# jsourati/nn-active-learning

Hardware: AMD Instinct MI355X
Metric: patches/sec Fisher-scored (32^3, 2-class) (higher is better)
Workload: dtype f32 (fp32 operands split into 16-bit pieces on the 16-bit MFMA, fp32 accumulate: fp16 pairs - 22-23 bits kept per operand, three products - in the conv under the head (forward + backward), in dec1's forward launch and in the other backward launches; bf16 triples - all 24 bits, exact, six products -

## Files before the change

include/alq.h:

```cpp
#ifndef ALQ_H
#define ALQ_H

#include <stddef.h>
#include <stdint.h>

#ifdef __cplusplus
extern "C" {
#endif

typedef struct alq_ctx alq_ctx;
typedef struct alq_model alq_model;

enum { ALQ_OK = 0, ALQ_EINVAL = -1, ALQ_EHIP = -2, ALQ_ENOMEM = -3, ALQ_EUNSUPPORTED = -4 };

enum { ALQ_CONV = 0, ALQ_CONVT = 1, ALQ_POOL = 2, ALQ_FC = 3 };

typedef struct {
    int32_t type;
    int32_t cout;
    int32_t k[3];
    int32_t s[3];
    int32_t relu;
    int32_t skip_src;
} alq_layer_t;
// ... 94 lines not shown
    float focal_gamma;
    float gce_q;
    float lwf_T;
    const float *d_class_w;
    const float *d_sample_w;
    const float *d_targets;
    const float *d_old_logits;
} alq_loss_t;

int alq_loss_stats(alq_ctx *ctx, const float *d_post, int c, int N, const int32_t *d_labels, const alq_loss_t *loss,
                   double *d_stats3);

int alq_param_grads_loss(alq_model *m, const float *d_x, int N, const int32_t *d_labels, const alq_loss_t *loss,
                         float loss_scale, float lwf_scale, float keep_prob, uint64_t seed, int64_t first_sample,
                         const int32_t *h_drop_layers, int n_drop_layers, float *d_grads, float *d_post, double *d_stats3);

int alq_rmsprop_step(alq_ctx *ctx, float *d_theta, const float *d_grad, float *d_ms, float *d_mom, int64_t n, float lr,
                     float decay, float momentum, float eps);

enum { ALQ_MT_L2 = 0, ALQ_MT_CE = 1 };
int64_t alq_mt_trip_voxels(void);
int alq_mt_cotangent(alq_ctx *ctx, const float *d_post, const float *d_teacher_post, int c, int64_t R, const int32_t *d_labels,
                     const alq_loss_t *loss, float loss_scale, float cons_scale, int measure, float *d_rows, double *d_stats3);
int alq_mt_stats(alq_ctx *ctx, const float *d_post, const float *d_teacher_post, int c, int64_t R, const int32_t *d_labels,
                 const alq_loss_t *loss, int measure, double *d_stats3);
int alq_param_grads_loss_mt(alq_model *m, const float *d_x, int N, const int32_t *d_labels, const alq_loss_t *loss,
                            float loss_scale, const float *d_teacher_post, int measure, float cons_scale, float keep_prob,
                            uint64_t seed, int64_t first_sample, const int32_t *h_drop_layers, int n_drop_layers, float *d_grads,
                            float *d_post, double *d_stats3);
int alq_model_set_aleatoric(alq_model *m, int on);
int alq_forward_au(alq_model *m, const float *d_x, int N, float keep_prob, uint64_t seed, int64_t first_sample,
                   const int32_t *h_drop_layers, int n_drop_layers, float *d_post, int64_t *d_pred, float *d_au, float *d_logits);
int64_t alq_mt_au_trip_voxels(void);
int alq_mt_cotangent_au(alq_ctx *ctx, const float *d_post, const float *d_teacher_post, const float *d_au, int c, int64_t R,
                        const int32_t *d_labels, const alq_loss_t *loss, float loss_scale, float cons_scale, float au_scale,
                        float au_log_rel_coeff, int measure, float *d_rows, double *d_stats3);
int alq_mt_stats_au(alq_ctx *ctx, const float *d_post, const float *d_teacher_post, const float *d_au, int c, int64_t R,
                    const int32_t *d_labels, const alq_loss_t *loss, float au_log_rel_coeff, int measure, double *d_stats3);
int alq_param_grads_loss_mt_au(alq_model *m, const float *d_x, int N, const int32_t *d_labels, const alq_loss_t *loss,
                               float loss_scale, const float *d_teacher_post, int measure, float cons_scale, float au_scale,
                               float au_log_rel_coeff, float keep_prob, uint64_t seed, int64_t first_sample,
                               const int32_t *h_drop_layers, int n_drop_layers, float *d_grads, float *d_post, double *d_stats3);
int alq_ema_step(alq_ctx *ctx, float *d_shadow, const float *d_theta, int64_t n, float decay);
int alq_perturb_input(alq_ctx *ctx, const float *d_x, float *d_out, int N, int H, int W, int C, float noise_std, uint64_t seed,
                      int64_t first_sample, int rotate, float angle);

int alq_sq_accum(alq_ctx *ctx, const float *d_grads, int64_t per_sample_len, int N, double *d_acc);

int alq_shrink_sum(alq_ctx *ctx, const float *d_grads, int N, int64_t P, const int64_t *h_layer_elems, int L, double *d_out);
int alq_class_layer_sums(alq_model *m, const float *d_x, int N, int J, const int32_t *d_cls, float *d_post, double *d_g);

int alq_diag_fisher(alq_model *m, const float *d_x, int N, const int32_t *d_cls, double *d_acc);

size_t alq_topk_mask_work_bytes(int64_t n);
int alq_topk_mask(alq_ctx *ctx, const double *d_v, int64_t n, int64_t k, float *d_mask, void *d_work);
int alq_threshold_mask(alq_ctx *ctx, const double *d_v, int64_t n, double thr, float *d_mask);
int alq_fisher_classes(alq_ctx *ctx, const double *d_g, const double *d_w, const double *d_diag, int N, int c, int L,
                       double *d_A);

int alq_row_norms(alq_ctx *ctx, const float *d_A, int64_t n, int f, double *d_norms);
int alq_cosine_sims(alq_ctx *ctx, const float *d_A, int64_t n, const float *d_B, int b, int f, const double *d_na,
                    const double *d_nb, double *d_C);
size_t alq_colsum_work_bytes(int64_t n, int b);
int alq_colsum_max(alq_ctx *ctx, const double *d_S, int64_t n, int b, const double *d_cmax,
                   const unsigned char *d_skip, double *d_out, void *d_work);
int alq_take_colmax(alq_ctx *ctx, const double *d_S, int64_t n, int b, int j, int first, double *d_v);
int alq_fold_rowmax(alq_ctx *ctx, const double *d_S, int t, int64_t n, double *d_v);

int alq_local_var2d(alq_ctx *ctx, const void *d_vol, int vol_is_f64, const int64_t pad_dims[3], const int32_t rads[3], int d,
                    const int64_t *d_inds, int64_t n, double *d_out);
int alq_segment_min(alq_ctx *ctx, const int32_t *d_labels, const int64_t dims[3], int32_t n_labels, const int64_t *d_inds,
                    const double *d_scores, int64_t n, double *d_table);

size_t alq_cc_work_bytes(const int64_t dims[3]);
int alq_cc_label(alq_ctx *ctx, const uint8_t *d_seg, const int64_t dims[3], int connectivity, int select_zero, int32_t *d_labels);
int alq_cc_keep_largest(alq_ctx *ctx, const uint8_t *d_seg, const int64_t dims[3], int connectivity, int skip_origin, uint8_t *d_out,
                        int64_t *d_info, void *d_work);
int alq_fill_holes(alq_ctx *ctx, const uint8_t *d_seg, const int64_t dims[3], uint8_t *d_out, int64_t *d_info, void *d_work);

typedef struct alq_dcrf_params {
    float sdims_smooth[2];
    float sdims_app[2];
    float schan;
    float compat_smooth, compat_app;
    int32_t niter;
} alq_dcrf_params;
size_t alq_dcrf_work_bytes(const int64_t dims[3]);
int alq_dcrf2d(alq_ctx *ctx, const float *d_post, const float *d_img, const int64_t dims[3], const alq_dcrf_params *par,
               float *d_q1, uint8_t *d_map, void *d_work);

int alq_llfc_grads(alq_ctx *ctx, const float *d_feat, const float *d_post, const int32_t *d_labels, int n, int d, int c,
                   float *d_out);
size_t alq_llfc_hess_max_bytes(void);
int alq_llfc_hess(alq_ctx *ctx, const float *d_feat_one, const float *d_post_one, int d, int c, double *d_H);
int alq_llfc_if_path(int d, int c);
size_t alq_llfc_if_work_bytes(int n_pool, int c);
int alq_llfc_stoch_if(alq_ctx *ctx, const float *d_pool_feat, const float *d_pool_post, const int32_t *d_pool_labels, int n_pool,
                      const float *d_tr_feat, const float *d_tr_post, int n_tr, const int32_t *d_draws, int T, double scale, int d,
                      int c, int path, float *d_V, void *d_work);

int alq_aopt_tile(void);
int alq_aopt_max_workgroups(void);
size_t alq_aopt_work_bytes(int64_t n, int L);
int alq_aopt_svec(alq_ctx *ctx, const double *d_A, int64_t n, int L, double *d_V);
int alq_aopt_stats(alq_ctx *ctx, const double *d_V, const double *d_q, int64_t n, int m, const double *h_kvec,
                   const double *h_R, double mu, double obj, double *d_out, void *d_work);
int alq_aopt_direction(alq_ctx *ctx, const double *d_V, const double *d_q, int64_t n, int m, const double *h_kvec,
                       const double *h_R, const double *h_c_r, const double *h_c_1, double ratio, double mu, double obj,
                       double *d_dq, double *d_out, void *d_work);
int alq_aopt_linesearch(alq_ctx *ctx, const double *d_q, const double *d_dq, int64_t n, const double *h_alpha, int J,
                        double *d_out, void *d_work);
int alq_aopt_update(alq_ctx *ctx, double *d_q, const double *d_dq, const double *d_V, int64_t n, int m, double alpha,
                    double *d_out, void *d_work);

typedef struct {
    int32_t layer;
    int32_t pad;
    int64_t idx;
    double delta;
} alq_flip_t;
int alq_ref64_scores(alq_ctx *ctx, const alq_layer_t *layers, int n_layers, const int32_t in_dims[4],
                     const double *const *h_dW, const double *const *h_db, const float *d_x, const int64_t *d_rows, int N,
                     const alq_flip_t *d_flips, int flips_per_sample, double eps, int cand_cap,
                     double *d_logits, double *d_S, double *d_rms, alq_flip_t *d_cand, double *d_cand_key, int32_t *d_cand_count);

int alq_prof_enable(alq_ctx *ctx, int on);
int alq_prof_reset(alq_ctx *ctx);
int alq_prof_num_classes(void);
const char *alq_prof_class_name(int cls);
int alq_prof_read(alq_ctx *ctx, int cls, double *ms, int64_t *launches, double *flops);

int alq_model_debug_copy(alq_model *m, int layer_idx, int what, int N, float *d_out,
                         int64_t *elems_out);

int alq_debug_set_stamp_buffer(void *d_buf);
int alq_debug_set(int key, int value);
enum {
    ALQ_INFO_SUBNORMALS_OK = 0,
    ALQ_INFO_C3D_FWD = 1,
    ALQ_INFO_C3D_BWD = 2,
    ALQ_INFO_C3D_ONE_ACC = 3,
    ALQ_INFO_FLIP_OVERFLOW = 5,
    ALQ_INFO_F16_DERIVED = 6,
    ALQ_INFO_T3D_FWD = 7,
    ALQ_INFO_T3D_BWD = 8,
    ALQ_INFO_E3D_BWD = 9,
    ALQ_INFO_D3D_FWD = 10,
    ALQ_INFO_D3D_BWD = 11,
    ALQ_INFO_F3D_FWD = 12,
    ALQ_INFO_C3D_BWD_FORM = 13,
    ALQ_INFO_HOST_PACK_ELEMS = 14,
    ALQ_INFO_LSUM = 15,
    ALQ_INFO_DCP_FORM = 16,
    ALQ_INFO_E3D_BWD_FORM = 17
};
int alq_model_engine_info(alq_model *m, int what);

int alq_synth_patches(alq_ctx *ctx, uint64_t seed, int64_t first_id, int64_t n,
                      int64_t elems_per_patch, float *d_out);

enum { ALQ_SRC_F32 = 0, ALQ_SRC_F64 = 1, ALQ_SRC_I16 = 2, ALQ_SRC_U8 = 3 };
int alq_vol_pack(alq_ctx *ctx, const void *const *d_src, int m, int src_type, const int32_t *dims, float *d_out);
int alq_mask_pack(alq_ctx *ctx, const uint8_t *d_src, const int32_t *dims, uint8_t *d_out);
int alq_slice_batch_check(const int32_t *h_dims, int nvol, const int32_t *h_desc, int b, const int32_t *crop, int C);
int alq_slice_batch(alq_ctx *ctx, const float *const *h_vols, const uint8_t *const *h_masks, const int32_t *h_dims, int nvol, int m,
                    const int32_t *h_desc, int b, const int32_t *crop, int C, float *d_X, int32_t *d_lab, int64_t *d_counts);
int64_t alq_slice_batch_trip_rows(void);
int alq_slice_batch_launch_samples(void);

#ifdef __cplusplus
}
#endif
#endif
```

nn-active-learning_amd/csrc/alq_internal.h:

```cpp
#pragma once
#include <hip/hip_runtime.h>

#include <cstdint>
#include <cstdio>
#include <memory>
#include <string>
#include <vector>

#include "alq.h"
#include "engine_switches.h"

namespace alq {

void set_error(const char *fmt, ...);

#define ALQ_HIP(expr)                                                                     \
    do {                                                                                  \
        hipError_t e_ = (expr);                                                           \
        if (e_ != hipSuccess) {                                                           \
            ::alq::set_error("%s:%d: %s -> %s", __FILE__, __LINE__, #expr,               \
                             hipGetErrorString(e_));                                      \
            return ALQ_EHIP;                                                              \
        }                                                                                 \
    } while (0)
// ... 254 lines not shown
    float *osumA, *osumB;
    const int *tdesc;
    const int *sdesc;
    const int *pdesc;
    const int *ttab;
    const int *vdesc;
    int in_cs, in_c0, out_cs, out_c0, Co;
    int mask_cs, mask_c0, mask_from, mask_to, split;
    int N, PT, tpg, rows;
    int PX, PYX, PZ;
    int smz, smy, smx;
    int soz, soy, sox, OD, OH, OW;
    int MD, MH, MW;
    int nph, ngr, NP;
    int nslots, plane_bytes;
    int in_pstride, out_pstride, in_bytes;
    int relu, accumulate, pair, store_from;
    int cls_ok;
    int in_split_ch, in_delta, out_split, out_delta, mask_split, mask_delta;
    int tt_ints, pd_off, td_off, wbytes, abytes;
    int dbg_repeat;
    unsigned long long *dbg;
    const unsigned *src_bits;
    int bits_pstride, bits_bytes;
    const float *fc_W;
    float *fc_part;
    unsigned char *fc_bits;
    int fc_F;
    int f16_ein;
    int f16_ew;
    const unsigned *in_amax, *in_amax2;
    unsigned *out_amax;
    int amax_from;
    int wp;
    int src_presplit;
    int xcd_order;
    int zreuse;
    float flip_tau;
    int flip_cap;
    unsigned *flip_cnt;
    unsigned *flip_list;
    const unsigned char *mask_bits;
    unsigned char *sign_out;
};

struct G4Geom {
    int kind = 0;
    int cls[3] = {0, 0, 0};
    int ID = 1, IH = 1, IW = 1, Ci = 0;
    int OD = 1, OH = 1, OW = 1, Co = 0;
    int k[3] = {1, 1, 1}, s[3] = {1, 1, 1}, lo[3] = {0, 0, 0};
    bool flipped = false;
    double flops_per_patch = 0;
};

struct Igemm4Plan {
    bool ok = false;
    Igemm4Args a;
    int NTW = 1;
    int wp = 3;
    int xw = 0;
    std::shared_ptr<Igemm4Plan> alt16;
    bool multi = false;
    bool fic = false;
    int tune_fic = -1;
    int tune_epi = -1;
    size_t lds_bytes = 0;
    double flops_per_patch = 0;
    int Ci = 0, Co = 0;
    struct Unit { int chunk = 0, S = 0, w_off = 0; std::vector<int> tap; };
    std::vector<Unit> units;
    std::vector<int> h_tdesc, h_sdesc, h_pdesc, h_ttab, h_vdesc;
    int *d_tdesc = nullptr, *d_sdesc = nullptr, *d_pdesc = nullptr, *d_ttab = nullptr, *d_vdesc = nullptr;
    std::vector<unsigned short> h_W;
    void *d_W = nullptr;
    std::vector<unsigned short> h_W16;
    void *d_W16 = nullptr;
    int w16_exp = 0;
};
int igemm4_build_plan(const G4Geom &g, int max_batch, Igemm4Plan *plan, int wp = 3);
void igemm4_pack_weights(Igemm4Plan *plan, const std::vector<float> &Bmat );
int igemm4_launch(alq_ctx *ctx, const Igemm4Plan &plan, const View &in, const View &out, const float *bias,
                  int relu, int accumulate, int N, int prof_cls, const Igemm2Fuse *fuse);

struct C3dPlan {
    bool ok = false;
    int D = 0;
    int w_exp = 0;
    int oneacc = 1;
    double flops_per_patch = 0;
    std::vector<unsigned short> h_W;
    void *d_W = nullptr;
    std::vector<unsigned short> h_W7;
    void *d_W7 = nullptr;
};
void c3d_bwd7_pack(C3dPlan *plan, const std::vector<float> &Bmat);
int c3d_subnormals_ok(alq_ctx *ctx);
int c3d_fwd_build(const View &in, const View &out, const int k[3], const int lo[3], const int s[3], C3dPlan *plan);
void c3d_fwd_pack(C3dPlan *plan, const std::vector<float> &Bmat );
int c3d_fwd_launch(alq_ctx *ctx, const C3dPlan &plan, const View &in, const float *bias, int N, const unsigned *amaxA, const unsigned *amaxB,
                   const float *fc_W, float *fc_part, float *asum_part, unsigned char *fc_bits, float flip_tau);
int c3d_bwd_build(const View &fwd_in, const View &fwd_out, const int k[3], const int lo[3], const int s[3], C3dPlan *plan);
void c3d_bwd_pack(C3dPlan *plan, const std::vector<float> &Bmat_fwd );
void c3d_presplit_vec(const float *v, long long F, int e, std::vector<unsigned short> *out);
int c3d_bwd_launch(alq_ctx *ctx, const C3dPlan &plan, int N, const unsigned char *bits, const void *vec16, int e_in, const unsigned char *maskA,
                   float *dB, float *sumA, float *sumB, int rows_per_wave = 8);

struct T3dPlan {
    bool ok = false;
    int kind = 0;
    int w_exp = 0;
    double flops_per_patch = 0;
    std::vector<unsigned short> h_W;
    void *d_W = nullptr;
};
int t3d_build(const View &in, const View &out, const int k[3], const int lo[3], const int s[3], T3dPlan *fwd, T3dPlan *bwd);
void t3d_fwd_pack(T3dPlan *plan, const float *W );
void t3d_bwd_pack(T3dPlan *plan, const float *W);
void t3d8_fwd_pack(T3dPlan *plan, const float *W );
void t3d8_bwd_pack(T3dPlan *plan, const float *W );
int t3d8_bwd_launch(alq_ctx *ctx, const T3dPlan &plan, const View &dout, const View &din, int N, float in_bound, const unsigned char *mask_bits, float *dsum);
int t3d_fwd_launch(alq_ctx *ctx, const T3dPlan &plan, const View &in, const View &out, const float *bias, int N, float *osum, unsigned *out_amax);
int t3d_bwd_launch(alq_ctx *ctx, const T3dPlan &plan, const View &dout, const View &din, int N, float in_bound, const unsigned char *mask_bits,
                   float *dsum);

struct E3dPlan {
    bool ok = false;
    int w_exp = 0;
    double flops_per_patch = 0;
    std::vector<unsigned short> h_Whi, h_Wlo;
    void *d_Whi = nullptr, *d_Wlo = nullptr;
};
int e3d_build(const View &in, const View &out, const int k[3], const int lo[3], const int s[3], E3dPlan *plan);
void e3d_pack(E3dPlan *plan, const float *W );
int e3d_bwd_launch(alq_ctx *ctx, const E3dPlan &plan, int N, const float *skip, const float *dpool, const unsigned char *am2, const unsigned char *sg2,
                   const unsigned char *am1, const unsigned char *sg1, float *dsum2, float *dsum1, float in_bound,
                   bool rows );

struct D3dPlan {
    bool ok = false;
    int w_exp = 0;
    double flops_per_patch = 0;
    std::vector<unsigned short> h_Whi, h_Wlo;
    void *d_Whi = nullptr, *d_Wlo = nullptr;
    std::vector<unsigned short> h_Bhi, h_Blo;
    void *d_Bhi = nullptr, *d_Blo = nullptr;
};
void d3d_bwd_pack(D3dPlan *plan, const float *W);
int d3d_bwd_launch(alq_ctx *ctx, const D3dPlan &plan, int N, const float *dout, float in_bound, float *dinA, float *dinB, float *sumB);
int d3d_build(const View &in, const View &out, const int k[3], const int lo[3], const int s[3], D3dPlan *plan);
void d3d_pack(D3dPlan *plan, const float *W );
int d3d_fwd_launch(alq_ctx *ctx, const D3dPlan &plan, int N, const float *inA, const float *inB, const unsigned *amaxA, const unsigned *amaxB,
                   const float *bias, int relu, float *out, unsigned char *sg, float *osum);

struct F3dPlan {
    bool ok = false;
    int w_exp = 0;
    double flops_per_patch = 0;
    std::vector<unsigned short> h_Whi, h_Wlo;
    void *d_Whi = nullptr, *d_Wlo = nullptr;
};
int f3d_build(const View &in, const View &out, const int k[3], const int lo[3], const int s[3], F3dPlan *plan);
void f3d_pack(F3dPlan *plan, const float *W );
int f3d_fwd_launch(alq_ctx *ctx, const F3dPlan &plan, int N, const float *in, const unsigned *amax, const float *bias, float *out, unsigned char *sg,
                   float *osum, float *pout, unsigned char *parg, float *posum);

struct DirectArgs {
    const float *in;
    float *out;
    const float *W;
    const float *bias;
    float *osum;
    int in_cs, in_c0, Ci, ID, IH, IW;
    int out_cs, out_c0, Co, OD, OH, OW;
    int MD, MH, MW;
    int PT, TZ, TY, TX, HZ, HY, HX, rows;
    int minz, miny, minx;
    int ntaps, tnx, tny, tnz;
    int tilesZ, tilesY, tilesX;
    int N, relu;
};

struct DirectPlan {
    DirectArgs a;
    bool ok = false;
    size_t lds_bytes = 0;
    double flops_per_patch = 0;
    float *d_W = nullptr;
};

int direct_build_plan(const IgemmPlan &p1, DirectPlan *dp);
int direct_launch(alq_ctx *ctx, const DirectPlan &dp, const View &in, const View &out, const float *bias, int relu,
                  int N, float *osum, int prof_cls);
int direct_conv_pool_launch(alq_ctx *ctx, const float *d_W, const View &in, const View &out, const View &pout,
                            const float *bias, int relu, uint8_t *argmax, float *osum, float *posum, int N,
                            double flops_per_patch, unsigned *amax = nullptr, unsigned char *sg = nullptr, unsigned char *psg = nullptr);

struct FcGemmPlan {
    bool ok = false;
    int K = 0, N = 0;
    std::vector<unsigned short> h_W;
    void *d_W = nullptr;
    std::vector<unsigned short> h_W16;
    void *d_W16 = nullptr;
    int w_exp = 0;
    int form = 0;
};
int fcgemm_build_plan(int K, int N, FcGemmPlan *plan);
void fcgemm_pack_weights(FcGemmPlan *plan, const std::vector<float> &Bmat );
void fcgemm_pack_weights_f16(FcGemmPlan *plan, const std::vector<float> &Bmat );
int fcgemm_launch(alq_ctx *ctx, const FcGemmPlan &plan, const View &in, const View &out, const float *bias, int relu,
                  int M, int prof_cls, float in_bound = 0.f, unsigned *row_amax = nullptr);

int wpack_stats(alq_ctx *ctx, const float *d_W, int Co, long long F, void *d_scal);
int wpack_permute(alq_ctx *ctx, const float *d_W, float *d_Wp, int Co, int D, int H, int Wd, int C);
int wpack_fc(alq_ctx *ctx, const float *d_Wp, long long ld, int K, int N, int kmajor, void *d_W3, void *d_W16, const void *d_scal);

struct Gemm {
    IgemmPlan p1;
    Igemm2Plan p2;
    Igemm3Plan p3;
    Igemm4Plan p4;
    FcGemmPlan pfc;
    bool pfc_f16 = false;
    bool p3_f16 = false;
    unsigned *fc_row_amax = nullptr;
    DirectPlan pd;
};

int k_pool_fwd(alq_ctx *, const View &in, const View &out, uint8_t *argmax, const int w[3],
               const int lo[3], int N, float *osum = nullptr, bool *fused = nullptr);
int k_pool_bwd_first(alq_ctx *, const View &dout, const View &pool_out, const uint8_t *argmax, const int w[3],
                     int ID, int IH, int IW, int N, float *dsum, int accumulate, int use_signs = 0);
int k_pool_bwd(alq_ctx *, const View &dout, const View &din, const uint8_t *argmax,
               const int w[3], const int lo[3], int N, int accumulate, const View *mask_act = nullptr,
               float *dsum = nullptr, bool *fused = nullptr, int store_din = 1, int use_signs = 0);
int k_chansum(alq_ctx *, const View &in, float *field, int N);
int k_mask_chansum(alq_ctx *, const View &dact, const View *act_or_null, float *field, int N);
int boxdot_slabs(long long vox);
int boxdot_conv_slabs(int D, int H, int W, const int k[3]);
int boxdot_convT_slabs(int ID, int IH, int IW, const int k[3], const int s[3]);
int k_boxdot_conv(alq_ctx *, const float *dsum, const float *asum, const float *asum2, int D, int H, int W,
                  const int k[3], const int lo[3], int N, double *Spart, int nslab_max);
int k_boxdot_convT(alq_ctx *, const float *dsum, const float *asum, const float *asum2, int ID, int IH, int IW,
                   const int k[3], const int s[3], const int lo[3], int N, double *Spart, int nslab_max);
int k_fc_small_fwd(alq_ctx *, const float *act, int64_t F, const float *Wp, int nout, int N,
                   float *partials, int nslices, unsigned *maskbits = nullptr);
int k_fc_small_dsum_bits(alq_ctx *, const unsigned *maskbits, const float *wv, int64_t F, int N, float *dsum);
int k_fc_small_finish(alq_ctx *, const float *partials, int nslices, const float *bias, int nout,
                      int relu, int N, float *out);
int k_fc_small_finish_diff(alq_ctx *, const float *partials, int nslices, const float *bias, int N, float *out);
int k_fc_small_bwd(alq_ctx *, const float *delta, int nout, const float *Wp, int64_t F, int N,
                   float *dact, const float *mask_act = nullptr, float *dsum = nullptr, int C = 0,
                   bool *fused = nullptr);
int k_rowsum_field(alq_ctx *, const float *field, int64_t len, int N, float *out);
struct FwdBoundsArgs { int nl; float L[16]; float B[16]; int src2[16]; int from_input = 0; };
int k_rowmax_abs(alq_ctx *, const float *x, int N, long long K, unsigned *out);
int k_fwd_bounds(alq_ctx *, const unsigned *amax0, int N, int stride, const FwdBoundsArgs &a, unsigned *bound_all);
int flip_segments(int N);
int flip_list_len(int N);
int k_flip_fix(alq_ctx *, unsigned *list, unsigned *cnt, int cap, int N, const float *inA, const float *inB, int CA, int CB,
               int D, int H, int W, int kz, int ky, int kx, int lz, int ly, int lx, const float *W32, const float *bias, int Co,
               unsigned char *bits, long long F, unsigned *overflow = nullptr);
int k_rowmax_u32(alq_ctx *, const unsigned *in, int len, int N, unsigned *out);
int k_softmax(alq_ctx *, const float *logits, int c, int N, float *post_cN, int64_t *pred);
int k_fill_unit_cotangent(alq_ctx *, float *dlogits, int N);
int k_fisher_finalize(alq_ctx *, const double *Spart, const int *nslab, int nslab_max, int max_batch, double *S,
                      int L, const double *sizes, const float *post_cN, const float *p1_branch, int N,
                      double diag_load, float *p1_out, double *g0, double *g1, double *A, double *trace,
                      double *Apart, int *nblocks_out);
int k_reduce_Asum(alq_ctx *, const double *Apart, int nblocks, int LL, double *Asum);
int fc_small_slices(int64_t F);

int k_dropout(alq_ctx *, const View &t, int N, long long first_sample, unsigned long long seed, int layer, float keep_prob);
int k_logit_cotangent(alq_ctx *, const float *post_cN, int c, int N, int mode, int cls, const int *labels, float scale,
                      float *dlogits);
int k_ce_loss(alq_ctx *, const float *post_cN, int c, int N, const int *labels, double *d_out);
long long wgrad_partial_floats(const View &U, const View &V, const int k[3]);
int k_wgrad(alq_ctx *, const View &U, const View &V, const int k[3], const int s[3], const int lo[3], int N, int sum_n,
            float *partial, float *d_out, long long out_stride);
int k_bgrad(alq_ctx *, const View &delta, int N, int sum_n, float *d_out, long long out_stride);
int k_fc_wgrad(alq_ctx *, const float *delta, const View &a, int nout, int N, int sum_n, float *d_out, long long out_stride);
int k_sgd(alq_ctx *, float *theta, const float *g, long long n, float lr);
int k_loss_cotangent(alq_ctx *, const float *post_cN, int c, int N, const int *labels, const alq_loss_t *loss, float loss_scale,
                     float lwf_scale, float *dlogits, double *d_stats3);
int k_dense_head_fwd(alq_ctx *, const float *x, long long R, int Ci, int c, const float *W, const float *b, float *post_cR, int64_t *pred,
                     float *z);
int k_dense_head_fwd_au(alq_ctx *, const float *x, long long R, int Ci, int c, const float *W, const float *b, float *post_cR,
                        int64_t *pred, float *au, float *z);
int k_dense_head_bwd(alq_ctx *, const float *delta, const float *x, long long R, int Ci, int c, const float *W, float *dx, int accumulate,
                     double *part, float *d_dW_db);
int k_rmsprop(alq_ctx *, float *theta, const float *g, float *ms, float *mom, long long n, float lr, float decay, float momentum,
              float eps);
int k_adam(alq_ctx *, float *theta, const float *g, float *m, float *v, long long n, float lr_t, float b1, float b2, float eps);
int k_sq_accum(alq_ctx *, const float *g, long long per, int N, double *acc);
int k_shrink_sum(alq_ctx *, const float *g, int N, long long P, const long long *off, int L, double *out);
int k_fisher_classes(alq_ctx *, const double *g, const double *w, const double *diag, int N, int c, int L, double *A);

long long gnorm_partials(const View &U, const View &V, const int k[3], const int s[3], const int lo[3]);
int k_gnorm_weight(alq_ctx *, const View &U, const View &V, const int k[3], const int s[3], const int lo[3], int N, double *part,
                   double *d_sq, int ld, int col);
int k_gnorm_bias(alq_ctx *, const View &delta, int N, double *d_sq, int ld, int col);
int k_gnorm_fc(alq_ctx *, const float *delta, int nout, const View &a, int N, double *d_sq, int ld, int col);

long long dfisher_weight_scratch(const View &U, const View &V, const int k[3], const int s[3], const int lo[3], int max_batch);
int k_dfisher_weight(alq_ctx *, const View &U, const View &V, const int k[3], const int s[3], const int lo[3], int N, double *scratch,
// ... 98 lines not shown
```

nn-active-learning_amd/csrc/engine_switches.h:

```cpp
#ifndef ALQ_ENGINE_SWITCHES_H
#define ALQ_ENGINE_SWITCHES_H
#include <cstddef>
#include <cstdlib>

namespace alq {

enum Knob {
    KNOB_REPEAT = 0,
    KNOB_FLAGS = 1,
    KNOB_NO_BWD_FUSE = 2,
    KNOB_NO_FWD_FUSE = 3,
    KNOB_NO_V3 = 4,
    KNOB_NO_V4 = 5,
    KNOB_NO_POOL_FIRST = 6,
    KNOB_NO_CONV_POOL = 7,
    KNOB_DCP_NARROW = 8,
    KNOB_E3D_GRID_CAP = 9,
    ALQ_NKNOBS = 10
};

struct EngineSwitches {
    int knobs[ALQ_NKNOBS] = {0, 0, 0, 0, 0, 0, 0, 0, 0, 0};
    int disable_v2 = 0;
    int disable_v3 = 0;
    int disable_v4 = 0;
    int no_fcgemm = 0;
    int no_split = 0;
    int no_wide2d_rule = 0;
    int no_v3_f16 = 0;
    int no_v3_f16_fwd = 0;
    int no_co_split = 0;
    int no_co_split_f16 = 0;
    int no_class_tiles = 0;
    int no_fc_bits = 0;
    int no_fc_fuse = 0;
    int no_fc_f16 = 0;
    int no_fc_f16_fwd = 0;
    int f16_derived_mask = 0;
    int has_f16_derived_mask = 0;
    int no_f16x2 = 0;
    int no_xcd_order = 0;
    int no_fixed = 0;
    int no_bound16 = 0;
    int no_flipfix = 0;
    int no_presplit = 0;
    int no_signs = 0;
    int no_signs0 = 0;
    int f16_fwd_mask = -1;
    int no_f16_derived = 0;
    int no_light_kernels = 0;
    int no_c3d = 0;
    int c3_bwd_rows = 7;
    int no_e3d = 0;
    int e3d_rows = 0;
    int no_d3d = 0;
    int no_d3b = 0;
    int no_f3d = 0;
    int no_t3d = 0;
};

enum SwitchRule {
    SW_PRESENT,
    SW_FIRST_IS_1,
    SW_ATOI_EQ,
    SW_INT,
    SW_ROWS
};

struct SwitchRow {
    const char *env;
    size_t member;
    SwitchRule rule;
    int arg;
};

#define ALQ_SW(env, member, rule, arg) {env, offsetof(EngineSwitches, member), rule, arg}
inline const SwitchRow kSwitchTable[] = {
    ALQ_SW("ALQ_DEBUG_REPEAT", knobs[KNOB_REPEAT], SW_INT, 0),
    ALQ_SW("ALQ_DEBUG_FLAGS", knobs[KNOB_FLAGS], SW_INT, 0),
    ALQ_SW("ALQ_NO_BWD_FUSE", knobs[KNOB_NO_BWD_FUSE], SW_INT, 0),
    ALQ_SW("ALQ_NO_FWD_FUSE", knobs[KNOB_NO_FWD_FUSE], SW_INT, 0),
    ALQ_SW("ALQ_NO_V3", knobs[KNOB_NO_V3], SW_INT, 0),
    ALQ_SW("ALQ_NO_V4", knobs[KNOB_NO_V4], SW_INT, 0),
    ALQ_SW("ALQ_NO_POOL_FIRST", knobs[KNOB_NO_POOL_FIRST], SW_INT, 0),
    ALQ_SW("ALQ_NO_CONV_POOL", knobs[KNOB_NO_CONV_POOL], SW_INT, 0),
    ALQ_SW("ALQ_DCP_NARROW", knobs[KNOB_DCP_NARROW], SW_INT, 0),
    ALQ_SW("ALQ_E3D_GRID_CAP", knobs[KNOB_E3D_GRID_CAP], SW_INT, 0),
    ALQ_SW("ALQ_DISABLE_V2", disable_v2, SW_FIRST_IS_1, 0),
    ALQ_SW("ALQ_DISABLE_V3", disable_v3, SW_FIRST_IS_1, 0),
    ALQ_SW("ALQ_DISABLE_V4", disable_v4, SW_PRESENT, 0),
    ALQ_SW("ALQ_NO_FCGEMM", no_fcgemm, SW_PRESENT, 0),
    ALQ_SW("ALQ_NO_SPLIT", no_split, SW_PRESENT, 0),
    ALQ_SW("ALQ_NO_WIDE2D_RULE", no_wide2d_rule, SW_PRESENT, 0),
    ALQ_SW("ALQ_NO_V3_F16", no_v3_f16, SW_PRESENT, 0),
    ALQ_SW("ALQ_NO_V3_F16_FWD", no_v3_f16_fwd, SW_PRESENT, 0),
    ALQ_SW("ALQ_NO_CO_SPLIT", no_co_split, SW_PRESENT, 0),
    ALQ_SW("ALQ_NO_CO_SPLIT_F16", no_co_split_f16, SW_PRESENT, 0),
    ALQ_SW("ALQ_NO_CLASS_TILES", no_class_tiles, SW_PRESENT, 0),
    ALQ_SW("ALQ_NO_FC_BITS", no_fc_bits, SW_PRESENT, 0),
    ALQ_SW("ALQ_NO_FC_FUSE", no_fc_fuse, SW_PRESENT, 0),
    ALQ_SW("ALQ_NO_FC_F16", no_fc_f16, SW_PRESENT, 0),
    ALQ_SW("ALQ_NO_FC_F16_FWD", no_fc_f16_fwd, SW_PRESENT, 0),
    ALQ_SW("ALQ_F16_DERIVED_MASK", f16_derived_mask, SW_INT, 0),
    ALQ_SW("ALQ_F16_DERIVED_MASK", has_f16_derived_mask, SW_PRESENT, 0),
    ALQ_SW("ALQ_NO_F16X2", no_f16x2, SW_PRESENT, 0),
    ALQ_SW("ALQ_NO_XCD_ORDER", no_xcd_order, SW_PRESENT, 0),
    ALQ_SW("ALQ_NO_FIXED", no_fixed, SW_PRESENT, 0),
    ALQ_SW("ALQ_NO_BOUND16", no_bound16, SW_PRESENT, 0),
    ALQ_SW("ALQ_NO_FLIPFIX", no_flipfix, SW_PRESENT, 0),
    ALQ_SW("ALQ_NO_PRESPLIT", no_presplit, SW_PRESENT, 0),
    ALQ_SW("ALQ_NO_SIGNS", no_signs, SW_PRESENT, 0),
    ALQ_SW("ALQ_NO_SIGNS0", no_signs0, SW_PRESENT, 0),
    ALQ_SW("ALQ_F16_FWD_MASK", f16_fwd_mask, SW_INT, 0),
    ALQ_SW("ALQ_F16_DERIVED", no_f16_derived, SW_ATOI_EQ, 0),
    ALQ_SW("ALQ_NO_F16_DERIVED", no_f16_derived, SW_ATOI_EQ, 1),
    ALQ_SW("ALQ_NO_LIGHT_KERNELS", no_light_kernels, SW_PRESENT, 0),
    ALQ_SW("ALQ_NO_C3D", no_c3d, SW_PRESENT, 0),
    ALQ_SW("ALQ_C3D_BWD_ROWS", c3_bwd_rows, SW_ROWS, 0),
    ALQ_SW("ALQ_NO_E3D", no_e3d, SW_PRESENT, 0),
    ALQ_SW("ALQ_E3D_ROWS", e3d_rows, SW_ATOI_EQ, 1),
    ALQ_SW("ALQ_NO_D3D", no_d3d, SW_PRESENT, 0),
    ALQ_SW("ALQ_NO_D3D_BWD", no_d3b, SW_PRESENT, 0),
    ALQ_SW("ALQ_NO_F3D", no_f3d, SW_PRESENT, 0),
    ALQ_SW("ALQ_NO_T3D", no_t3d, SW_PRESENT, 0),
};
#undef ALQ_SW
inline const int kNumSwitchRows = (int)(sizeof(kSwitchTable) / sizeof(kSwitchTable[0]));

inline int &switch_member(EngineSwitches &sw, const SwitchRow &row) {
    return *reinterpret_cast<int *>(reinterpret_cast<char *>(&sw) + row.member);
}

inline EngineSwitches read_engine_switches() {
    EngineSwitches sw;
    for (const SwitchRow &row : kSwitchTable) {
        const char *v = std::getenv(row.env);
        int &dst = switch_member(sw, row);
        switch (row.rule) {
            case SW_PRESENT:    if (v) dst = 1; break;
            case SW_FIRST_IS_1: if (v && v[0] == '1') dst = 1; break;
            case SW_ATOI_EQ:    if (v && std::atoi(v) == row.arg) dst = 1; break;
            case SW_INT:        if (v) dst = std::atoi(v); break;
            case SW_ROWS:       dst = (v && std::atoi(v) == 4) ? 4 : ((v && std::atoi(v) == 8) ? 8 : 7); break;
        }
    }
    return sw;
}

}
#endif
```

nn-active-learning_amd/csrc/igemm2.hip:

```cpp
#include "alq_internal.h"

#include <algorithm>
#include <cmath>
#include <cstring>

namespace alq {

typedef float f32x4 __attribute__((ext_vector_type(4)));
typedef float f32x2 __attribute__((ext_vector_type(2)));

#ifdef ALQ_STAMPS
#define STAMP(var) asm volatile("s_memtime %0\n\ts_waitcnt lgkmcnt(0)" : "=s"(var)::"memory")
#define PHASE_END(idx)                         \
    do {                                       \
        unsigned long long t_now_;             \
        STAMP(t_now_);                         \
        ph[idx] += t_now_ - t_last;            \
        t_last = t_now_;                       \
    } while (0)
#else
#define PHASE_END(idx) do {} while (0)
#endif

constexpr int I2_CBP = 12;
// ... 331 lines not shown
                        mm(a1, b1);
                        __builtin_amdgcn_sched_barrier(0);
                    }
                }
            }
            PHASE_END(6);
        }
        have_pend = true;
        p_out = c_out; p_cls = c_cls; p_l = c_l; p_g = c_g;
        more = next_more;
    }
    if (have_pend) flush();
#ifdef ALQ_STAMPS
    PHASE_END(7);
    if (a.dbg && tid == 0)
        for (int i = 0; i < 8; ++i) a.dbg[blockIdx.x * 8 + i] = ph[i];
#endif
}

int igemm2_build_plan(const IgemmPlan &p1, Igemm2Plan *p2) {
    p2->ok = false;
    const IgemmArgs &a1 = p1.a;
    if (p1.smallc || p1.CB != 8 || a1.NB != 1 || p1.NTW > 3 || a1.ntaps > 27 || a1.Co % 4) return ALQ_OK;
    const int halo = a1.HZ * a1.HY * a1.HX;
    const int nhv = a1.PT * halo;
    if (nhv * 2 > 256 * I2_MAXSLOT) return ALQ_OK;
    if (a1.HZ > 255 || a1.HY > 255 || a1.HX > 255 || a1.PT > 127) return ALQ_OK;
    const size_t wchunk = (size_t)a1.ntaps * p1.NTW * 128 * 4;
    size_t wres_max = I2_WRES_MAX;
    if (const char *e = getenv("ALQ_WRES_KB")) wres_max = (size_t)atoi(e) * 1024;
    const bool wres = wchunk * a1.nchunks <= wres_max * p1.NTW;
    const size_t wbytes = wres ? wchunk * a1.nchunks : wchunk;
    const size_t lds = wbytes + (size_t)nhv * I2_CBP * 4;
    if (lds > 156 * 1024) return ALQ_OK;
    Igemm2Args &a = p2->a;
    std::memset(&a, 0, sizeof(a));
    a.Ci = a1.Ci; a.ID = a1.ID; a.IH = a1.IH; a.IW = a1.IW;
    a.Co = a1.Co; a.OD = a1.OD; a.OH = a1.OH; a.OW = a1.OW;
    a.MD = a1.MD; a.MH = a1.MH; a.MW = a1.MW;
    a.sm = a1.sm; a.so = a1.so; a.ooffz = a1.ooffz; a.ooffy = a1.ooffy; a.ooffx = a1.ooffx;
    a.PT = a1.PT; a.TZ = a1.TZ; a.TY = a1.TY; a.TX = a1.TX; a.HZ = a1.HZ; a.HY = a1.HY; a.HX = a1.HX;
    a.rows = a1.rows; a.minz = a1.minz; a.miny = a1.miny; a.minx = a1.minx;
    a.ntaps = a1.ntaps; a.nchunks = a1.nchunks;
    a.tilesZ = a1.tilesZ; a.tilesY = a1.tilesY; a.tilesX = a1.tilesX;
    {
        std::vector<int> off(a1.ntaps);
        for (int t = 0; t < a1.ntaps; ++t) off[t] = a1.tapoff[t] / 10 * I2_CBP;
        bool found = false;
        for (int nx = 1; nx <= a1.ntaps && !found; ++nx) {
            if (a1.ntaps % nx) continue;
            for (int ny = 1; nx * ny <= a1.ntaps && !found; ++ny) {
                if ((a1.ntaps / nx) % ny) continue;
                const int nz = a1.ntaps / (nx * ny);
                const int sx = nx > 1 ? off[1] - off[0] : 0;
                const int sy = ny > 1 ? off[nx] - off[0] : 0;
                const int sz = nz > 1 ? off[nx * ny] - off[0] : 0;
                bool okb = true;
                for (int t = 0; t < a1.ntaps && okb; ++t) {
                    const int ix = t % nx, iy = (t / nx) % ny, iz = t / (nx * ny);
                    okb = off[t] == off[0] + iz * sz + iy * sy + ix * sx;
                }
                if (okb) {
                    a.t0 = off[0]; a.tsx = sx; a.tsy = sy; a.tsz = sz; a.tnx = nx; a.tny = ny;
                    found = true;
                }
            }
        }
        if (!found) return ALQ_OK;
    }
    a.split = 1 << 30;
    {
        const int dimsI[3] = {a.ID, a.IH, a.IW}, dimsM[3] = {a.MD, a.MH, a.MW};
        const int T[3] = {a.TZ, a.TY, a.TX}, tiles[3] = {a.tilesZ, a.tilesY, a.tilesX};
        const int mins[3] = {a.minz, a.miny, a.minx}, H[3] = {a.HZ, a.HY, a.HX};
        auto cls_of = [&](int d, int t) { return (t == 0 ? 1 : 0) | (t == tiles[d] - 1 ? 2 : 0); };
        auto valid1 = [&](int d, int t, int h) {
            const int c = t * T[d] * a.sm + mins[d] + h;
            return c >= 0 && c < dimsI[d];
        };
        for (int d = 0; d < 3; ++d)
            for (int t = 1; t + 1 < tiles[d]; ++t)
                for (int h = 0; h < H[d]; ++h)
                    if (!valid1(d, t, h)) return ALQ_OK;
        a.tpg = a.tilesZ * a.tilesY * a.tilesX;
        a.in_pstride = a.PT * a.ID * a.IH * a.IW;
        a.out_pstride = a.PT * a.OD * a.OH * a.OW;
        p2->h_tdesc.assign((size_t)a.tpg * 8, 0);
        for (int tz = 0; tz < a.tilesZ; ++tz)
            for (int ty = 0; ty < a.tilesY; ++ty)
                for (int tx = 0; tx < a.tilesX; ++tx) {
                    int *td = &p2->h_tdesc[(((size_t)tz * a.tilesY + ty) * a.tilesX + tx) * 8];
                    const int mz0 = tz * a.TZ, my0 = ty * a.TY, mx0 = tx * a.TX;
                    const int z0 = mz0 * a.sm + a.minz, y0 = my0 * a.sm + a.miny, x0 = mx0 * a.sm + a.minx;
                    td[0] = (z0 * a.IH + y0) * a.IW + x0;
                    td[1] = ((mz0 * a.so + a.ooffz) * a.OH + my0 * a.so + a.ooffy) * a.OW + mx0 * a.so + a.ooffx;
                    const int cls = cls_of(0, tz) | (cls_of(1, ty) << 2) | (cls_of(2, tx) << 4);
                    const bool full = a.rows == 256 && mz0 + a.TZ <= a.MD && my0 + a.TY <= a.MH && mx0 + a.TX <= a.MW;
                    td[2] = cls | (full ? 256 : 0);
                    td[3] = mz0; td[4] = my0; td[5] = mx0;
                }
        (void)dimsM;
        auto rep = [&](int d, int c) { return (c & 1) ? 0 : ((c & 2) ? tiles[d] - 1 : (tiles[d] > 2 ? 1 : 0)); };
        p2->h_sdesc.assign((size_t)nhv * 4, 0);
        for (int pt = 0; pt < a.PT; ++pt)
            for (int hz = 0; hz < a.HZ; ++hz)
                for (int hy = 0; hy < a.HY; ++hy)
                    for (int hx = 0; hx < a.HX; ++hx) {
                        const int hv = ((pt * a.HZ + hz) * a.HY + hy) * a.HX + hx;
                        int *sd = &p2->h_sdesc[(size_t)hv * 4];
                        sd[0] = ((pt * a.ID + hz) * a.IH + hy) * a.IW + hx;
                        unsigned long long m = 0;
                        for (int c = 0; c < 64; ++c) {
                            const int cz = c & 3, cy = (c >> 2) & 3, cx = (c >> 4) & 3;
                            if (valid1(0, rep(0, cz), hz) && valid1(1, rep(1, cy), hy) && valid1(2, rep(2, cx), hx))
                                m |= 1ull << c;
                        }
                        sd[1] = (int)(unsigned)(m & 0xffffffffull);
                        sd[2] = (int)(unsigned)(m >> 32);
                        sd[3] = (pt << 24) | (hz << 16) | (hy << 8) | hx;
                    }
    }
    p2->NTW = p1.NTW;
    p2->wres = wres;
    p2->lds_bytes = lds;
    int max_wgs = 2;
    if (const char *e = getenv("ALQ_MAX_WGS")) max_wgs = atoi(e);
    p2->wgs_per_cu = std::max<int>(1, std::min<int>(max_wgs, (int)((160 * 1024) / (lds + 512))));
    p2->flops_per_patch = p1.flops_per_patch;
    p2->ok = true;
    return ALQ_OK;
}

void igemm2_pack_weights(Igemm2Plan *p2, const std::vector<float> &Bmat) {
    const Igemm2Args &a = p2->a;
    const int NTW = p2->NTW, Ci = a.Ci, Co = a.Co;
    p2->h_W.assign((size_t)a.nchunks * a.ntaps * NTW * 128, 0.f);
    for (int ch = 0; ch < a.nchunks; ++ch)
        for (int tp = 0; tp < a.ntaps; ++tp)
            for (int nt = 0; nt < NTW; ++nt)
                for (int lane = 0; lane < 64; ++lane)
                    for (int s = 0; s < 2; ++s) {
                        const int c = ch * 8 + 2 * (lane >> 4) + s;
                        const int co = nt * 16 + (lane & 15);
                        if (co < Co)
                            p2->h_W[((((size_t)ch * a.ntaps + tp) * NTW + nt) * 64 + lane) * 2 + s] =
                                Bmat[((size_t)tp * Ci + c) * Co + co];
                    }
}

unsigned long long *g_igemm2_dbg = nullptr;
int g_no_f16x2 = 0;
int g_no_xcd_order = 0;
int g_no_fixed = 0;
int g_dbg_knobs[ALQ_NKNOBS] = {0, 0, 0, 0, 0, 0, 0, 0, 0, 0};

template <int NTW, bool WRES, int GEO, bool SUMS>
static int launch2_s(alq_ctx *ctx, const Igemm2Plan &plan, const Igemm2Args &a, unsigned grid) {
    auto kfn = igemm2_kernel<NTW, WRES, GEO, SUMS>;
    if (plan.lds_bytes > 64 * 1024)
        ALQ_HIP(hipFuncSetAttribute(reinterpret_cast<const void *>(kfn), hipFuncAttributeMaxDynamicSharedMemorySize,
                                    (int)plan.lds_bytes));
    hipLaunchKernelGGL(kfn, dim3(grid), dim3(256), plan.lds_bytes, ctx->stream, a);
    ALQ_HIP(hipGetLastError());
    return ALQ_OK;
}

template <int NTW, bool WRES, int GEO>
static int launch2_t(alq_ctx *ctx, const Igemm2Plan &plan, const Igemm2Args &a, unsigned grid) {
    return (a.osumA || a.osumB) ? launch2_s<NTW, WRES, GEO, true>(ctx, plan, a, grid)
                                : launch2_s<NTW, WRES, GEO, false>(ctx, plan, a, grid);
}

int igemm2_launch(alq_ctx *ctx, const Igemm2Plan &plan, const View &in, const View &out, const float *bias, int relu,
                  int accumulate, int N, int prof_cls, const Igemm2Fuse *fuse) {
    Igemm2Args a = plan.a;
    ALQ_REQUIRE(in.C == a.Ci && in.D == a.ID && in.H == a.IH && in.W == a.IW, ALQ_EINVAL,
                "igemm2: input view does not match plan");
    ALQ_REQUIRE(out.C == a.Co && out.D == a.OD && out.H == a.OH && out.W == a.OW, ALQ_EINVAL,
                "igemm2: output view does not match plan");
    ALQ_REQUIRE(plan.d_W != nullptr, ALQ_EINVAL, "igemm2: weights not set");
    ALQ_REQUIRE((long long)N * in.vox() * in.cs < (1LL << 29) && (long long)N * out.vox() * out.cs < (1LL << 29),
                ALQ_EUNSUPPORTED, "igemm2: tensor exceeds the 32-bit byte-offset range (lower the batch)");
    ALQ_REQUIRE(in.cs % 4 == 0 && in.c0 % 4 == 0 && out.cs % 4 == 0 && out.c0 % 4 == 0, ALQ_EUNSUPPORTED,
                "igemm2: channel slice not 16-byte aligned");
    if (fuse) ALQ_REQUIRE(fuse->split % 4 == 0 && fuse->mask_cs % 4 == 0 && fuse->mask_c0 % 4 == 0 && fuse->mask_from % 4 == 0, ALQ_EUNSUPPORTED,
                          "igemm2: fused epilogue needs 4-channel aligned slices");
    a.in = in.p; a.in_cs = in.cs; a.in_c0 = in.c0;
    a.out = out.p; a.out_cs = out.cs; a.out_c0 = out.c0;
    a.W = plan.d_W; a.bias = bias; a.relu = relu; a.accumulate = accumulate; a.N = N;
    a.in_bytes = (int)((long long)N * in.vox() * in.cs * 4);
    a.dbg = nullptr;
    if (g_igemm2_dbg) {
        static int want = -2;
        if (want == -2) { const char *e = getenv("ALQ_STAMP_ONLY"); want = e ? atoi(e) : -1; }
        static int ordinal = 0;
        static unsigned long long *last = nullptr;
        if (last != g_igemm2_dbg) { last = g_igemm2_dbg; ordinal = 0; }
        if (want < 0 || ordinal == want) a.dbg = g_igemm2_dbg;
        ++ordinal;
    }
    a.dbg_repeat = g_dbg_knobs[KNOB_REPEAT];
    a.dbg_flags = g_dbg_knobs[KNOB_FLAGS];
    if (fuse) {
        a.mask = fuse->mask; a.mask_cs = fuse->mask_cs; a.mask_c0 = fuse->mask_c0; a.mask_from = fuse->mask_from;
        a.osumA = fuse->osumA; a.osumB = fuse->osumB;
        a.split = fuse->split > 0 ? fuse->split : (1 << 30);
    }
    const int pgroups = (N + a.PT - 1) / a.PT;
    const long long total = (long long)pgroups * a.tilesZ * a.tilesY * a.tilesX;
    const unsigned grid = (unsigned)std::min<long long>(total, 256LL * plan.wgs_per_cu);
    ProfScope ps(ctx, prof_cls, plan.flops_per_patch * N);
    int geo = 0;
    if (a.ntaps == 27 && a.tnx == 3 && a.tny == 3 && a.HY == 6 && a.HX == 18) {
        const int SX = I2_CBP, SY = 18 * I2_CBP, SZ = 6 * 18 * I2_CBP;
        if (a.t0 == 0 && a.tsx == SX && a.tsy == SY && a.tsz == SZ) geo = 1;
        if (a.t0 == 2 * (SX + SY + SZ) && a.tsx == -SX && a.tsy == -SY && a.tsz == -SZ) geo = 2;
    }
#define ALQ_L2(NT)                                                                                       \
    case NT:                                                                                             \
        if (geo == 1) return plan.wres ? launch2_t<NT, true, 1>(ctx, plan, a, grid) : launch2_t<NT, false, 1>(ctx, plan, a, grid); \
        if (geo == 2) return plan.wres ? launch2_t<NT, true, 2>(ctx, plan, a, grid) : launch2_t<NT, false, 2>(ctx, plan, a, grid); \
        return plan.wres ? launch2_t<NT, true, 0>(ctx, plan, a, grid) : launch2_t<NT, false, 0>(ctx, plan, a, grid)
    switch (plan.NTW) { ALQ_L2(1); ALQ_L2(2); ALQ_L2(3); }
#undef ALQ_L2
    set_error("igemm2: NTW=%d unsupported", plan.NTW);
    return ALQ_EUNSUPPORTED;
}

}
```

nn-active-learning_amd/csrc/model.hip:

```cpp
#include <algorithm>
#include <cmath>
#include <cstring>
#include <string>

#include "model_types.h"

namespace alq {

static void same_pads(int in, int k, int s, int *out, int *lo) {
    *out = (in + s - 1) / s;
    int total = (*out - 1) * s + k - in;
    if (total < 0) total = 0;
    *lo = total / 2;
}

}

using namespace alq;

static int g_knob_override[ALQ_NKNOBS] = {-1, -1, -1, -1, -1, -1, -1, -1, -1, -1};

static void apply_knobs(const alq_model *m) {
    for (int k = 0; k < ALQ_NKNOBS; ++k) g_dbg_knobs[k] = g_knob_override[k] >= 0 ? g_knob_override[k] : m->sw.knobs[k];
    g_no_f16x2 = m->sw.no_f16x2;
    g_no_xcd_order = m->sw.no_xcd_order;
    g_no_fixed = m->sw.no_fixed;
}

static int gemm_build(const EngineSwitches &sw, const ConvDesc &d, int max_batch, Gemm *g, const G4Geom *g4 = nullptr) {
    ALQ_TRY(igemm_build_plan(d, max_batch, &g->p1));
    if (g4 && !sw.disable_v4) {
        G4Geom gg = *g4;
        gg.flops_per_patch = g->p1.flops_per_patch;
        ALQ_TRY(igemm4_build_plan(gg, max_batch, &g->p4));
    }
    ALQ_TRY(igemm2_build_plan(g->p1, &g->p2));
    ALQ_TRY(direct_build_plan(g->p1, &g->pd));
    if (sw.disable_v2) { g->p2.ok = false; g->pd.ok = false; }
    ALQ_TRY(igemm3_build_plan(g->p2, &g->p3));
    if (d.ID == 1 && d.IH == 1 && d.IW == 1 && d.tz.size() == 1 && d.sm == 1 && d.so == 1 && !sw.no_fcgemm)
        ALQ_TRY(fcgemm_build_plan(d.Ci, d.Co, &g->pfc));
    if (sw.disable_v3) g->p3.ok = false;
    return ALQ_OK;
}

int prepare_call(alq_model *m, bool fisher) {
    m->last.call_fisher = fisher;
    apply_knobs(m);
    if (!two_slot_allowed()) ALQ_TRY(refresh_fallback_forms(m));
    return ALQ_OK;
}

enum GemmRoute { ROUTE_DIRECT, ROUTE_FCGEMM, ROUTE_IGEMM4, ROUTE_IGEMM3, ROUTE_IGEMM2, ROUTE_IGEMM };
static GemmRoute gemm_route(const Gemm &g, const View &in, const View &out, int accumulate, const Igemm2Fuse *fuse) {
    if (g.pd.ok && !accumulate && !(fuse && (fuse->mask || fuse->osumB || fuse->split))) return ROUTE_DIRECT;
    if (g.pfc.ok && !accumulate && !fuse && two_slot_allowed()) return ROUTE_FCGEMM;
    const bool split_view = in.split != 0 || out.split != 0;
    if (g.p4.ok && (two_slot_allowed() || split_view)) return ROUTE_IGEMM4;
    if (g.p3.ok && !g_dbg_knobs[KNOB_NO_V3]) return ROUTE_IGEMM3;
    return g.p2.ok ? ROUTE_IGEMM2 : ROUTE_IGEMM;
}

int gemm_launch(alq_ctx *ctx, const Gemm &g, const View &in, const View &out, const float *bias, int relu,
                int accumulate, int N, int cls, const Igemm2Fuse *fuse, bool *fused, float fc_in_bound) {
    const GemmRoute route = gemm_route(g, in, out, accumulate, fuse);
    ALQ_REQUIRE(route <= ROUTE_FCGEMM || g.p4.ok || (in.split == 0 && out.split == 0), ALQ_EUNSUPPORTED, "split concat view without a two-slot plan");
    if (fused) *fused = fuse != nullptr && route != ROUTE_FCGEMM && route != ROUTE_IGEMM;
    const int cls3 = cls == PROF_IGEMM_BWD ? PROF_IGEMM3_BWD : PROF_IGEMM3_FWD;
    switch (route) {
        case ROUTE_DIRECT: return direct_launch(ctx, g.pd, in, out, bias, relu, N, fuse ? fuse->osumA : nullptr, PROF_DIRECT);
        case ROUTE_FCGEMM:
            return fcgemm_launch(ctx, g.pfc, in, out, bias, relu, N, cls3, (g_no_f16x2 || bias || relu) ? 0.f : fc_in_bound,
                                 (cls == PROF_IGEMM_FWD && !g_no_f16x2) ? g.fc_row_amax : nullptr);
        case ROUTE_IGEMM4: return igemm4_launch(ctx, g.p4, in, out, bias, relu, accumulate, N, cls3, fuse);
        case ROUTE_IGEMM3: return igemm3_launch(ctx, g.p2, g.p3, in, out, bias, relu, accumulate, N, cls3, fuse);
        case ROUTE_IGEMM2: return igemm2_launch(ctx, g.p2, in, out, bias, relu, accumulate, N, cls, fuse);
        case ROUTE_IGEMM: break;
    }
    return igemm_launch(ctx, g.p1, in, out, bias, relu, accumulate, N, cls);
}

static void enum_taps(const int k[3], std::vector<int> *tz, std::vector<int> *ty, std::vector<int> *tx) {
    for (int z = 0; z < k[0]; ++z)
        for (int y = 0; y < k[1]; ++y)
            for (int x = 0; x < k[2]; ++x) {
                tz->push_back(z); ty->push_back(y); tx->push_back(x);
            }
}

static int build_model(alq_model *m, const alq_layer_t *specs, int n_layers) {
    const EngineSwitches &sw = m->sw;
    m->layers.resize(n_layers);
    struct Shp { int D, H, W, C; };
    std::vector<Shp> outs(n_layers);
    Shp cur = {m->in_dims[0], m->in_dims[1], m->in_dims[2], m->in_dims[3]};
    bool flat = false;
    int pidx = 0;
    std::vector<int> src_of(n_layers, -1);
    std::vector<int> dest_of(n_layers, -1);
    for (int i = 0; i < n_layers; ++i) {
        Layer &ly = m->layers[i];
        ly.spec = specs[i];
        const alq_layer_t &sp = ly.spec;
        Shp in = cur;
        if (sp.skip_src >= 0) {
            ALQ_REQUIRE(sp.skip_src < i - 1, ALQ_EUNSUPPORTED, "layer %d: skip source %d must be an earlier, non-adjacent layer", i, sp.skip_src);
            ALQ_REQUIRE(dest_of[sp.skip_src] < 0, ALQ_EUNSUPPORTED, "layer %d feeds more than one concat", sp.skip_src);
            const Shp &s = outs[sp.skip_src];
            ALQ_REQUIRE(!flat && s.D == cur.D && s.H == cur.H && s.W == cur.W, ALQ_EUNSUPPORTED,
                        "layer %d: concat of maps of different size (resize_image_with_crop_or_pad) is outside the scored path", i);
            in.C = cur.C + s.C;
            src_of[i] = sp.skip_src;
            dest_of[sp.skip_src] = i;
        }
        Shp o = in;
        switch (sp.type) {
            case ALQ_CONV: {
                ALQ_REQUIRE(!flat, ALQ_EINVAL, "layer %d: conv after fc", i);
                ALQ_REQUIRE(sp.s[0] == 1 && sp.s[1] == 1 && sp.s[2] == 1, ALQ_EUNSUPPORTED, "layer %d: strided conv", i);
                for (int d = 0; d < 3; ++d) {
                    int od;
                    same_pads((&in.D)[d], sp.k[d], 1, &od, &ly.lo[d]);
                }
                o.C = sp.cout;
                ly.pidx = pidx++;
                ly.w_elems = (int64_t)sp.k[0] * sp.k[1] * sp.k[2] * in.C * sp.cout;
                ly.b_elems = sp.cout;
                break;
            }
            case ALQ_CONVT: {
                ALQ_REQUIRE(!flat, ALQ_EINVAL, "layer %d: conv_transpose after fc", i);
                for (int d = 0; d < 3; ++d) {
                    ALQ_REQUIRE(sp.k[d] >= sp.s[d], ALQ_EUNSUPPORTED, "layer %d: conv_transpose kernel < stride", i);
                    int od;
                    same_pads((&in.D)[d] * sp.s[d], sp.k[d], sp.s[d], &od, &ly.lo[d]);
                }
                ALQ_REQUIRE(sp.s[0] == sp.s[1] || in.D == 1, ALQ_EUNSUPPORTED, "layer %d: anisotropic stride", i);
                ALQ_REQUIRE(sp.s[1] == sp.s[2], ALQ_EUNSUPPORTED, "layer %d: anisotropic stride", i);
                o.D = in.D * sp.s[0]; o.H = in.H * sp.s[1]; o.W = in.W * sp.s[2];
                o.C = sp.cout;
                ly.pidx = pidx++;
                ly.w_elems = (int64_t)sp.k[0] * sp.k[1] * sp.k[2] * in.C * sp.cout;
                ly.b_elems = sp.cout;
                break;
            }
            case ALQ_POOL: {
                ALQ_REQUIRE(!flat, ALQ_EINVAL, "layer %d: pool after fc", i);
                for (int d = 0; d < 3; ++d) {
                    ALQ_REQUIRE(sp.k[d] == sp.s[d], ALQ_EUNSUPPORTED, "layer %d: pool window != stride", i);
                    ALQ_REQUIRE(sp.k[0] * sp.k[1] * sp.k[2] <= 255, ALQ_EUNSUPPORTED, "layer %d: pool window too large", i);
                    same_pads((&in.D)[d], sp.k[d], sp.s[d], &(&o.D)[d], &ly.lo[d]);
                }
                break;
            }
            case ALQ_FC: {
                ly.F = (int64_t)in.D * in.H * in.W * in.C;
                o = {1, 1, 1, sp.cout};
                ly.pidx = pidx++;
                ly.w_elems = ly.F * sp.cout;
                ly.b_elems = sp.cout;
                flat = true;
                break;
            }
            default:
                ALQ_REQUIRE(false, ALQ_EINVAL, "layer %d: unknown type %d", i, sp.type);
        }
        outs[i] = o;
        cur = o;
    }
    m->L = pidx;
    if (n_layers > 0 && specs[n_layers - 1].type == ALQ_CONV) {
        const int hl = n_layers - 1;
        const alq_layer_t &hs = specs[hl];
// ... 270 lines not shown
            }
        } else if (sp.type == ALQ_POOL) {
            uint8_t *am;
            ALQ_TRY(m->dalloc(&am, (size_t)NB * ly.out.vox() * ly.out.C));
            ly.argmax = am;
        } else {
            ALQ_REQUIRE(ly.in.cs == ly.in.C && ly.in.c0 == 0, ALQ_EUNSUPPORTED, "layer %d: fc on a concat slice", i);
            if (sp.cout <= 8) {
                ly.dense_fc_small = true;
                ly.fc_slices = fc_small_slices(ly.F);
                ALQ_TRY(m->dalloc(&ly.d_Wp, (size_t)sp.cout * ly.F));
                ALQ_TRY(m->dalloc(&ly.fc_partials, (size_t)NB * ly.fc_slices * sp.cout));
                if (sp.cout == 2 && ly.F % 1024 == 0 && i == n_layers - 1 && i > 0 && m->layers[i - 1].spec.relu && m->layers[i - 1].pidx > 0 &&
                    m->layers[i - 1].spec.type == ALQ_CONV && m->layers[i - 1].out.C == 8 && !sw.no_fc_bits) {
                    ALQ_TRY(m->dalloc(&ly.fc_maskbits, (size_t)NB * (ly.F / 16)));
                    ALQ_TRY(m->dalloc(&ly.fc_wv, (size_t)ly.F));
                    ALQ_TRY(m->dalloc(&ly.fc_wv16, (size_t)ly.F));
                    const Layer &cv = m->layers[i - 1];
                    const Igemm4Plan &fp = cv.fwd[0].p4;
                    if (sp.cout == 2 && !sp.relu && fp.ok && fp.NTW == 1 && !fp.multi && fp.a.pair && fp.a.PT == 1 && cv.out.cs == 8 &&
                        cv.out.c0 == 0 && !cv.out.split && cv.osum && !cv.out_is_skip_src && !sw.no_fc_fuse &&
                        cv.bwd.p4.ok && cv.bwd.p4.NTW == 1 && !cv.bwd.p4.multi && cv.bwd.p4.a.PT == 1 && !cv.dout.split) {
                        ly.fc_slices2 = fp.a.tpg * 4;
                        ALQ_TRY(m->dalloc(&ly.fc_part2, (size_t)NB * ly.fc_slices2));
                        if (cv.c3f.ok && ly.F == (int64_t)cv.out.vox() * 8) {
                            ALQ_TRY(m->dalloc(&ly.c3_part, (size_t)NB * 4));
                            ALQ_TRY(m->dalloc(&ly.c3_asum, (size_t)NB * 4));
                            if (cv.c3b.ok) ALQ_TRY(m->dalloc(&ly.fc_wv16c, (size_t)ly.F * 2));
                        }
                    }
                }
            } else {
                ConvDesc d;
                d.ID = d.IH = d.IW = 1; d.Ci = (int)ly.F;
                d.OD = d.OH = d.OW = 1; d.Co = sp.cout;
                d.MD = d.MH = d.MW = 1;
                d.tz = {0}; d.ty = {0}; d.tx = {0};
                ly.fwd.resize(1);
                ALQ_TRY(gemm_build(sw, d, NB, &ly.fwd[0]));
                if (ly.fwd[0].pfc.ok && !sw.no_fc_f16_fwd) {
                    ly.fwd[0].pfc_f16 = true;
                    ALQ_TRY(m->dalloc(&ly.fwd[0].fc_row_amax, (size_t)m->max_batch));
                }
                if (!first_param) {
                    ConvDesc b = d;
                    b.Ci = sp.cout; b.Co = (int)ly.F;
                    ALQ_TRY(gemm_build(sw, b, NB, &ly.bwd));
                    ly.bwd.pfc_f16 = ly.bwd.pfc.ok && !sw.no_fc_f16;
                    ly.has_bwd = true;
                }
            }
        }
    }
    ALQ_HIP(hipMemcpy(m->sizes, h_sizes.data(), m->L * sizeof(double), hipMemcpyHostToDevice));
    std::vector<int> h_nslab(m->L, 1);
    for (const Layer &ly : m->layers) {
        if (ly.pidx < 0) continue;
        if (ly.spec.type == ALQ_CONV) h_nslab[ly.pidx] = boxdot_conv_slabs(ly.out.D, ly.out.H, ly.out.W, ly.spec.k);
        else if (ly.spec.type == ALQ_CONVT) h_nslab[ly.pidx] = boxdot_convT_slabs(ly.in.D, ly.in.H, ly.in.W, ly.spec.k, ly.spec.s);
        else h_nslab[ly.pidx] = boxdot_slabs(1);
        m->nslab_max = std::max(m->nslab_max, h_nslab[ly.pidx]);
    }
    ALQ_TRY(m->dalloc(&m->nslab, (size_t)m->L));
    ALQ_TRY(m->dalloc(&m->Spart, (size_t)m->L * NB * m->nslab_max));
    ALQ_HIP(hipMemcpy(m->nslab, h_nslab.data(), m->L * sizeof(int), hipMemcpyHostToDevice));
    return ALQ_OK;
}

View flat_view(const View &v) {
    View f;
    f.p = v.p; f.D = f.H = f.W = 1;
    f.C = (int)(v.vox() * v.C); f.cs = f.C; f.c0 = 0;
    return f;
}

static int ensure_bounds(alq_model *m) {
    if (m->bound_all) return ALQ_OK;
    const int nl = (int)m->layers.size();
    ALQ_TRY(m->dalloc(&m->bound_all, (size_t)nl * m->max_batch));
    for (int k = 0; k < nl; ++k) m->layers[k].bound_fwd = m->bound_all + (size_t)k * m->max_batch;
    return ALQ_OK;
}

static int ensure_amax_tiles(alq_model *m, size_t len) {
    if (len <= m->amax_tiles_len) return ALQ_OK;
    ALQ_TRY(m->dalloc(&m->amax_tiles, (size_t)m->max_batch * len));
    m->amax_tiles_len = len;
    return ALQ_OK;
}

static FwdBoundsArgs fwd_bounds_args(const alq_model *m) {
    const int nl = (int)m->layers.size();
    FwdBoundsArgs ba;
    ba.nl = nl;
    for (int k = 0; k < nl && k < 16; ++k) {
        const Layer &lk = m->layers[k];
        const bool par = lk.pidx >= 0 && lk.spec.type != ALQ_FC;
        ba.L[k] = par ? lk.out_l1 : 1.f;
        ba.B[k] = par ? lk.out_bmax : 0.f;
        ba.src2[k] = lk.spec.skip_src;
    }
    return ba;
}


static bool dcp_applies(const alq_model *m, int i, const DropSpec *drop) {
    if (i != 0 || m->layers.size() < 2) return false;
    const Layer &ly = m->layers[0], &nx = m->layers[1];
    const alq_layer_t &sp = ly.spec;
    const View &in = ly.in;
    return ly.spec.type == ALQ_CONV && nx.spec.type == ALQ_POOL && ly.fwd[0].pd.ok && ly.fwd[0].pd.d_W && in.C == 1 && in.cs == 1 &&
           sp.cout == 8 && sp.k[0] == 3 && sp.k[1] == 3 && sp.k[2] == 3 && ly.lo[0] == 1 && ly.lo[1] == 1 && ly.lo[2] == 1 &&
           nx.spec.k[0] == 2 && nx.spec.k[1] == 2 && nx.spec.k[2] == 2 && nx.lo[0] == 0 && nx.lo[1] == 0 && nx.lo[2] == 0 &&
           in.D % 2 == 0 && in.H % 2 == 0 && in.W % 2 == 0 && nx.out.D * 2 == in.D && nx.out.H * 2 == in.H &&
           nx.out.W * 2 == in.W && ((ly.out.cs | ly.out.c0 | nx.out.cs | nx.out.c0) & 3) == 0 && !g_dbg_knobs[KNOB_NO_CONV_POOL] &&
           !(drop && (drop->on(0) || drop->on(1)));
}

static bool flipfix_applies(const alq_model *m, const Layer &ly, const Layer &nx, const View &in, const Igemm2Fuse &fz, bool with_sums) {
    const alq_layer_t &sp = ly.spec;
    return with_sums && fz.fc_bits && fz.in_amax && !g_no_f16x2 && !m->sw.no_flipfix && ly.d_W32 && ly.fwd_l1 > 0.f &&
           sp.s[0] == 1 && sp.s[1] == 1 && sp.s[2] == 1 && in.c0 == 0 && nx.F % 64 == 0 &&
           ((in.split == 0 && in.cs == in.C) || (in.split > 0 && in.cs == in.split && in.C == 2 * in.split));
}

static bool c3d_fwd_applies(const alq_model *m, const Layer &ly, const Layer &nx, const Igemm2Fuse &fz) {
    return ly.c3f.ok && ly.c3f.d_W && nx.c3_part && fz.in_amax && fz.in_amax2 && !g_no_f16x2 && !m->sw.no_c3d;
}

static bool d3d_fwd_applies(const alq_model *m, int i, const View &in, const Igemm2Fuse *fuse, const std::vector<char> &prod, bool with_sums,
                            bool light, const DropSpec *drop) {
    const Layer &ly = m->layers[i];
    return fuse && ly.d3f.ok && ly.d3f.d_Whi && !m->sw.no_d3d && fuse->in_amax && fuse->in_amax2 && !prod[i] && !g_no_f16x2 && two_slot_allowed() &&
           ((with_sums && fuse->osumA) || (light && !m->sw.no_light_kernels)) && in.split == 16 && !(drop && drop->on(i));
}

static bool f3d_fwd_applies(const alq_model *m, int i, const View &in, const Igemm2Fuse *fuse, const std::vector<char> &prod,
                            const std::vector<char> &cons, bool with_sums, bool light, const DropSpec *drop) {
    const Layer &ly = m->layers[i];
    const Layer *nx = i + 1 < (int)m->layers.size() ? &m->layers[i + 1] : nullptr;
    return fuse && ly.f3f.ok && ly.f3f.d_Whi && !m->sw.no_f3d && cons[i] == 2 && fuse->in_amax && !fuse->in_amax2 && !prod[i] && !g_no_f16x2 && two_slot_allowed() &&
           ((with_sums && fuse->osumA) || (light && !m->sw.no_light_kernels)) && ly.spec.relu && in.split == 0 && !(drop && (drop->on(i) || drop->on(i + 1))) && nx && nx->spec.type == ALQ_POOL &&
           nx->spec.k[0] == 2 && nx->spec.k[1] == 2 && nx->spec.k[2] == 2 && nx->lo[0] == 0 && nx->lo[1] == 0 && nx->lo[2] == 0 && nx->out.D == 8 && nx->out.H == 8 &&
           nx->out.W == 8 && nx->out.C == 16 && nx->out.cs == 16 && nx->out.c0 == 0 && !nx->out.split && nx->argmax && !prod[i + 1];
}

static bool t3d_fwd_applies(const alq_model *m, int i, const std::vector<char> &prod, const std::vector<char> &cons, bool with_sums,
                            const DropSpec *drop) {
    const Layer &ly = m->layers[i];
    return ly.t3f.ok && ly.t3f.d_W && !m->sw.no_t3d && !g_dbg_knobs[KNOB_NO_FWD_FUSE] && two_slot_allowed() && !cons[i] && !ly.spec.relu &&
           !(drop && drop->on(i)) && (!with_sums || ly.osum) && !(ly.t3f.kind == 8 && prod[i]);
}

int run_forward(alq_model *m, const float *d_x, int N, bool with_sums, bool keep_all, const DropSpec *drop) {
    alq_ctx *ctx = m->ctx;
    const int nl = (int)m->layers.size();
    bool skip_next = false;
    bool fc_head_fused = false;
    bool c3_head = false;
    m->last.fwd = {};
    const bool no16 = g_no_f16x2 != 0;
    std::vector<char> prod(nl, 0), cons(nl, 0);
    const bool light = !with_sums && !keep_all;
    if ((with_sums || light) && !no16 && !g_dbg_knobs[KNOB_NO_FWD_FUSE] && two_slot_allowed()) {
        auto prod_ok = [&](int p) {
            if (p < 0) return false;
            const Layer &l = m->layers[p];
            if (p == 0 && dcp_applies(m, 0, drop)) return true;
            if (!l.osum) return false;
            if (l.spec.type == ALQ_CONV) return l.fwd[0].p4.ok && !l.fwd[0].pd.ok && !l.fwd[0].pfc.ok && l.fwd[0].p4.a.PT == 1;
            if (l.spec.type == ALQ_CONVT) return l.fwd_all.ok && l.fwd_all.a.PT == 1;
            return false;
        };
        size_t need = 0;
        for (int j = 1; j < nl; ++j) {
            const Layer &l = m->layers[j];
            if (l.dense_head) continue;
            const Igemm4Plan *pl = l.spec.type == ALQ_CONV ? &l.fwd[0].p4 : (l.spec.type == ALQ_CONVT ? &l.fwd_all : nullptr);
            if (!pl || !pl->ok || !pl->d_W16 || pl->multi || pl->a.PT != 1 || !l.osum) continue;
            if (l.spec.type == ALQ_CONV && (l.fwd[0].pd.ok || l.fwd[0].pfc.ok)) continue;
            const int s_ = l.spec.skip_src;
            if (m->sw.f16_fwd_mask < 0 && !m->sw.no_f16_derived && nl <= 16 && ((m->f16_fwd_derived >> j) & 1) && l.spec.type == ALQ_CONV && dcp_applies(m, 0, drop) &&
                (s_ >= 0) == (l.in.split != 0) && !(drop && drop->layers)) {
                cons[j] = 2;
                prod[0] = 1;
                continue;
            }
            if (!(j == nl - 2 && m->layers[nl - 1].fc_part2 && l.spec.type == ALQ_CONV) && m->sw.f16_fwd_mask < 0) continue;
            if (l.spec.type == ALQ_CONVT && !pl->fic) continue;
            if (!prod_ok(j - 1) || (s_ >= 0 && !prod_ok(s_))) continue;
            if ((s_ >= 0) != (l.in.split != 0)) continue;
            if (m->sw.f16_fwd_mask >= 0 && !((m->sw.f16_fwd_mask >> j) & 1)) continue;
            cons[j] = 1; prod[j - 1] = 1;
            if (s_ >= 0) prod[s_] = 1;
        }
        for (int p = 0; p < nl; ++p) {
            if (!prod[p]) continue;
            Layer &l = m->layers[p];
            if (!l.amax_fwd) ALQ_TRY(m->dalloc(&l.amax_fwd, (size_t)m->max_batch));
            if (l.spec.type == ALQ_CONV && !(p == 0 && dcp_applies(m, 0, drop))) need = std::max(need, (size_t)l.fwd[0].p4.a.tpg * 4);
            if (l.spec.type == ALQ_CONVT) need = std::max(need, (size_t)l.fwd_all.a.tpg * (l.fwd_all.multi ? l.fwd_all.a.ngr : 1) * 4);
            if (l.spec.type == ALQ_CONVT && l.t3f.ok) need = std::max(need, (size_t)16);
        }
        ALQ_TRY(ensure_amax_tiles(m, need));
    }
    bool any_derived = false;
    for (int j = 0; j < nl; ++j) any_derived = any_derived || cons[j] == 2;
    m->last.fwd.f16_derived = any_derived;
    if (any_derived) ALQ_TRY(ensure_bounds(m));
    const bool v3f16 = m->v3_fwd_f16 && (with_sums || light) && !no16 && !drop && !any_derived && !dcp_applies(m, 0, drop) && nl <= 16 &&
                       !g_dbg_knobs[KNOB_NO_FWD_FUSE] && two_slot_allowed() && m->layers[0].in.split == 0 && m->layers[0].in.cs == m->layers[0].in.C;
    if (v3f16) {
        if (!m->in_amax) ALQ_TRY(m->dalloc(&m->in_amax, (size_t)m->max_batch));
        ALQ_TRY(ensure_bounds(m));
        ALQ_TRY(k_rowmax_abs(ctx, d_x, N, (long long)m->layers[0].in.vox() * m->layers[0].in.C, m->in_amax));
        FwdBoundsArgs ba = fwd_bounds_args(m);
        ba.from_input = 1;
        ALQ_TRY(k_fwd_bounds(ctx, m->in_amax, N, m->max_batch, ba, m->bound_all));
    }
    auto take_amax = [&](Igemm2Fuse &fz, int j) {
        if (!cons[j]) return;
        const bool dv = cons[j] == 2;
        fz.in_amax = dv ? m->layers[j - 1].bound_fwd : m->layers[j - 1].amax_fwd;
        if (m->layers[j].spec.skip_src >= 0) {
            const Layer &sl = m->layers[m->layers[j].spec.skip_src];
            fz.in_amax2 = dv ? sl.bound_fwd : sl.amax_fwd;
        }
    };
    for (Layer &l : m->layers) l.signs_ready = false;
    for (int i = 0; i < nl; ++i) {
        Layer &ly = m->layers[i];
        ALQ_REQUIRE(ly.pidx < 0 || ly.weights_set, ALQ_EINVAL, "weights of parameterised layer %d not set", ly.pidx);
        if (ly.dense_head) break;
        if (skip_next) { skip_next = false; continue; }
        View in = ly.in;
        if (i == 0) in.p = const_cast<float *>(d_x);
        Igemm2Fuse fz;
        fz.osumA = with_sums ? ly.osum : nullptr;
        const bool head_conv = i + 2 == nl && m->layers[nl - 1].fc_part2 && ly.spec.type == ALQ_CONV;
        const bool light_here = light && (prod[i] || cons[i] || head_conv);
        const Igemm2Fuse *fuse = ((with_sums || light_here) && ly.osum && !g_dbg_knobs[KNOB_NO_FWD_FUSE]) ? &fz : nullptr;
        bool fused = false;
        switch (ly.spec.type) {
            case ALQ_CONV: {
                Layer *nx = i + 1 < nl ? &m->layers[i + 1] : nullptr;
                const alq_layer_t &sp = ly.spec;
                if (dcp_applies(m, i, drop)) {
                    if (prod[i]) ALQ_HIP(hipMemsetAsync(ly.amax_fwd, 0, (size_t)N * sizeof(unsigned), ctx->stream));
                    const bool sg_here = with_sums && !m->sw.no_signs && !m->sw.no_signs0 && sp.relu && ly.out.sg != nullptr;
                    ALQ_TRY(direct_conv_pool_launch(ctx, ly.fwd[0].pd.d_W, in, ly.out, nx->out, ly.d_bias, sp.relu, nx->argmax,
                                                    with_sums ? ly.osum : nullptr, with_sums ? nx->osum : nullptr, N,
                                                    ly.fwd[0].pd.flops_per_patch, prod[i] ? ly.amax_fwd : nullptr,
                                                    sg_here ? ly.out.sg : nullptr, (sg_here && nx->out.sg) ? nx->out.sg : nullptr));
                    m->last.fwd.dcp = g_dcp_last_form;
                    ly.signs_ready = sg_here;
                    nx->signs_ready = sg_here && nx->out.sg != nullptr;
                    if (any_derived)
                        ALQ_TRY(k_fwd_bounds(ctx, ly.amax_fwd, N, m->max_batch, fwd_bounds_args(m), m->bound_all));
                    fused = true;
                    skip_next = true;
                    break;
                }
                if (fuse && nx && i + 2 == nl && nx->fc_part2 && two_slot_allowed()) {
                    fz.fc_W = nx->fc_wv; fz.fc_F = nx->F; fz.fc_part = nx->fc_part2; fz.fc_bits = with_sums ? nx->fc_maskbits : nullptr;
                    take_amax(fz, i);
                    const bool flipfix = flipfix_applies(m, ly, *nx, in, fz, with_sums);
                    if (flipfix) {
                        if (!m->flip_list) {
                            m->flip_cap = flip_list_len(m->max_batch);
                            ALQ_TRY(m->dalloc(&m->flip_cnt, (size_t)flip_segments(m->max_batch)));
                            ALQ_TRY(m->dalloc(&m->flip_list, (size_t)m->flip_cap));
                            ALQ_TRY(m->dalloc(&m->flip_overflow, (size_t)1));
                            ALQ_HIP(hipMemsetAsync(m->flip_overflow, 0, sizeof(unsigned), ctx->stream));
                        }
                        fz.flip_cnt = m->flip_cnt; fz.flip_list = m->flip_list; fz.flip_cap = m->flip_cap; fz.flip_l1 = ly.fwd_l1; fz.flip_bias_nonzero = ly.out_bmax > 0.f;
                    }
                    c3_head = c3d_fwd_applies(m, ly, *nx, fz);
                    if (c3_head)
                        ALQ_TRY(c3d_fwd_launch(ctx, ly.c3f, in, ly.d_bias, N, fz.in_amax, fz.in_amax2, nx->fc_wv, nx->c3_part,
                                               with_sums ? nx->c3_asum : nullptr, reinterpret_cast<unsigned char *>(fz.fc_bits),
                                               flipfix ? std::ldexp(ly.fwd_l1, -24) : 0.f));
                    else
                        ALQ_TRY(igemm4_launch(ctx, ly.fwd[0].p4, in, ly.out, ly.d_bias, ly.spec.relu, 0, N, PROF_IGEMM3_FWD, &fz));
                    if (flipfix)
                        ALQ_TRY(k_flip_fix(ctx, m->flip_list, m->flip_cnt, m->flip_cap, N, in.p, in.split ? in.p + in.delta : nullptr,
                                           in.split ? in.split : in.C, in.split ? in.C - in.split : 0, in.D, in.H, in.W, sp.k[0], sp.k[1], sp.k[2],
                                           ly.lo[0], ly.lo[1], ly.lo[2], ly.d_W32, ly.d_bias, sp.cout,
                                           reinterpret_cast<unsigned char *>(nx->fc_maskbits), nx->F, m->flip_overflow));
                    fused = true;
                    fc_head_fused = true;
                    m->last.fwd.head_fused = true;
                    m->last.fwd.c3 = c3_head;
                    break;
                }
                if (fuse) take_amax(fz, i);
                if (d3d_fwd_applies(m, i, in, fuse, prod, with_sums, light, drop)) {
                    const bool sgd = with_sums && !m->sw.no_signs && ly.spec.relu && ly.out.sg;
                    ALQ_TRY(d3d_fwd_launch(ctx, ly.d3f, N, in.p, in.p + in.delta, fz.in_amax, fz.in_amax2, ly.d_bias, ly.spec.relu ? 1 : 0, ly.out.p,
                                           sgd ? ly.out.sg : nullptr, fz.osumA));
                    ly.signs_ready = sgd;
                    fused = true;
                    m->last.fwd.d3f = 1;
                    break;
                }
                if (f3d_fwd_applies(m, i, in, fuse, prod, cons, with_sums, light, drop)) {
                    const bool sgd = with_sums && !m->sw.no_signs && ly.out.sg;
                    ALQ_TRY(f3d_fwd_launch(ctx, ly.f3f, N, in.p, fz.in_amax, ly.d_bias, ly.out.p, sgd ? ly.out.sg : nullptr, fz.osumA, nx->out.p, nx->argmax,
                                           with_sums ? nx->osum : nullptr));
                    ly.signs_ready = sgd;
                    nx->signs_ready = false;
                    fused = true;
                    skip_next = true;
                    m->last.fwd.f3f = 1;
                    break;
                }
                if (fuse && prod[i]) fz.out_amax = m->amax_tiles;
                if (!ly.fwd_co.empty() && !prod[i] && !cons[i] && two_slot_allowed()) {
                    Igemm2Fuse sz;
                    const bool s16 = v3f16 && i >= 1 && in.split == 0 && ly.spec.skip_src < 0 && !m->sw.no_co_split_f16;
                    if (s16) sz.in_amax = m->layers[i - 1].bound_fwd;
                    for (size_t j = 0; j < ly.fwd_co.size(); ++j) {
                        View oj = ly.out;
                        oj.c0 = ly.out.c0 + (int)j * ly.fwd_co_w;
                        oj.C = ly.fwd_co_w;
                        bool f1 = false;
                        ALQ_TRY(gemm_launch(ctx, ly.fwd_co[j], in, oj, ly.d_bias + j * ly.fwd_co_w, ly.spec.relu, 0, N, PROF_IGEMM_FWD, s16 ? &sz : nullptr, &f1));
                    }
                    fused = false;
                    ly.signs_ready = false;
                    break;
                }
                const bool sg_here = with_sums && fuse && !m->sw.no_signs && ly.spec.relu && ly.out.sg && gemm_route(ly.fwd[0], in, ly.out, 0, fuse) == ROUTE_IGEMM4;
                if (sg_here) fz.sign_out = ly.out.sg;
                {
                    Igemm2Fuse hz;
                    const Igemm2Fuse *fu = fuse;
                    if (v3f16 && !ly.fwd[0].p4.ok && !ly.fwd[0].pd.ok && !ly.fwd[0].pfc.ok && ly.fwd[0].p3.ok && ly.fwd[0].p3.d_W16 && ly.fwd[0].p2.a.PT == 1 &&
                        in.split == 0 && ly.spec.skip_src < 0) {
                        if (fuse) hz = *fuse;
                        hz.in_amax = i == 0 ? m->in_amax : m->layers[i - 1].bound_fwd;
                        hz.in_amax2 = nullptr;
                        fu = &hz;
                    }
                    bool f2 = false;
                    ALQ_TRY(gemm_launch(ctx, ly.fwd[0], in, ly.out, ly.d_bias, ly.spec.relu, 0, N, PROF_IGEMM_FWD, fu, &f2));
                    fused = fuse ? f2 : false;
                }
                ly.signs_ready = sg_here;
                if (fuse && prod[i]) ALQ_TRY(k_rowmax_u32(ctx, m->amax_tiles, ly.fwd[0].p4.a.tpg * 4, N, ly.amax_fwd));
                break;
            }
            case ALQ_CONVT: {
                if (t3d_fwd_applies(m, i, prod, cons, with_sums, drop)) {
                    const bool want_amax = prod[i] != 0;
                    ALQ_TRY(t3d_fwd_launch(ctx, ly.t3f, in, ly.out, ly.d_bias, N, with_sums ? ly.osum : nullptr, want_amax ? m->amax_tiles : nullptr));
                    if (want_amax) ALQ_TRY(k_rowmax_u32(ctx, m->amax_tiles, 16, N, ly.amax_fwd));
                    ly.signs_ready = false;
                    fused = true;
                    m->last.fwd.t3f += 1;
                    break;
                }
                if (ly.fwd_all.ok && two_slot_allowed()) {
                    const bool want_amax = fuse && prod[i];
                    if (fuse) take_amax(fz, i);
                    if (want_amax) fz.out_amax = m->amax_tiles;
                    const bool sg_here = with_sums && fuse && !m->sw.no_signs && ly.spec.relu && ly.out.sg;
                    if (sg_here) fz.sign_out = ly.out.sg;
                    ALQ_TRY(igemm4_launch(ctx, ly.fwd_all, in, ly.out, ly.d_bias, ly.spec.relu, 0, N, PROF_IGEMM3_FWD, fuse));
                    ly.signs_ready = sg_here;
                    if (want_amax)
                        ALQ_TRY(k_rowmax_u32(ctx, m->amax_tiles, ly.fwd_all.a.tpg * (ly.fwd_all.multi ? ly.fwd_all.a.ngr : 1) * 4, N, ly.amax_fwd));
                    fused = fuse != nullptr;
                    break;
                }
                bool all = true;
                for (auto &p : ly.fwd) {
                    bool f1 = false;
                    ALQ_TRY(gemm_launch(ctx, p, in, ly.out, ly.d_bias, ly.spec.relu, 0, N, PROF_IGEMM_FWD, fuse, &f1));
                    all = all && f1;
                }
                fused = all;
                break;
            }
            case ALQ_POOL:
                ALQ_TRY(k_pool_fwd(ctx, in, ly.out, ly.argmax, ly.spec.k, ly.lo, N, with_sums ? ly.osum : nullptr, &fused));
                break;
            case ALQ_FC:
                if (with_sums) {
                    const bool prev_spatial = i > 0 && m->layers[i - 1].osum != nullptr;
                    if (c3_head) ALQ_TRY(k_rowsum_field(ctx, ly.c3_asum, 4, N, ly.asum));
                    else if (prev_spatial) ALQ_TRY(k_rowsum_field(ctx, m->layers[i - 1].osum, m->layers[i - 1].out.vox(), N, ly.asum));
                    else ALQ_TRY(k_chansum(ctx, flat_view(in), ly.asum, N));
                }
                if (ly.dense_fc_small && fc_head_fused) {
                    ALQ_TRY(k_fc_small_finish_diff(ctx, c3_head ? ly.c3_part : ly.fc_part2, c3_head ? 4 : ly.fc_slices2, ly.d_bias, N, ly.out.p));
                } else if (ly.dense_fc_small) {
                    ALQ_TRY(k_fc_small_fwd(ctx, in.p, ly.F, ly.d_Wp, ly.spec.cout, N, ly.fc_partials, ly.fc_slices,
                                           with_sums ? ly.fc_maskbits : nullptr));
                    ALQ_TRY(k_fc_small_finish(ctx, ly.fc_partials, ly.fc_slices, ly.d_bias, ly.spec.cout,
                                              ly.spec.relu, N, ly.out.p));
                } else {
                    ALQ_TRY(gemm_launch(ctx, ly.fwd[0], flat_view(in), ly.out, ly.d_bias, ly.spec.relu, 0, N,
                                        PROF_IGEMM_FWD));
                }
                break;
        }
        if (drop && drop->on(i)) {
            ALQ_REQUIRE(keep_all && !with_sums, ALQ_EINVAL, "dropout only in passes that keep every activation");
            ALQ_TRY(k_dropout(ctx, ly.spec.type == ALQ_FC ? flat_view(ly.out) : ly.out, N, drop->first_sample, drop->seed, i, drop->keep_prob));
        }
        if (with_sums && ly.osum && !fused) ALQ_TRY(k_chansum(ctx, ly.out, ly.osum, N));
        if (with_sums && i == 0 && ly.pidx == 0 && ly.spec.type != ALQ_FC && in.C > 1)
            ALQ_TRY(k_chansum(ctx, in, ly.asum, N));
    }
    return ALQ_OK;
}

struct SideStream {
    alq_ctx *c;
    hipStream_t main;
    bool on = false;
    explicit SideStream(alq_ctx *ctx) : c(ctx), main(ctx->stream) {
        if (!c->side || c->side_off) return;
        if (hipEventRecord(c->ev_fork, main) != hipSuccess || hipStreamWaitEvent(c->side, c->ev_fork, 0) != hipSuccess) {
            (void)hipGetLastError();
            return;
        }
        c->stream = c->side;
        c->side_used = true;
        on = true;
    }
    ~SideStream() { if (on) c->stream = main; }
    SideStream(const SideStream &) = delete;
    SideStream &operator=(const SideStream &) = delete;
};

static int side_join(alq_ctx *c) {
    if (!c->side || !c->side_used) return ALQ_OK;
    c->side_used = false;
    ALQ_HIP(hipEventRecord(c->ev_join, c->side));
    ALQ_HIP(hipStreamWaitEvent(c->stream, c->ev_join, 0));
    return ALQ_OK;
}


static bool pool_first_ok(const Layer &pl, const Layer &src) {
    return pl.spec.type == ALQ_POOL && src.pidx == 0 && src.spec.type != ALQ_FC && pl.spec.k[1] == 2 && pl.spec.k[2] == 2 &&
           (pl.spec.k[0] == 1 || pl.spec.k[0] == 2) && pl.lo[0] == 0 && pl.lo[1] == 0 && pl.lo[2] == 0 &&
           src.out.D == pl.out.D * pl.spec.k[0] && src.out.H == pl.out.H * 2 && src.out.W == pl.out.W * 2 &&
           (pl.out.C == 4 || pl.out.C == 8 || pl.out.C == 16) && ((pl.dout.cs | pl.dout.c0 | pl.out.cs | pl.out.c0) & 3) == 0 &&
           src.spec.relu && !g_dbg_knobs[KNOB_NO_POOL_FIRST];
}

static bool e3d_bwd_applies(const alq_model *m, int i, bool prev_is_src) {
    const Layer &ly = m->layers[i];
    if (!(ly.spec.type == ALQ_POOL && i >= 3 && !m->sw.no_e3d && two_slot_allowed() && !g_no_f16x2 && !m->sw.no_bound16 && !m->sw.no_signs &&
          !g_dbg_knobs[KNOB_NO_BWD_FUSE] && !g_dbg_knobs[KNOB_NO_POOL_FIRST]))
        return false;
    const Layer &cv = m->layers[i - 1], &p1 = m->layers[i - 2], &c0 = m->layers[i - 3];
    return cv.spec.type == ALQ_CONV && cv.e3b.ok && cv.e3b.d_Whi && cv.spec.relu && cv.signs_ready && cv.out.sg && prev_is_src &&
           p1.spec.type == ALQ_POOL && pool_first_ok(p1, c0) && c0.dsum_partial && p1.signs_ready && p1.out.sg && p1.spec.k[0] == 2 &&
           ly.spec.k[0] == 2 && ly.spec.k[1] == 2 && ly.spec.k[2] == 2 && ly.lo[0] == 0 && ly.lo[1] == 0 && ly.lo[2] == 0 &&
           ly.dout.D == 8 && ly.dout.H == 8 && ly.dout.W == 8 && ly.dout.C == 16 && ly.dout.cs == 16 && ly.dout.c0 == 0 && !ly.dout.split &&
           cv.dout.cs == 16 && cv.dout.c0 == 0 && !cv.dout.split && cv.out.cs == 16 && cv.out.c0 == 0 && p1.out.cs == 8 && p1.out.c0 == 0 &&
           p1.out.C == 8 && c0.out.D == 32 && cv.dout_bound > 0.f && cv.dsum && c0.dsum;
}

static bool head_bits_apply(const alq_model *m, int i, bool prev_param, bool prev_is_src) {
    const Layer &ly = m->layers[i];
    const Layer *prev = i > 0 ? &m->layers[i - 1] : nullptr;
    return ly.dense_fc_small && ly.fc_maskbits && prev_param && prev->out.cs == prev->out.C &&
           prev->out.c0 == 0 && two_slot_allowed() && prev->bwd.p4.ok && prev->bwd.p4.NTW == 1 && !prev->bwd.p4.multi &&
           prev->bwd.p4.a.PT == 1 && !prev->dout.split && !prev_is_src &&
           !(i >= 2 && m->layers[i - 2].out_is_skip_src && prev->spec.skip_src < 0);
}

static bool c3d_bwd_applies(const alq_model *m, const Layer &ly, const unsigned short *vec16c, const Igemm2Fuse *fuse, int acc) {
    return ly.c3b.ok && ly.c3b.d_W && vec16c && !m->sw.no_c3d && !g_no_f16x2 && fuse && !acc && fuse->in_vec_amax > 0.f &&
           fuse->split == 8 && fuse->store_from == 8 && fuse->mask_bits && fuse->mask_from == 0 && fuse->mask_to == 8 && fuse->osumA && fuse->osumB &&
           ly.din.split == 8 && ly.din.cs == 8 && ly.din.C == 16;
}

static bool t3d_bwd_applies(const alq_model *m, const Layer &ly, const Igemm2Fuse *fuse, int acc, bool hand, bool prev_param) {
    return ly.spec.type == ALQ_CONVT && ly.t3b.ok && ly.t3b.d_W && !m->sw.no_t3d && two_slot_allowed() && !g_no_f16x2 && !acc && fuse && !hand &&
           fuse->in_bound > 0.f && !fuse->in_amax && fuse->split == 0 && fuse->store_from == 0 && fuse->osumA && !fuse->osumB && fuse->mask_from == 0 &&
           (!fuse->mask || fuse->mask_bits) && !ly.dout.split && !ly.din.split && prev_param;
}

static bool d3d_bwd_applies(const alq_model *m, const Layer &ly, const Igemm2Fuse *fuse, int acc, bool hand) {
    return ly.spec.type == ALQ_CONV && ly.d3f.ok && ly.d3f.d_Bhi && !m->sw.no_d3d && !m->sw.no_d3b && two_slot_allowed() && !g_no_f16x2 && !acc && fuse && !hand &&
           fuse->in_bound > 0.f && !fuse->in_amax && fuse->split == 16 && fuse->store_from == 0 && !fuse->mask && !fuse->osumA && fuse->osumB &&
           !ly.dout.split && ly.dout.cs == 16 && ly.dout.c0 == 0 && ly.din.split == 16 && ly.din.cs == 16 && ly.din.c0 == 0 && ly.din.C == 32;
}

static int run_backward_main(alq_model *m, const float *d_x, int N);
static int run_backward(alq_model *m, const float *d_x, int N) {
    const int rc = run_backward_main(m, d_x, N);
    const int rj = side_join(m->ctx);
    return rc != ALQ_OK ? rc : rj;
}

static int run_backward_main(alq_model *m, const float *d_x, int N) {
    alq_ctx *ctx = m->ctx;
    const int nl = (int)m->layers.size();
    ALQ_REQUIRE(m->nclass == 2, ALQ_EUNSUPPORTED, "Fisher scoring is binary (PW_NNAL.py:766), got %d classes", m->nclass);
    ALQ_TRY(k_fill_unit_cotangent(ctx, m->dlogits, N));
    for (Layer &l : m->layers) { l.delta_ready = false; l.dsum_partial = false; l.dout_bits = nullptr; l.dout_vec = nullptr; l.dout_vec16 = nullptr; l.dout_vec16c = nullptr; l.dout_amax = nullptr; }
    m->last.bwd = {};
    {
        for (Layer &l : m->layers) l.dout_bound = 0.f;
        m->layers[nl - 1].dout_bound = 1.f;
        for (int i = nl - 1; i >= 1; --i) {
            const Layer &ly = m->layers[i];
            double inb = ly.dout_bound;
            if (ly.spec.type == ALQ_FC)
                inb = (ly.spec.cout == 2 && ly.fc_wv_amax > 0.f && i == nl - 1) ? (double)ly.fc_wv_amax : (i < nl - 1 ? ly.bwd_l1 * ly.dout_bound : 0.0);
            else if (ly.spec.type != ALQ_POOL) inb = ly.bwd_l1 * ly.dout_bound;
            if (!(inb > 0.0) || ly.dout_bound <= 0.f) inb = 0.0;
            auto add = [&](Layer &p) { p.dout_bound = (p.dout_bound < 0.f || inb <= 0.0) ? -1.f : p.dout_bound + (float)(inb * (1.0 + 1e-6)); };
            add(m->layers[i - 1]);
            if (ly.spec.skip_src >= 0) add(m->layers[ly.spec.skip_src]);
        }
    }
    int e3_conv = -1;
    for (int i = nl - 1; i >= 0; --i) {
        Layer &ly = m->layers[i];
        const bool prev_is_src = (i > 0 && m->layers[i - 1].out_is_skip_src && ly.spec.skip_src < 0);
        if (e3d_bwd_applies(m, i, prev_is_src)) {
            Layer &cv = m->layers[i - 1], &p1 = m->layers[i - 2], &c0 = m->layers[i - 3];
            ALQ_TRY(e3d_bwd_launch(ctx, cv.e3b, N, cv.dout.p, ly.dout.p, ly.argmax, cv.out.sg, p1.argmax, p1.out.sg, cv.dsum, c0.dsum, cv.dout_bound, m->sw.e3d_rows != 0));
            m->last.bwd.e3b_form = m->sw.e3d_rows ? 1 : 2;
            cv.delta_ready = true;
            c0.delta_ready = true;
            e3_conv = i - 1;
            m->last.bwd.e3b = 1;
            continue;
        }
        if (e3_conv >= 0 && i == e3_conv - 1) continue;
        Layer *prev = i > 0 ? &m->layers[i - 1] : nullptr;
        const bool prev_param = prev && prev->pidx >= 0 && prev->spec.type != ALQ_FC;
        if (ly.spec.type == ALQ_POOL && prev_param && pool_first_ok(ly, *prev) && (prev->dsum_partial || !prev_is_src)) {
            ALQ_TRY(k_pool_bwd_first(ctx, ly.dout, ly.out, ly.argmax, ly.spec.k, prev->out.D, prev->out.H, prev->out.W, N,
                                     prev->dsum, prev->dsum_partial ? 1 : 0, ly.signs_ready ? 1 : 0));
            prev->delta_ready = true;
            continue;
        }
        if (ly.spec.type == ALQ_POOL) {
            bool fused = false;
            ALQ_TRY(k_pool_bwd(ctx, ly.dout, ly.din, ly.argmax, ly.spec.k, ly.lo, N, prev_is_src ? 1 : 0,
                               (prev_param && prev->spec.relu) ? &prev->out : nullptr, prev_param ? prev->dsum : nullptr,
                               &fused, !(prev_param && prev->pidx == 0),
                               (prev_param && prev->signs_ready) ? 1 : 0));
            if (prev_param && fused) prev->delta_ready = true;
            continue;
        }
        const bool isfc = ly.spec.type == ALQ_FC;
        if (!ly.delta_ready) {
            View dv = isfc ? flat_view(ly.dout) : ly.dout;
            View av = isfc ? flat_view(ly.out) : ly.out;
            ALQ_TRY(k_mask_chansum(ctx, dv, ly.spec.relu ? &av : nullptr, ly.dsum, N));
        }
        const float *as1 = ly.asum, *as2 = nullptr;
        if (!isfc) {
            if (i == 0) as1 = ly.in.C == 1 ? d_x : ly.asum;
            else as1 = m->layers[i - 1].osum;
            if (ly.spec.skip_src >= 0) as2 = m->layers[ly.spec.skip_src].osum;
        }
        double *Sdst = m->Spart + (size_t)ly.pidx * m->max_batch * m->nslab_max;
        {
            SideStream beside(ctx);
            if (ly.spec.type == ALQ_CONVT) {
                ALQ_TRY(k_boxdot_convT(ctx, ly.dsum, as1, as2, ly.in.D, ly.in.H, ly.in.W, ly.spec.k, ly.spec.s, ly.lo, N, Sdst, m->nslab_max));
            } else if (isfc) {
                const int one[3] = {1, 1, 1}, zero[3] = {0, 0, 0};
                ALQ_TRY(k_boxdot_conv(ctx, ly.dsum, ly.asum, nullptr, 1, 1, 1, one, zero, N, Sdst, m->nslab_max));
            } else {
                ALQ_TRY(k_boxdot_conv(ctx, ly.dsum, as1, as2, ly.out.D, ly.out.H, ly.out.W, ly.spec.k, ly.lo, N, Sdst, m->nslab_max));
            }
        }
        if (ly.pidx == 0) break;
        if (i == e3_conv) continue;
        const int acc = prev_is_src ? 1 : 0;
        bool fused = false;
        if (isfc) {
            ALQ_REQUIRE(!acc, ALQ_EUNSUPPORTED, "layer %d: fc consumer of a skip source", i);
            if (head_bits_apply(m, i, prev_param, prev_is_src)) {
                {
                    SideStream beside(ctx);
                    ALQ_TRY(k_fc_small_dsum_bits(ctx, ly.fc_maskbits, ly.fc_wv, ly.F, N, prev->dsum));
                }
                prev->dout_bits = ly.fc_maskbits;
                prev->dout_vec = ly.fc_wv;
                prev->dout_vec16 = ly.fc_wv16;
                prev->dout_vec16c = ly.fc_wv16c;
                prev->dout_vec_amax = ly.spec.cout == 2 ? ly.fc_wv_amax : 0.f;
                fused = true;
            } else if (ly.dense_fc_small) {
                const bool can = prev_param && prev->out.cs == prev->out.C;
                ALQ_TRY(k_fc_small_bwd(ctx, ly.dout.p, ly.spec.cout, ly.d_Wp, ly.F, N, ly.din.p,
                                       (can && prev->spec.relu) ? prev->out.p : nullptr, can ? prev->dsum : nullptr,
                                       can ? prev->out.C : 0, &fused));
            } else {
                ALQ_TRY(gemm_launch(ctx, ly.bwd, ly.dout, flat_view(ly.din), nullptr, 0, 0, N, PROF_IGEMM_BWD, nullptr, nullptr,
                                    (ly.dout_bound > 0.f && !m->sw.no_bound16) ? ly.dout_bound : 0.f));
            }
        } else {
            Igemm2Fuse fz;
            const Igemm2Fuse *fuse = nullptr;
            if (prev_param && !g_dbg_knobs[KNOB_NO_BWD_FUSE]) {
                const int Cs = ly.spec.skip_src >= 0 ? m->layers[ly.spec.skip_src].out.C : 0;
                if (prev->spec.relu) {
                    fz.mask = prev->out.p; fz.mask_cs = prev->out.cs; fz.mask_c0 = prev->out.c0; fz.mask_from = Cs;
                    if (prev->signs_ready) fz.mask_bits = prev->out.sg;
                }
                if (Cs > 0) { fz.split = Cs; fz.osumB = prev->dsum; } else { fz.osumA = prev->dsum; }
                if (Cs > 0 && (two_slot_allowed() || ly.din.split) && ly.bwd.p4.ok) {
                    Layer &sl = m->layers[ly.spec.skip_src];
                    const bool next_pool = ly.spec.skip_src + 1 < nl && pool_first_ok(m->layers[ly.spec.skip_src + 1], sl);
                    const bool sliced = sl.out.p == prev->out.p && sl.out.cs == prev->out.cs && prev->out.c0 == sl.out.c0 + Cs;
                    const bool splitv = ly.in.split == Cs && sl.out.p == ly.in.p;
                    if (next_pool && (sliced || splitv) && (Cs & 3) == 0) {
                        fz.mask = sl.out.p; fz.mask_cs = sl.out.cs; fz.mask_c0 = sl.out.c0; fz.mask_from = 0;
                        fz.mask_bits = (sl.signs_ready && (!prev->spec.relu || prev->signs_ready)) ? sl.out.sg : nullptr;
                        if (splitv) { fz.mask_split = Cs; fz.mask_delta = ly.in.delta; }
                        if (!prev->spec.relu) fz.mask_to = Cs;
                        fz.osumA = sl.dsum; fz.store_from = Cs;
                        sl.dsum_partial = true;
                    }
                }
                fuse = &fz;
            }
            if (ly.dout_bits) {
                fz.in_bits = ly.dout_bits; fz.in_vec = ly.dout_vec; fz.in_vec_amax = ly.dout_vec_amax;
                fz.in_vec16 = m->sw.no_presplit ? nullptr : ly.dout_vec16;
                const unsigned short *vec16c = ly.dout_vec16c;
                ly.dout_bits = nullptr; ly.dout_vec = nullptr; ly.dout_vec16 = nullptr; ly.dout_vec16c = nullptr;
                const bool honoured = fuse != nullptr;
                const bool c3 = c3d_bwd_applies(m, ly, vec16c, fuse, acc);
                m->last.bwd.c3_bwd = c3;
                if (c3) {
                    int ex = 0;
                    (void)std::frexp(fz.in_vec_amax, &ex);
                    ALQ_TRY(c3d_bwd_launch(ctx, ly.c3b, N, reinterpret_cast<const unsigned char *>(fz.in_bits), vec16c, 14 - ex, fz.mask_bits,
                                           ly.din.p + ly.din.delta, fz.osumA, fz.osumB, m->sw.c3_bwd_rows));
                } else {
                    ALQ_TRY(igemm4_launch(ctx, ly.bwd.p4, ly.dout, ly.din, nullptr, 0, acc, N, PROF_IGEMM3_BWD, &fz));
                }
                fused = honoured;
            } else {
                const bool p4_here = fuse && two_slot_allowed() && ly.bwd.p4.ok && !ly.bwd.p4.multi && ly.bwd.p4.a.PT == 1 && !g_no_f16x2;
                bool hand = false;
                if (p4_here && prev_param && !acc && !(prev->dout_bound > 0.f && !m->sw.no_bound16) && prev->pidx > 0 && prev->bwd.p4.ok && !prev->bwd.p4.multi && prev->bwd.p4.a.PT == 1 &&
                    prev->bwd.p4.d_W16 && !prev->dout.split &&
                    ((prev->bwd.p4.NTW == 1 && prev->bwd.p4.fic) || prev->bwd.p4.NTW == 2)) {
                    const size_t len = (size_t)ly.bwd.p4.a.tpg * 4;
                    if (!m->amax_a) { ALQ_TRY(m->dalloc(&m->amax_a, (size_t)m->max_batch)); ALQ_TRY(m->dalloc(&m->amax_b, (size_t)m->max_batch)); }
                    ALQ_TRY(ensure_amax_tiles(m, len));
                    fz.out_amax = m->amax_tiles;
                    fz.amax_from = fz.split > 0 && fz.split < (1 << 29) ? fz.split : 0;
                    hand = true;
                }
                if (p4_here && !acc && ly.dout_amax) fz.in_amax = ly.dout_amax;
                if (p4_here && !acc && !fz.in_amax && ly.dout_bound > 0.f && !m->sw.no_bound16) fz.in_bound = ly.dout_bound;
                if (!fuse && !acc && two_slot_allowed() && ly.bwd.p4.ok && !ly.bwd.p4.multi && ly.bwd.p4.a.PT == 1 && !g_no_f16x2 && !ly.dout_amax &&
                    ly.dout_bound > 0.f && !m->sw.no_bound16 && !g_dbg_knobs[KNOB_NO_BWD_FUSE]) {
                    fz = Igemm2Fuse();
                    fz.in_bound = ly.dout_bound;
                    fuse = &fz;
                }
                if (!ly.bwd.p4.ok && ly.bwd.p3.ok && ly.bwd.p3.d_W16 && !acc && !g_no_f16x2 && ly.dout_bound > 0.f && !m->sw.no_bound16 && !g_dbg_knobs[KNOB_NO_BWD_FUSE] &&
                    two_slot_allowed() && !ly.bwd.pd.ok && !ly.bwd.pfc.ok) {
                    if (!fuse) { fz = Igemm2Fuse(); fuse = &fz; }
                    fz.in_bound = ly.dout_bound;
                }
                const unsigned *mine = ly.dout_amax;
                ly.dout_amax = nullptr;
                if (t3d_bwd_applies(m, ly, fuse, acc, hand, prev_param)) {
                    ALQ_TRY(t3d_bwd_launch(ctx, ly.t3b, ly.dout, ly.din, N, fz.in_bound, fz.mask ? fz.mask_bits : nullptr, fz.osumA));
                    fused = true;
                    m->last.bwd.t3b += 1;
                } else if (d3d_bwd_applies(m, ly, fuse, acc, hand)) {
                    ALQ_TRY(d3d_bwd_launch(ctx, ly.d3f, N, ly.dout.p, fz.in_bound, ly.din.p, ly.din.p + ly.din.delta, fz.osumB));
                    fused = true;
                    m->last.bwd.d3b = 1;
                } else
                ALQ_TRY(gemm_launch(ctx, ly.bwd, ly.dout, ly.din, nullptr, 0, acc, N, PROF_IGEMM_BWD, fuse, &fused));
                if (hand) {
                    unsigned *dst = mine == m->amax_a ? m->amax_b : m->amax_a;
                    ALQ_TRY(k_rowmax_u32(ctx, m->amax_tiles, ly.bwd.p4.a.tpg * 4, N, dst));
                    prev->dout_amax = dst;
                }
            }
        }
        if (prev_param && fused) prev->delta_ready = true;
    }
    return ALQ_OK;
}

int make_drop(const alq_model *m, float keep_prob, uint64_t seed, int64_t first_sample, const int32_t *h_layers, int n_layers,
              DropSpec *d) {
    ALQ_REQUIRE(keep_prob > 0.f && keep_prob <= 1.f, ALQ_EINVAL, "keep_prob %g outside (0, 1]", (double)keep_prob);
    ALQ_REQUIRE(n_layers == 0 || h_layers, ALQ_EINVAL, "dropout layer list missing");
    d->keep_prob = keep_prob; d->seed = seed; d->first_sample = first_sample; d->layers = 0;
    for (int i = 0; i < n_layers; ++i) {
        ALQ_REQUIRE(h_layers[i] >= 0 && h_layers[i] < (int)m->layers.size() && h_layers[i] < 64, ALQ_EINVAL, "dropout layer %d", h_layers[i]);
        d->layers |= 1ull << h_layers[i];
    }
    return ALQ_OK;
}

extern "C" {

int alq_model_out_voxels(const alq_model *m) { return m ? (int)m->V : ALQ_EINVAL; }

int alq_model_set_aleatoric(alq_model *m, int on) {
    ALQ_REQUIRE(m, ALQ_EINVAL, "alq_model_set_aleatoric: null model");
    ALQ_REQUIRE(m->dense && m->nclass >= 3, ALQ_EUNSUPPORTED,
                "alq_model_set_aleatoric: a log-variance channel needs a 1x1 conv head of 3 .. 8 channels (2 .. 7 classes beside it)");
    if (on && !m->au) {
        ALQ_HIP(hipSetDevice(m->ctx->device));
        ALQ_TRY(m->dalloc(&m->au, (size_t)m->max_batch * m->V));
    }
    m->aleatoric = on != 0;
    return ALQ_OK;
}

int alq_forward_au(alq_model *m, const float *d_x, int N, float keep_prob, uint64_t seed, int64_t first_sample,
                   const int32_t *h_drop_layers, int n_drop_layers, float *d_post, int64_t *d_pred, float *d_au, float *d_logits) {
    ALQ_REQUIRE(m && d_x && d_au, ALQ_EINVAL, "alq_forward_au: null argument");
    ALQ_REQUIRE(m->aleatoric, ALQ_EUNSUPPORTED, "alq_forward_au: the model has no log-variance channel (alq_model_set_aleatoric)");
    ALQ_REQUIRE(N >= 0 && N <= m->max_batch, ALQ_EINVAL, "alq_forward_au: N=%d exceeds max_batch=%d", N, m->max_batch);
    if (N == 0) return ALQ_OK;
    ALQ_HIP(hipSetDevice(m->ctx->device));
    DropSpec ds;
    ALQ_TRY(make_drop(m, keep_prob, seed, first_sample, h_drop_layers, n_drop_layers, &ds));
    ALQ_TRY(prepare_call(m, false));
    ALQ_TRY(run_forward(m, d_x, N, false, true, &ds));
    return dense_forward_head(m, d_x, N, d_post, d_pred, false, d_au, d_logits);
}

int alq_forward_dropout(alq_model *m, const float *d_x, int N, float keep_prob, uint64_t seed, int64_t first_sample,
                        const int32_t *h_drop_layers, int n_drop_layers, float *d_post, int64_t *d_pred) {
    ALQ_REQUIRE(m && d_x, ALQ_EINVAL, "alq_forward_dropout: null argument");
    ALQ_REQUIRE(N >= 0 && N <= m->max_batch, ALQ_EINVAL, "alq_forward_dropout: N=%d exceeds max_batch=%d", N, m->max_batch);
    if (N == 0) return ALQ_OK;
    ALQ_HIP(hipSetDevice(m->ctx->device));
    DropSpec ds;
    ALQ_TRY(make_drop(m, keep_prob, seed, first_sample, h_drop_layers, n_drop_layers, &ds));
    ALQ_TRY(prepare_call(m, false));
    ALQ_TRY(run_forward(m, d_x, N, false, true, &ds));
    if (m->dense) return dense_forward_head(m, d_x, N, d_post, d_pred, false);
    ALQ_TRY(k_softmax(m->ctx, m->logits, m->nclass, N, d_post ? d_post : m->post, d_pred));
    return ALQ_OK;
}

int alq_model_create(alq_ctx *ctx, const alq_layer_t *layers, int n_layers, const int32_t in_dims[4],
                     int max_batch, alq_model **out) {
    ALQ_REQUIRE(ctx && layers && in_dims && out, ALQ_EINVAL, "alq_model_create: null argument");
    ALQ_REQUIRE(n_layers >= 1 && n_layers <= 64 && max_batch >= 1, ALQ_EINVAL, "alq_model_create: bad sizes");
    ALQ_HIP(hipSetDevice(ctx->device));
    alq_model *m = new alq_model();
    m->ctx = ctx;
    m->max_batch = max_batch;
    m->sw = read_engine_switches();
    for (int i = 0; i < 4; ++i) m->in_dims[i] = in_dims[i];
    m->epp = (int64_t)in_dims[0] * in_dims[1] * in_dims[2] * in_dims[3];
    const int rc = build_model(m, layers, n_layers);
    if (rc != ALQ_OK) {
        alq_model_destroy(m);
        return rc;
    }
    if (const char *t = getenv("ALQ_G4_TUNE")) {
        std::string all(t);
        size_t pos = 0;
        while (pos < all.size()) {
            size_t end = all.find(';', pos);
            if (end == std::string::npos) end = all.size();
            const std::string item = all.substr(pos, end - pos);
            pos = end + 1;
            if (item.size() < 3 || (item[0] != 'f' && item[0] != 'b')) continue;
            const size_t colon = item.find(':');
            if (colon == std::string::npos) continue;
            const int li = atoi(item.substr(1, colon - 1).c_str());
            if (li < 0 || li >= (int)m->layers.size()) continue;
            Layer &ly = m->layers[li];
            Igemm4Plan *pl = item[0] == 'b' ? &ly.bwd.p4 : (ly.spec.type == ALQ_CONVT ? &ly.fwd_all : (ly.fwd.empty() ? nullptr : &ly.fwd[0].p4));
            if (!pl) continue;
            const size_t fi = item.find("fic="), ei = item.find("epi=");
            if (fi != std::string::npos) pl->tune_fic = atoi(item.c_str() + fi + 4);
            if (ei != std::string::npos) pl->tune_epi = atoi(item.c_str() + ei + 4);
        }
    }
    {
        const int nl = (int)m->layers.size();
        if (nl >= 4 && nl <= 16 && m->layers[nl - 1].fc_part2 && m->layers[nl - 2].spec.type == ALQ_CONV &&
            m->layers[nl - 3].spec.type == ALQ_CONVT && !m->layers[nl - 3].spec.relu && m->layers[nl - 4].spec.type == ALQ_CONV &&
            m->layers[nl - 4].spec.relu)
            m->f16_fwd_derived = 1 << (nl - 4);
        for (int i = 1; i + 1 < nl; ++i)
            if (m->layers[i].f3f.ok && m->f16_fwd_derived) m->f16_fwd_derived |= 1 << i;
        if (m->sw.has_f16_derived_mask) m->f16_fwd_derived = m->sw.f16_derived_mask;
    }
    *out = m;
    return ALQ_OK;
}

int alq_model_destroy(alq_model *m) {
    if (!m) return ALQ_OK;
    (void)hipStreamSynchronize(m->ctx->stream);
    for (void *p : m->allocs) (void)hipFree(p);
    delete m;
    return ALQ_OK;
}

int alq_model_num_param_layers(const alq_model *m) { return m ? m->L : ALQ_EINVAL; }
int alq_model_max_batch(const alq_model *m) { return m ? m->max_batch : ALQ_EINVAL; }

int alq_model_layer_out_elems(const alq_model *m, int layer_idx, int64_t *elems) {
    ALQ_REQUIRE(m && elems && layer_idx >= 0 && layer_idx < (int)m->layers.size(), ALQ_EINVAL, "bad layer index");
    *elems = m->layers[layer_idx].out.elems();
    return ALQ_OK;
}

int alq_forward(alq_model *m, const float *d_x, int N, float *d_post, int64_t *d_pred, float *d_feat,
                int feature_layer_idx) {
    ALQ_REQUIRE(m && d_x, ALQ_EINVAL, "alq_forward: null argument");
    ALQ_REQUIRE(N >= 0 && N <= m->max_batch, ALQ_EINVAL, "alq_forward: N=%d exceeds max_batch=%d", N, m->max_batch);
    if (N == 0) return ALQ_OK;
    ALQ_HIP(hipSetDevice(m->ctx->device));
    ALQ_TRY(prepare_call(m, false));
    ALQ_TRY(run_forward(m, d_x, N, false, d_feat != nullptr));
    if (m->dense) ALQ_TRY(dense_forward_head(m, d_x, N, d_post, d_pred, d_feat && feature_layer_idx == (int)m->layers.size() - 1));
    else ALQ_TRY(k_softmax(m->ctx, m->logits, m->nclass, N, d_post ? d_post : m->post, d_pred));
    if (d_feat) {
        ALQ_REQUIRE(feature_layer_idx >= 0 && feature_layer_idx < (int)m->layers.size(), ALQ_EINVAL, "bad feature layer");
        const View &v = m->layers[feature_layer_idx].out;
        ALQ_REQUIRE(v.cs == v.C, ALQ_EUNSUPPORTED, "feature layer is a concat slice");
        ALQ_HIP(hipMemcpyAsync(d_feat, v.p, (size_t)N * v.elems() * sizeof(float), hipMemcpyDeviceToDevice, m->ctx->stream));
    }
    return ALQ_OK;
}

int alq_fisher(alq_model *m, const float *d_x, int N, const float *d_p1_in, double diag_load, float *d_p1_out,
               double *d_g0, double *d_g1, double *d_A, double *d_trace, double *d_Asum) {
    ALQ_REFUSE_DENSE(m, "alq_fisher");
    ALQ_REQUIRE(m && d_x, ALQ_EINVAL, "alq_fisher: null argument");
    ALQ_REQUIRE(N >= 0 && N <= m->max_batch, ALQ_EINVAL, "alq_fisher: N=%d exceeds max_batch=%d", N, m->max_batch);
    ALQ_HIP(hipSetDevice(m->ctx->device));
    if (N == 0) {
        if (d_Asum) ALQ_HIP(hipMemsetAsync(d_Asum, 0, sizeof(double) * m->L * m->L, m->ctx->stream));
        return ALQ_OK;
    }
    struct SkipGuard {
        alq_ctx *c;
        explicit SkipGuard(alq_ctx *ctx) : c(ctx) { c->prof_skip = c->prof_on && (c->prof_pass++ % c->prof_every) != 0; }
        ~SkipGuard() { c->prof_skip = false; }
    } guard(m->ctx);
    ALQ_TRY(prepare_call(m, true));
    ALQ_TRY(run_forward(m, d_x, N, true));
    ALQ_TRY(k_softmax(m->ctx, m->logits, m->nclass, N, m->post, nullptr));
    ALQ_TRY(run_backward(m, d_x, N));
    int nblocks = 0;
    ALQ_TRY(k_fisher_finalize(m->ctx, m->Spart, m->nslab, m->nslab_max, m->max_batch, m->S, m->L, m->sizes, m->post,
                              d_p1_in, N, diag_load, d_p1_out, d_g0, d_g1, d_A, d_trace, m->Apart, &nblocks));
    if (d_Asum) ALQ_TRY(k_reduce_Asum(m->ctx, m->Apart, nblocks, m->L * m->L, d_Asum));
    return ALQ_OK;
}

static int stage_rows(alq_model *m, const float *d_pool, const int64_t *d_rows, int N) {
    ALQ_REQUIRE(d_pool && d_rows, ALQ_EINVAL, "null pool / row list");
    if (!m->x_stage) ALQ_TRY(m->dalloc(&m->x_stage, (size_t)m->max_batch * m->epp));
    return gather_rows_impl(m->ctx, d_pool, d_rows, N, m->epp, m->x_stage);
}

int alq_forward_rows(alq_model *m, const float *d_pool, const int64_t *d_rows, int N, float *d_post, int64_t *d_pred,
                     float *d_feat, int feature_layer_idx) {
    ALQ_REFUSE_DENSE(m, "alq_forward_rows");
    ALQ_REQUIRE(m != nullptr, ALQ_EINVAL, "alq_forward_rows: null model");
    ALQ_REQUIRE(N >= 0 && N <= m->max_batch, ALQ_EINVAL, "alq_forward_rows: N=%d exceeds max_batch=%d", N, m->max_batch);
    if (N == 0) return ALQ_OK;
    ALQ_HIP(hipSetDevice(m->ctx->device));
    ALQ_TRY(stage_rows(m, d_pool, d_rows, N));
    return alq_forward(m, m->x_stage, N, d_post, d_pred, d_feat, feature_layer_idx);
}

int alq_fisher_rows(alq_model *m, const float *d_pool, const int64_t *d_rows, int N, const float *d_p1_in, double diag_load,
                    float *d_p1_out, double *d_g0, double *d_g1, double *d_A, double *d_trace, double *d_Asum) {
    ALQ_REFUSE_DENSE(m, "alq_fisher_rows");
    ALQ_REQUIRE(m != nullptr, ALQ_EINVAL, "alq_fisher_rows: null model");
    ALQ_REQUIRE(N >= 0 && N <= m->max_batch, ALQ_EINVAL, "alq_fisher_rows: N=%d exceeds max_batch=%d", N, m->max_batch);
    ALQ_HIP(hipSetDevice(m->ctx->device));
    if (N > 0) ALQ_TRY(stage_rows(m, d_pool, d_rows, N));
    return alq_fisher(m, N > 0 ? m->x_stage : d_pool, N, d_p1_in, diag_load, d_p1_out, d_g0, d_g1, d_A, d_trace, d_Asum);
}

int alq_model_debug_copy(alq_model *m, int layer_idx, int what, int N, float *d_out, int64_t *elems_out) {
    ALQ_REQUIRE(m && d_out && N >= 1 && N <= m->max_batch, ALQ_EINVAL, "alq_model_debug_copy: bad argument");
    ALQ_HIP(hipSetDevice(m->ctx->device));
    if (what == 4) {
        if (elems_out) *elems_out = (int64_t)N * m->L;
        return debug_f64_copy(m->ctx, m->S, (long long)N * m->L, d_out);
    }
    if (what == 5) {
        const Layer &head = m->layers.back();
        ALQ_REQUIRE(head.fc_part2 && m->last.fwd.head_fused, ALQ_EUNSUPPORTED, "the last pass did not run the fused fc head");
        const int ns = m->last.fwd.c3 ? 4 : head.fc_slices2;
        if (elems_out) *elems_out = (int64_t)N * ns;
        ALQ_HIP(hipMemcpyAsync(d_out, m->last.fwd.c3 ? head.c3_part : head.fc_part2, (size_t)N * ns * sizeof(float), hipMemcpyDeviceToDevice,
                               m->ctx->stream));
        return ALQ_OK;
    }
    ALQ_REQUIRE(layer_idx >= 0 && layer_idx < (int)m->layers.size(), ALQ_EINVAL, "bad layer index");
    const Layer &ly = m->layers[layer_idx];
    if (what >= 6 && what <= 10) {
        ALQ_REQUIRE(ly.spec.type == ALQ_FC && ly.fwd.size() == 1 && ly.fwd[0].pfc.ok && ly.weights_set, ALQ_EUNSUPPORTED, "layer %d has no streaming-GEMM weights", layer_idx);
        if (what == 10) {
            int32_t wd[4] = {ly.fwd[0].pfc.w_exp, ly.bwd.pfc.w_exp, 0, 0};
            std::memcpy(&wd[2], &ly.bwd_l1, 8);
            if (elems_out) *elems_out = 4;
            ALQ_HIP(hipMemcpyAsync(d_out, wd, 16, hipMemcpyHostToDevice, m->ctx->stream));
            ALQ_HIP(hipStreamSynchronize(m->ctx->stream));
            return ALQ_OK;
        }
        const FcGemmPlan &pl = what <= 7 ? ly.fwd[0].pfc : ly.bwd.pfc;
        const void *src = (what & 1) ? pl.d_W16 : pl.d_W;
        ALQ_REQUIRE(pl.ok && src, ALQ_EUNSUPPORTED, "layer %d: this form is not packed", layer_idx);
        const int64_t e = (int64_t)pl.K * pl.N * ((what & 1) ? 2 : 3) / 2;
        if (elems_out) *elems_out = e;
        ALQ_HIP(hipMemcpyAsync(d_out, src, (size_t)e * 4, hipMemcpyDeviceToDevice, m->ctx->stream));
        return ALQ_OK;
    }
    if (what >= 11 && what <= 13) {
        if (what == 11) {
            ALQ_REQUIRE(ly.osum && m->last.call_fisher, ALQ_EUNSUPPORTED, "layer %d: no channel sums of its output in the last pass", layer_idx);
            if (elems_out) *elems_out = (int64_t)N * ly.out.vox();
            ALQ_HIP(hipMemcpyAsync(d_out, ly.osum, (size_t)N * ly.out.vox() * sizeof(float), hipMemcpyDeviceToDevice, m->ctx->stream));
            return ALQ_OK;
        }
        if (what == 12) {
            const View &v = ly.out;
            ALQ_REQUIRE(v.sg && ly.signs_ready && ((v.C | v.cs | v.c0) & 3) == 0 && ((int64_t)N * v.vox() * v.cs) % 16 == 0, ALQ_EUNSUPPORTED,
                        "layer %d: no sign field of its output in the last pass", layer_idx);
            if (elems_out) *elems_out = (int64_t)N * v.vox() * v.cs / 16;
            ALQ_HIP(hipMemcpyAsync(d_out, v.sg, (size_t)N * v.vox() * v.cs / 4, hipMemcpyDeviceToDevice, m->ctx->stream));
            return ALQ_OK;
        }
        ALQ_REQUIRE(ly.spec.type == ALQ_POOL && ly.argmax && ((int64_t)N * ly.out.vox() * ly.out.C) % 4 == 0, ALQ_EUNSUPPORTED, "layer %d has no arg-max field", layer_idx);
        if (elems_out) *elems_out = (int64_t)N * ly.out.vox() * ly.out.C / 4;
        ALQ_HIP(hipMemcpyAsync(d_out, ly.argmax, (size_t)N * ly.out.vox() * ly.out.C, hipMemcpyDeviceToDevice, m->ctx->stream));
        return ALQ_OK;
    }
    if (what == 0 || what == 1) {
        const Layer &head = m->layers.back();
        ALQ_REQUIRE(!(layer_idx + 2 == (int)m->layers.size() && head.spec.type == ALQ_FC &&
                      (what == 0 ? m->last.fwd.head_fused
                                 : (m->last.call_fisher && head.fc_maskbits != nullptr && two_slot_allowed()))),
                    ALQ_EUNSUPPORTED, "layer %d: this tensor is not materialised in a Fisher pass (fc head fused into the layer: "
                    "create the model under ALQ_NO_FC_BITS=1 to keep it)", layer_idx);
        const View &v = what == 0 ? ly.out : ly.dout;
        if (elems_out) *elems_out = (int64_t)N * v.elems();
        return debug_view_copy(m->ctx, v, N, d_out);
    }
    ALQ_REQUIRE(ly.pidx >= 0 && !ly.dense_head && (what == 2 || what == 3), ALQ_EINVAL, "layer has no channel-sum fields");
    const bool isfc = ly.spec.type == ALQ_FC;
    const int64_t e = (int64_t)N * (isfc ? 1 : (what == 2 ? ly.in.vox() : ly.out.vox()));
    if (elems_out) *elems_out = e;
    ALQ_HIP(hipMemcpyAsync(d_out, what == 2 ? ly.asum : ly.dsum, e * sizeof(float), hipMemcpyDeviceToDevice,
                           m->ctx->stream));
    return ALQ_OK;
}

int alq_model_engine_info(alq_model *m, int what) {
    ALQ_REQUIRE(m, ALQ_EINVAL, "alq_model_engine_info: bad argument");
    switch (what) {
        case ALQ_INFO_SUBNORMALS_OK:
            ALQ_HIP(hipSetDevice(m->ctx->device));
            return c3d_subnormals_ok(m->ctx);
        case ALQ_INFO_C3D_FWD: return m->last.fwd.c3 ? 1 : 0;
        case ALQ_INFO_C3D_BWD: return m->last.bwd.c3_bwd ? 1 : 0;
        case ALQ_INFO_C3D_ONE_ACC:
            for (const Layer &ly : m->layers)
                if (ly.c3f.ok) return ly.c3f.oneacc;
            return 0;
        case ALQ_INFO_FLIP_OVERFLOW: {
            ALQ_HIP(hipSetDevice(m->ctx->device));
            if (!m->flip_overflow) return 0;
            unsigned h = 0;
            ALQ_HIP(hipMemcpyAsync(&h, m->flip_overflow, sizeof(unsigned), hipMemcpyDeviceToHost, m->ctx->stream));
            ALQ_HIP(hipStreamSynchronize(m->ctx->stream));
            return h > 0x7fffffffu ? 0x7fffffff : (int)h;
        }
        case ALQ_INFO_F16_DERIVED: return m->last.fwd.f16_derived ? 1 : 0;
        case ALQ_INFO_T3D_FWD: return m->last.fwd.t3f;
        case ALQ_INFO_T3D_BWD: return m->last.bwd.t3b;
        case ALQ_INFO_E3D_BWD: return m->last.bwd.e3b;
        case ALQ_INFO_D3D_FWD: return m->last.fwd.d3f;
        case ALQ_INFO_D3D_BWD: return m->last.bwd.d3b;
        case ALQ_INFO_F3D_FWD: return m->last.fwd.f3f;
        case ALQ_INFO_C3D_BWD_FORM: return m->last.bwd.c3_bwd ? m->sw.c3_bwd_rows : 0;
        case ALQ_INFO_HOST_PACK_ELEMS: return m->host_pack_elems > 0x7fffffffll ? 0x7fffffff : (int)m->host_pack_elems;
        case ALQ_INFO_LSUM: return m->last.lsum;
        case ALQ_INFO_DCP_FORM: return m->last.fwd.dcp;
        case ALQ_INFO_E3D_BWD_FORM: return m->last.bwd.e3b_form;
        default: break;
    }
    set_error("alq_model_engine_info: bad argument");
    return ALQ_EINVAL;
}

int alq_debug_set(int key, int value) {
    ALQ_REQUIRE(key >= 0 && key < ALQ_NKNOBS, ALQ_EINVAL, "alq_debug_set: bad key");
    g_knob_override[key] = value > 0 ? value : -1;
    g_dbg_knobs[key] = value;
    return ALQ_OK;
}

int alq_debug_set_stamp_buffer(void *d_buf) {
    g_igemm2_dbg = reinterpret_cast<unsigned long long *>(d_buf);
    return ALQ_OK;
}

}
```

nn-active-learning_amd/csrc/model_types.h:

```cpp
#pragma once
#include <algorithm>

#include "alq_internal.h"

namespace alq {

struct Layer {
    alq_layer_t spec;
    int pidx = -1;
    View in, out;
    View din, dout;
    int lo[3] = {0, 0, 0};
    bool dense_fc_small = false;
    bool dense_head = false;
    int64_t F = 0;
    int64_t w_elems = 0, b_elems = 0;
    float *d_bias = nullptr;
    float *d_Wp = nullptr;
    std::vector<Gemm> fwd;
    std::vector<Gemm> fwd_co;
    int fwd_co_w = 0;
    Igemm4Plan fwd_all;
    Gemm bwd;
    bool has_bwd = false;
    bool weights_set = false;
    float *d_Wres = nullptr;
    bool fallback_stale = false;
    uint8_t *argmax = nullptr;
    float *asum = nullptr, *dsum = nullptr;
    double *ls_field = nullptr;
    float *osum = nullptr;
    bool delta_ready = false;
    bool signs_ready = false;
    bool dsum_partial = false;
    float *fc_partials = nullptr;
    unsigned *fc_maskbits = nullptr;
    float *fc_wv = nullptr;
    unsigned *fc_wv16 = nullptr;
    float fc_wv_amax = 0.f;
    const unsigned *dout_amax = nullptr;
    unsigned *amax_fwd = nullptr;
    float dout_vec_amax = 0.f;
    double bwd_l1 = 0;
    float dout_bound = 0.f;
    float *d_W32 = nullptr;
    float fwd_l1 = 0.f;
    float out_l1 = 0.f, out_bmax = 0.f;
    unsigned *bound_fwd = nullptr;
    float *fc_part2 = nullptr;
    int fc_slices2 = 0;
    C3dPlan c3f, c3b;
    D3dPlan d3f;
    F3dPlan f3f;
    E3dPlan e3b;
    T3dPlan t3f, t3b;
    float *c3_part = nullptr, *c3_asum = nullptr;
    unsigned short *fc_wv16c = nullptr;
    const unsigned short *dout_vec16c = nullptr;
    const unsigned *dout_bits = nullptr;
    const float *dout_vec = nullptr;
    const unsigned *dout_vec16 = nullptr;
    int fc_slices = 0;
    bool out_is_skip_src = false;
    std::vector<std::vector<int>> class_taps;
    std::vector<float> hv_hW;
    int hv_src = 0;
    bool hv_stale = false;
    float *hv_W = nullptr;
    double *hv_A = nullptr, *hv_D = nullptr, *hv_Ra = nullptr, *hv_Rd = nullptr;
};

}

struct PassInfo {
    struct Fwd {
        bool head_fused = false;
        bool c3 = false;
        int t3f = 0;
        int d3f = 0;
        int f3f = 0;
        int dcp = 0;
        bool f16_derived = false;
    } fwd;
    struct Bwd {
        bool c3_bwd = false;
        int t3b = 0;
        int e3b = 0;
        int e3b_form = 0;
        int d3b = 0;
    } bwd;
    int lsum = 0;
    bool call_fisher = false;
};

struct alq_model {
    alq_ctx *ctx = nullptr;
    int max_batch = 0;
    alq::EngineSwitches sw;
    PassInfo last;
    unsigned *amax_a = nullptr, *amax_b = nullptr, *amax_tiles = nullptr;
    unsigned *flip_cnt = nullptr, *flip_list = nullptr;
    int flip_cap = 0;
    unsigned *bound_all = nullptr;
    unsigned *in_amax = nullptr;
    bool v3_fwd_f16 = false;
    unsigned *flip_overflow = nullptr;
    size_t amax_tiles_len = 0;
    int in_dims[4] = {1, 1, 1, 1};
    int nclass = 0;
    bool dense = false;
    int64_t V = 1;
    bool aleatoric = false;
    float *au = nullptr;
    double *dh_part = nullptr;
    int L = 0;
    std::vector<alq::Layer> layers;
    std::vector<void *> allocs;
    float *logits = nullptr, *dlogits = nullptr, *post = nullptr;
    double *S = nullptr, *sizes = nullptr, *Apart = nullptr;
    double *Spart = nullptr;
    int *nslab = nullptr;
    int nslab_max = 1;
    float *wg_partial = nullptr;
    size_t wg_partial_len = 0;
    double *gn_partial = nullptr;
    size_t gn_partial_len = 0;
    double *df_scratch = nullptr;
    double *ls_part = nullptr;
    std::vector<int> ls_nslab;
    int ls_nslab_max = 0;
    float *x_stage = nullptr;
    int64_t epp = 0;
    int f16_fwd_derived = 0;
    int64_t host_pack_elems = 0;
    void *d_wscal = nullptr;
    bool hv_ready = false;
    double *hv_part = nullptr;
    double *hv_p64 = nullptr;

    template <typename T>
    int dalloc(T **p, size_t count) {
        void *q = nullptr;
        const size_t bytes = std::max<size_t>(count * sizeof(T), 256);
        if (hipMalloc(&q, bytes) != hipSuccess) {
            alq::set_error("hipMalloc of %zu bytes failed", bytes);
            return ALQ_ENOMEM;
        }
        allocs.push_back(q);
        *p = reinterpret_cast<T *>(q);
        return ALQ_OK;
    }
};

template <typename T, typename D>
int ensure(alq_model *m, D **d, size_t count) {
    T *p = static_cast<T *>(*d);
    if (!p) ALQ_TRY(m->dalloc(&p, count));
    *d = p;
    return ALQ_OK;
}

template <typename T, typename D>
int upload(alq_model *m, D **d, const std::vector<T> &h) {
    ALQ_TRY(ensure<T>(m, d, h.size()));
    ALQ_HIP(hipMemcpyAsync(*d, h.data(), h.size() * sizeof(T), hipMemcpyHostToDevice, m->ctx->stream));
    return ALQ_OK;
}

template <typename T, typename D>
int upload_release(alq_model *m, D **d, std::vector<T> *h) {
    ALQ_TRY(upload(m, d, *h));
    ALQ_HIP(hipStreamSynchronize(m->ctx->stream));
    std::vector<T>().swap(*h);
    return ALQ_OK;
}

namespace alq { int refresh_fallback_forms(alq_model *m); }

struct DropSpec {
    unsigned long long layers = 0;
    float keep_prob = 1.f;
    unsigned long long seed = 0;
    long long first_sample = 0;
    bool on(int i) const { return keep_prob < 1.f && i < 64 && ((layers >> i) & 1ull); }
};
int make_drop(const alq_model *m, float keep_prob, uint64_t seed, int64_t first_sample, const int32_t *h_layers, int n_layers, DropSpec *d);
int prepare_call(alq_model *m, bool fisher);
int run_forward(alq_model *m, const float *d_x, int N, bool with_sums, bool keep_all = false, const DropSpec *drop = nullptr);
int gemm_launch(alq_ctx *ctx, const alq::Gemm &g, const alq::View &in, const alq::View &out, const float *bias, int relu, int accumulate, int N,
                int cls, const alq::Igemm2Fuse *fuse = nullptr, bool *fused = nullptr, float fc_in_bound = 0.f);
alq::View flat_view(const alq::View &v);

int dense_forward_head(alq_model *m, const float *d_x, int N, float *d_post, int64_t *d_pred, bool want_logits, float *d_au = nullptr,
                       float *d_logits = nullptr);
#define ALQ_REFUSE_ALEATORIC(m, who)                                                                                           \
    ALQ_REQUIRE(!(m) || !(m)->aleatoric, ALQ_EUNSUPPORTED,                                                                      \
                "%s: the model's head has a log-variance channel (alq_model_set_aleatoric): alq_param_grads_loss_mt_au", who)
#define ALQ_REFUSE_DENSE(m, who)                                                                                                \
    ALQ_REQUIRE(!(m) || !(m)->dense, ALQ_EUNSUPPORTED, "%s: not defined for a fully-convolutional model (1x1 conv head)", who)
```

nn-active-learning_amd/csrc/sweep_common.h:

```cpp
#ifndef ALQ_SWEEP_COMMON_H
#define ALQ_SWEEP_COMMON_H
#include "alq_internal.h"

#include <algorithm>

namespace alq {

typedef float f32x4 __attribute__((ext_vector_type(4)));
typedef float f32x2 __attribute__((ext_vector_type(2)));
typedef int i32x4 __attribute__((ext_vector_type(4)));
typedef int i32x2 __attribute__((ext_vector_type(2)));
typedef __bf16 bf16x2 __attribute__((ext_vector_type(2)));
typedef __bf16 bf16x8 __attribute__((ext_vector_type(8)));
typedef _Float16 f16x8 __attribute__((ext_vector_type(8)));
typedef _Float16 f16x2 __attribute__((ext_vector_type(2)));

__device__ inline __amdgpu_buffer_rsrc_t sw_rsrc(const void *base, unsigned long long bytes) {
    return __builtin_amdgcn_make_buffer_rsrc(const_cast<void *>(base), 0, (int)(unsigned)bytes, 0x00020000);
}
constexpr unsigned SW_OOB = 0xffffff00u;

__device__ inline int sw_s(unsigned v) { return __builtin_amdgcn_readfirstlane((int)v); }

template <int V> struct IC { static constexpr int value = V; };

constexpr int SW_FILL_MASK = 0x096;

__device__ inline int sw_patch_exp(unsigned fm) {
    const int ex = (int)((fm >> 23) & 255u) - 126;
    const int ce = 14 - ex;
    return fm ? (ce < 96 ? ce : 96) : 0;
}

#define SW_XCD_DEAL(N)                                                                                         \
    const int G8 = (int)gridDim.x >> 3, xcd = (int)blockIdx.x & 7, jb = (int)blockIdx.x >> 3;                  \
    const int npx = (N) > xcd ? ((N) - xcd + 7) >> 3 : 0
#define SW_PATCH_ORDER(N)                                                                                      \
    SW_XCD_DEAL(N);                                                                                            \
    const int npw = npx > jb ? (npx - jb + G8 - 1) / G8 : 0;                                                   \
    auto patch_of = [&](int i) __attribute__((always_inline)) { return 8 * (jb + (i < npw ? i : npw - 1) * G8) + xcd; }

inline unsigned sweep_grid(const alq_ctx *ctx, long long items, int per_cu) {
    const long long g = std::min<long long>((long long)per_cu * ctx->num_cus, items);
    return (unsigned)std::max<long long>(8, (g + 7) / 8 * 8);
}

inline bool is_conv3_same(const int k[3], const int lo[3], const int s[3]) {
    return k[0] == 3 && k[1] == 3 && k[2] == 3 && s[0] == 1 && s[1] == 1 && s[2] == 1 && lo[0] == 1 && lo[1] == 1 && lo[2] == 1;
}

#define SWEEP_REQUIRE_PATCHES(N, name) ALQ_REQUIRE((N) < 4096, ALQ_EUNSUPPORTED, name ": 32-bit byte offsets hold fewer than 4096 patches per pass")

template <typename K, typename A>
inline int sweep_launch(alq_ctx *ctx, K kernel, unsigned grid, unsigned block, size_t lds, const A &args) {
    ALQ_HIP(hipFuncSetAttribute(reinterpret_cast<const void *>(kernel), hipFuncAttributeMaxDynamicSharedMemorySize, (int)lds));
    hipLaunchKernelGGL(kernel, dim3(grid), dim3(block), lds, ctx->stream, args);
    ALQ_HIP(hipGetLastError());
    return ALQ_OK;
}

}

#endif
```

nn-active-learning_amd/csrc/t3d.hip:

```cpp
#include "f16_pair.h"
#include "sweep_common.h"
#ifndef T3_CLOBBER
#define T3_CLOBBER : "memory"
#endif

#include <algorithm>
#include <cmath>
#include <cstdlib>
#include <cstring>
#include <vector>

namespace alq {

struct T3FwdArgs {
    const float *in;
    float *out;
    const unsigned short *W;
    const float *bias;
    float *osum;
    unsigned *out_amax;
    int N;
};
struct T3BwdArgs {
    const float *dout;
    float *din;
    const unsigned short *W;
    const unsigned char *mask_bits;
    float *dsum;
    float inv;
    float scale;
    int N;
};

constexpr int T3F_ROWB = 17 * 32, T3F_WAVE = 2 * 3 * T3F_ROWB;
constexpr int T3B_ROWB = 34 * 16, T3B_WAVE = 6 * 2 * T3B_ROWB;

__device__ inline unsigned t3_split2(float &a, float &b) {
    const bf16x2 h = __builtin_convertvector(f32x2{a, b}, bf16x2);
    const unsigned hb = __builtin_bit_cast(unsigned, h);
    a -= __builtin_bit_cast(float, hb << 16);
    b -= __builtin_bit_cast(float, hb & 0xffff0000u);
    return hb;
}
__device__ inline unsigned t3_pack2(float a, float b) {
    return __builtin_amdgcn_perm(__builtin_bit_cast(unsigned, b), __builtin_bit_cast(unsigned, a), 0x07060302u);
}

struct T3Cur { int p, iz, s; bool ok; };
__device__ inline T3Cur t3_tile(int T, int total, int wave) {
    const int G8 = (int)gridDim.x >> 3, x = (int)blockIdx.x & 7, j = (int)blockIdx.x >> 3;
    const int v = j + (T >> 4) * G8;
    T3Cur c;
    c.p = 8 * (v >> 2) + x;
    c.iz = 4 * (v & 3) + wave;
    c.s = T & 15;
    c.ok = T < total;
    return c;
}
__device__ inline int t3_total_tiles(int N) {
    const int G8 = (int)gridDim.x >> 3, x = (int)blockIdx.x & 7, j = (int)blockIdx.x >> 3;
    const int np = N > x ? (N - x + 7) >> 3 : 0;
    const int nv = 4 * np;
    return nv > j ? 16 * ((nv - j + G8 - 1) / G8) : 0;
}

constexpr int T3F_PF = 4;
template <bool SUMS, bool AMAX>
__global__ __launch_bounds__(256, 2) void t3d_fwd_kernel(const T3FwdArgs a) {
    extern __shared__ __attribute__((aligned(16))) char t3lds[];
    const int lane = threadIdx.x & 63, wave = __builtin_amdgcn_readfirstlane((int)(threadIdx.x >> 6));
    char *strip = t3lds + wave * T3F_WAVE;
    if (lane < 12) {
        const int r = lane >> 1;
        *reinterpret_cast<i32x4 *>(strip + r * T3F_ROWB + (lane & 1) * 16) = i32x4{0, 0, 0, 0};
    }
    const int n = lane & 15, kg = lane >> 4;
    const int w_off = ((lane >> 2) + 1) * 32 + (lane & 3) * 8;
    const int f_off = (n + 1 - (kg >> 1)) * 32 + (kg & 1) * 16;
    bf16x8 wr[9][3];
#pragma unroll
    for (int c = 0; c < 9; ++c)
#pragma unroll
        for (int pc = 0; pc < 3; ++pc)
            wr[c][pc] = *reinterpret_cast<const bf16x8 *>(a.W + ((size_t)(c * 3 + pc) * 64 + lane) * 8);
    f32x4 bias4 = *reinterpret_cast<const f32x4 *>(a.bias + 4 * (kg & 1));
#pragma unroll
    for (int c = 0; c < 9; ++c)
#pragma unroll
        for (int pc = 0; pc < 3; ++pc) asm volatile("" : "+v"(wr[c][pc]));
    asm volatile("" : "+v"(bias4));
    const __amdgpu_buffer_rsrc_t in_rsrc = sw_rsrc(a.in, (unsigned long long)a.N * 16 * 16 * 16 * 16 * 4);
    const __amdgpu_buffer_rsrc_t out_rsrc = sw_rsrc(a.out, (unsigned long long)a.N * 32 * 32 * 32 * 8 * 4);
    const __amdgpu_buffer_rsrc_t sum_rsrc = sw_rsrc(a.osum, SUMS ? (unsigned long long)a.N * 32 * 32 * 32 * 4 : 0ull);
    const unsigned ld_off = (unsigned)lane * 16u;
    const unsigned st_off = (unsigned)(2 * n + (kg >> 1)) * 32u + (unsigned)(kg & 1) * 16u;
    const unsigned sm_off = (kg & 1) ? SW_OOB : (unsigned)(2 * n + (kg >> 1)) * 4u;
    const int total = t3_total_tiles(a.N);

    f32x4 R0[T3F_PF], R1[T3F_PF];
    auto fetch = [&](int T, f32x4 &r0, f32x4 &r1) __attribute__((always_inline)) {
        const T3Cur c = t3_tile(T, total, wave);
        const unsigned row0 = ((unsigned)(c.p * 16 + c.iz) * 16u + (unsigned)c.s) * 1024u;
        r0 = __builtin_bit_cast(f32x4, __builtin_amdgcn_raw_buffer_load_b128(in_rsrc, (int)(c.ok ? ld_off : SW_OOB), (int)row0, 0));
        r1 = __builtin_bit_cast(f32x4, __builtin_amdgcn_raw_buffer_load_b128(in_rsrc, (int)((c.ok && c.iz > 0) ? ld_off : SW_OOB), (int)(row0 - 16u * 1024u), 0));
    };
#pragma unroll
    for (int k = 0; k < T3F_PF; ++k) { R0[k] = f32x4{0.f, 0.f, 0.f, 0.f}; R1[k] = f32x4{0.f, 0.f, 0.f, 0.f}; }

    bf16x8 fo[2][3];
#pragma unroll
    for (int d = 0; d < 2; ++d)
#pragma unroll
        for (int pc = 0; pc < 3; ++pc) fo[d][pc] = bf16x8{0, 0, 0, 0, 0, 0, 0, 0};
    float amx = 0.f;
    const __amdgpu_buffer_rsrc_t amx_rsrc = sw_rsrc(a.out_amax, AMAX ? (unsigned long long)a.N * 16 * 4 : 0ull);
    static_assert(16 % T3F_PF == 0, "a sweep must start at k = 0");
    if (total > 0)
    for (int T0 = -T3F_PF; T0 < total; T0 += T3F_PF) {
        const bool live = T0 >= 0;
        const unsigned st_o = live ? st_off : SW_OOB, sm_o = live ? sm_off : SW_OOB;
#pragma unroll
        for (int k = 0; k < T3F_PF; ++k) {
            const int T = T0 + k;
            __builtin_amdgcn_sched_barrier(0);
            const T3Cur cur = t3_tile(live ? T : 0, total, wave);
            const int p = cur.p, iz = cur.iz, iy = cur.s;
            {
                auto split_row = [&](int base, const f32x4 &R) __attribute__((always_inline)) {
                    float x = R.x, y = R.y, z = R.z, w = R.w;
                    const unsigned h0 = t3_split2(x, y), h1 = t3_split2(z, w);
                    const unsigned m0 = t3_split2(x, y), m1 = t3_split2(z, w);
                    *reinterpret_cast<i32x2 *>(strip + (base + 0) * T3F_ROWB + w_off) = i32x2{(int)h0, (int)h1};
                    *reinterpret_cast<i32x2 *>(strip + (base + 1) * T3F_ROWB + w_off) = i32x2{(int)m0, (int)m1};
                    *reinterpret_cast<i32x2 *>(strip + (base + 2) * T3F_ROWB + w_off) = i32x2{(int)t3_pack2(x, y), (int)t3_pack2(z, w)};
                };
                split_row(0, R0[k]);
                split_row(3, R1[k]);
            }
            fetch(T + T3F_PF, R0[k], R1[k]);
            bf16x8 fn[2][3];
#pragma unroll
            for (int d = 0; d < 2; ++d)
#pragma unroll
                for (int pc = 0; pc < 3; ++pc)
                    fn[d][pc] = *reinterpret_cast<const bf16x8 *>(strip + (d * 3 + pc) * T3F_ROWB + f_off);
            if (k == 0) {
                const int keep = iy == 0 ? 0 : -1;
#pragma unroll
                for (int d = 0; d < 2; ++d)
#pragma unroll
                    for (int pc = 0; pc < 3; ++pc) {
                        i32x4 t = __builtin_bit_cast(i32x4, fo[d][pc]);
                        t.x &= keep; t.y &= keep; t.z &= keep; t.w &= keep;
                        fo[d][pc] = __builtin_bit_cast(bf16x8, t);
                    }
            }
            f32x4 acc[2][2];
#pragma unroll
            for (int i = 0; i < 2; ++i)
#pragma unroll
                for (int j = 0; j < 2; ++j) acc[i][j] = f32x4{0.f, 0.f, 0.f, 0.f};
#pragma unroll
            for (int cz = 0; cz < 3; ++cz)
#pragma unroll
                for (int cy = 0; cy < 3; ++cy) {
                    const int pz = cz == 2, dz = cz == 1, py = cy == 2, dy = cy == 1;
                    const bf16x8 *w = wr[cz * 3 + cy];
                    const bf16x8 *f = dy ? fo[dz] : fn[dz];
                    f32x4 c = acc[pz][py];
                    c = __builtin_amdgcn_mfma_f32_16x16x32_bf16(w[2], f[0], c, 0, 0, 0);
                    c = __builtin_amdgcn_mfma_f32_16x16x32_bf16(w[0], f[2], c, 0, 0, 0);
                    c = __builtin_amdgcn_mfma_f32_16x16x32_bf16(w[1], f[1], c, 0, 0, 0);
                    c = __builtin_amdgcn_mfma_f32_16x16x32_bf16(w[1], f[0], c, 0, 0, 0);
                    c = __builtin_amdgcn_mfma_f32_16x16x32_bf16(w[0], f[1], c, 0, 0, 0);
                    c = __builtin_amdgcn_mfma_f32_16x16x32_bf16(w[0], f[0], c, 0, 0, 0);
                    acc[pz][py] = c;
                }
#pragma unroll
            for (int d = 0; d < 2; ++d)
#pragma unroll
                for (int pc = 0; pc < 3; ++pc) fo[d][pc] = fn[d][pc];
            f32x4 vv[4];
#pragma unroll
            for (int i = 0; i < 4; ++i) {
                f32x4 v = acc[i >> 1][i & 1];
                v.x += bias4.x; v.y += bias4.y; v.z += bias4.z; v.w += bias4.w;
                vv[i] = v;
                if constexpr (AMAX)
                    amx = fmaxf(fmaxf(amx, fmaxf(__builtin_fabsf(v.x), __builtin_fabsf(v.y))), fmaxf(__builtin_fabsf(v.z), __builtin_fabsf(v.w)));
            }
#pragma unroll
            for (int i = 0; i < 4; ++i) {
                const int pz = i >> 1, py = i & 1;
                const f32x4 v = vv[i];
                const unsigned orow = ((unsigned)p * 32u + (unsigned)(2 * iz + pz)) * 32u + (unsigned)(2 * iy + py);
                __builtin_amdgcn_raw_buffer_store_b128(__builtin_bit_cast(i32x4, v), out_rsrc, (int)st_o, (int)(orow * 1024u), 0);
                if constexpr (SUMS) {
                    const float s = (v.x + v.y) + (v.z + v.w);
                    const float t = s + __shfl_xor(s, 16, 64);
// ... 477 lines not shown
```

Before: 283,700.

## Fuse dec1 conv forward with following transposed-conv upsample into one kernel

Adds a d3t kernel that computes the dec1 3x3x3 conv with fp16-pair MFMA and, in the same launch, splits its output into bf16 triples in LDS and runs the 2x transposed conv, writing the upsampled output directly. The intermediate dec1 activation is no longer written and re-read from global memory when it is not needed. Where a later pass needs it (backward masks, debug reads), a separate d3d launch materialises it. The fused kernel uses a large LDS footprint and one wave per EU, so occupancy is lower and the schedule is more complex.

```diff
diff --git a/include/alq.h b/include/alq.h
--- a/include/alq.h
+++ b/include/alq.h
@@ -270,7 +270,8 @@
     ALQ_INFO_HOST_PACK_ELEMS = 14,
     ALQ_INFO_LSUM = 15,
     ALQ_INFO_DCP_FORM = 16,
-    ALQ_INFO_E3D_BWD_FORM = 17
+    ALQ_INFO_E3D_BWD_FORM = 17,
+    ALQ_INFO_D3T_FWD = 19
 };
 int alq_model_engine_info(alq_model *m, int what);
 
diff --git a/nn-active-learning_amd/csrc/alq_internal.h b/nn-active-learning_amd/csrc/alq_internal.h
--- a/nn-active-learning_amd/csrc/alq_internal.h
+++ b/nn-active-learning_amd/csrc/alq_internal.h
@@ -430,6 +430,8 @@
 void d3d_pack(D3dPlan *plan, const float *W );
 int d3d_fwd_launch(alq_ctx *ctx, const D3dPlan &plan, int N, const float *inA, const float *inB, const unsigned *amaxA, const unsigned *amaxB,
                    const float *bias, int relu, float *out, unsigned char *sg, float *osum);
+int d3t_fwd_launch(alq_ctx *ctx, const D3dPlan &plan, const T3dPlan &up, int N, const float *inA, const float *inB, const unsigned *amaxA, const unsigned *amaxB,
+                   const float *bias, int relu, float *mid, unsigned char *sg, float *osum, const float *bias2, float *out, float *osum2, unsigned *out_amax);
 
 struct F3dPlan {
     bool ok = false;
diff --git a/nn-active-learning_amd/csrc/d3t.hip b/nn-active-learning_amd/csrc/d3t.hip
--- /dev/null
+++ b/nn-active-learning_amd/csrc/d3t.hip
@@ -0,0 +1,426 @@
+#include "f16_pair.h"
+#include "sweep_common.h"
+
+#include <algorithm>
+#include <cmath>
+#include <cstdlib>
+#include <cstring>
+
+namespace alq {
+
+struct D3TArgs {
+    const float *inA, *inB;
+    const unsigned *amaxA, *amaxB;
+    const unsigned short *Whi;
+    const unsigned short *Wlo;
+    const float *bias;
+    float *mid;
+    unsigned char *sg;
+    float *osum;
+    const unsigned short *W2;
+    const float *bias2;
+    float *out;
+    float *osum2;
+    unsigned *out_amax;
+    int e_w;
+    int relu;
+    int N;
+};
+
+constexpr int DT_KG = 18 * 16;
+constexpr int DT_ROWB = 4 * DT_KG;
+constexpr int DT_SLOT = 2 * DT_ROWB;
+constexpr int DT_PLANE = 18 * DT_SLOT;
+constexpr int DT_STRIP = 2 * DT_PLANE;
+constexpr int DT_UPIECE = 17 * 32;
+constexpr int DT_UROW = 3 * DT_UPIECE;
+constexpr int DT_UPLANE = 16 * DT_UROW;
+constexpr int DT_RING = DT_STRIP;
+constexpr int DT_W2 = DT_RING + 2 * DT_UPLANE;
+constexpr int DT_W2B = 9 * 3 * 64 * 16;
+constexpr int DT_AMX = DT_W2 + DT_W2B;
+constexpr int DT_B2 = DT_AMX + 32;
+constexpr int DT_LDS = DT_B2 + 32;
+static_assert(DT_LDS <= 163840, "LDS of a compute unit");
+
+#ifndef DT_PIPE
+#define DT_PIPE 2
+#endif
+
+struct DTRow { f32x4 a, b; };
+
+template <bool SUMS, bool STORE_MID>
+__global__ __launch_bounds__(256) __attribute__((amdgpu_waves_per_eu(1, 1))) void d3t_fwd_kernel(const D3TArgs a) {
+    extern __shared__ __attribute__((aligned(16))) char dtlds[];
+    const int lane = threadIdx.x & 63, wave = __builtin_amdgcn_readfirstlane((int)(threadIdx.x >> 6));
+    char *strip = dtlds;
+    for (int i = threadIdx.x; i < DT_W2 / 16; i += 256) reinterpret_cast<i32x4 *>(dtlds)[i] = i32x4{0, 0, 0, 0};
+    for (int i = threadIdx.x; i < DT_W2B / 16; i += 256)
+        reinterpret_cast<i32x4 *>(dtlds + DT_W2)[i] = reinterpret_cast<const i32x4 *>(a.W2)[i];
+    if (threadIdx.x < 8) {
+        reinterpret_cast<float *>(dtlds + DT_AMX)[threadIdx.x] = 0.f;
+        reinterpret_cast<float *>(dtlds + DT_B2)[threadIdx.x] = a.bias2[threadIdx.x];
+    }
+    __syncthreads();
+    const int n = lane & 15, kg = lane >> 4;
+    f16x8 wh[27], wl[27];
+#pragma unroll
+    for (int c = 0; c < 27; ++c) {
+        wh[c] = *reinterpret_cast<const f16x8 *>(a.Whi + ((size_t)c * 64 + lane) * 8);
+        wl[c] = *reinterpret_cast<const f16x8 *>(a.Wlo + ((size_t)c * 64 + lane) * 8);
+    }
+#pragma unroll
+    for (int c = 0; c < 27; ++c) asm volatile("" : "+a"(wh[c]), "+a"(wl[c]));
+    f32x4 bias4 = *reinterpret_cast<const f32x4 *>(a.bias + 4 * kg);
+    asm volatile("" : "+v"(bias4));
+    const float relu_floor = a.relu ? 0.f : -__builtin_inff();
+
+    typedef const unsigned __attribute__((address_space(4))) *cu32p;
+    const cu32p amaxA_c = (cu32p)(unsigned long long)a.amaxA, amaxB_c = (cu32p)(unsigned long long)a.amaxB;
+    auto patch_exp = [&](int p) __attribute__((always_inline)) {
+        const unsigned fa = amaxA_c[p], fb = amaxB_c[p];
+        return sw_patch_exp(fa > fb ? fa : fb);
+    };
+
+    const __amdgpu_buffer_rsrc_t ia_rsrc = sw_rsrc(a.inA, (unsigned long long)a.N * 4096 * 64);
+    const __amdgpu_buffer_rsrc_t ib_rsrc = sw_rsrc(a.inB, (unsigned long long)a.N * 4096 * 64);
+    const __amdgpu_buffer_rsrc_t o_rsrc = sw_rsrc(a.mid, STORE_MID ? (unsigned long long)a.N * 4096 * 64 : 0ull);
+    const __amdgpu_buffer_rsrc_t s_rsrc = sw_rsrc(a.sg, (SUMS && a.sg) ? (unsigned long long)a.N * 4096 * 4 : 0ull);
+    const __amdgpu_buffer_rsrc_t u_rsrc = sw_rsrc(a.osum, SUMS ? (unsigned long long)a.N * 4096 * 4 : 0ull);
+    const __amdgpu_buffer_rsrc_t o2_rsrc = sw_rsrc(a.out, (unsigned long long)a.N * 32 * 32 * 32 * 8 * 4);
+    const __amdgpu_buffer_rsrc_t u2_rsrc = sw_rsrc(a.osum2, SUMS ? (unsigned long long)a.N * 32 * 32 * 32 * 4 : 0ull);
+    const __amdgpu_buffer_rsrc_t amx_rsrc = sw_rsrc(a.out_amax, a.out_amax ? (unsigned long long)a.N * 16 * 4 : 0ull);
+
+    const int sx = lane >> 2, cq = lane & 3;
+    char *const w_base = strip + (4 * wave + 1) * DT_SLOT + (cq >> 1) * DT_KG + (sx + 1) * 16 + (cq & 1) * 8;
+    const unsigned ldA = (unsigned)lane * 16u;
+    const char *const f_base = strip + 4 * wave * DT_SLOT + kg * DT_KG + n * 16;
+    const unsigned e_out = (unsigned)n * 64u + (unsigned)kg * 16u, e_sg = (unsigned)n * 4u + (unsigned)kg;
+    const unsigned e_sum = kg == 0 ? (unsigned)n * 4u : SW_OOB;
+    float *const amx_lds = reinterpret_cast<float *>(dtlds + DT_AMX);
+
+    const bool flat = ((int)gridDim.x & 7) != 0;
+    const int G8 = flat ? (int)gridDim.x : (int)gridDim.x >> 3, xcd = flat ? 0 : (int)blockIdx.x & 7, jb = flat ? (int)blockIdx.x : (int)blockIdx.x >> 3;
+    const int pmul = flat ? 1 : 8;
+    const int npx = flat ? a.N : (a.N > xcd ? (a.N - xcd + 7) >> 3 : 0);
+    const int npw = npx > jb ? (npx - jb + G8 - 1) / G8 : 0;
+    auto patch_of = [&](int i) __attribute__((always_inline)) { return pmul * (jb + (i < npw ? i : npw - 1) * G8) + xcd; };
+
+    DTRow RA[4];
+    auto fetch = [&](int q) __attribute__((always_inline)) {
+        const unsigned row0 = ((unsigned)patch_of(q >> 4) * 16u + (unsigned)(q & 15)) * 16u + 4u * (unsigned)wave;
+#pragma unroll
+        for (int r = 0; r < 4; ++r) {
+            RA[r].a = __builtin_bit_cast(f32x4, __builtin_amdgcn_raw_buffer_load_b128(ia_rsrc, (int)ldA, sw_s((row0 + r) * 1024u), 0));
+            RA[r].b = __builtin_bit_cast(f32x4, __builtin_amdgcn_raw_buffer_load_b128(ib_rsrc, (int)ldA, sw_s((row0 + r) * 1024u), 0));
+        }
+    };
+    auto stage_unit = [&](auto U, int img, float sc, float sc11) __attribute__((always_inline)) {
+        constexpr int u = decltype(U)::value, r = u >> 1, h = u & 1;
+        char *dst = w_base + img * DT_PLANE + r * DT_SLOT + h * 2 * DT_KG;
+        const f32x4 g = h ? RA[r].b : RA[r].a;
+        const f16x2 h01 = __builtin_convertvector(f32x2{g.x * sc, g.y * sc}, f16x2), h23 = __builtin_convertvector(f32x2{g.z * sc, g.w * sc}, f16x2);
+        const f16x2 l01 = __builtin_convertvector(f32x2{__builtin_fmaf((float)h01.x, -2048.f, g.x * sc11), __builtin_fmaf((float)h01.y, -2048.f, g.y * sc11)}, f16x2);
+        const f16x2 l23 = __builtin_convertvector(f32x2{__builtin_fmaf((float)h23.x, -2048.f, g.z * sc11), __builtin_fmaf((float)h23.y, -2048.f, g.w * sc11)}, f16x2);
+        *reinterpret_cast<i32x2 *>(dst) = i32x2{__builtin_bit_cast(int, h01), __builtin_bit_cast(int, h23)};
+        *reinterpret_cast<i32x2 *>(dst + DT_ROWB) = i32x2{__builtin_bit_cast(int, l01), __builtin_bit_cast(int, l23)};
+    };
+
+    f32x4 acc[3][4], acx[3][4];
+#pragma unroll
+    for (int st = 0; st < 3; ++st)
+#pragma unroll
+        for (int ry = 0; ry < 4; ++ry) { acc[st][ry] = f32x4{0.f, 0.f, 0.f, 0.f}; acx[st][ry] = f32x4{0.f, 0.f, 0.f, 0.f}; }
+    f32x4 okeep[2];
+    okeep[0] = okeep[1] = f32x4{0.f, 0.f, 0.f, 0.f};
+
+    auto epi_row = [&](auto ST, auto RY, int p, int zo, bool tv, float inv) __attribute__((always_inline)) {
+        constexpr int st = decltype(ST)::value, ry = decltype(RY)::value;
+        const unsigned vrow = (unsigned)sw_s((((unsigned)p * 16u + (unsigned)(tv ? zo : 0)) * 16u + (unsigned)(4 * wave + ry)) * 16u);
+        const f32x4 c = acc[st][ry], cx = acx[st][ry];
+        const float v0 = __builtin_fmaxf(__builtin_fmaf(__builtin_fmaf(cx.x, 0x1p-11f, c.x), inv, bias4.x), relu_floor);
+        const float v1 = __builtin_fmaxf(__builtin_fmaf(__builtin_fmaf(cx.y, 0x1p-11f, c.y), inv, bias4.y), relu_floor);
+        const float v2 = __builtin_fmaxf(__builtin_fmaf(__builtin_fmaf(cx.z, 0x1p-11f, c.z), inv, bias4.z), relu_floor);
+        const float v3 = __builtin_fmaxf(__builtin_fmaf(__builtin_fmaf(cx.w, 0x1p-11f, c.w), inv, bias4.w), relu_floor);
+        if constexpr (STORE_MID) {
+            const f32x4 o = f32x4{v0, v1, v2, v3};
+            okeep[ry & 1] = o;
+            __builtin_amdgcn_raw_buffer_store_b128(__builtin_bit_cast(i32x4, o), o_rsrc, (int)(tv ? e_out : SW_OOB), (int)(vrow * 64u), 0);
+            ALQ_STORE_HOLD("v"(o));
+        }
+        if constexpr (SUMS) {
+            const unsigned bits = (v0 > 0.f ? 1u : 0u) | (v1 > 0.f ? 2u : 0u) | (v2 > 0.f ? 4u : 0u) | (v3 > 0.f ? 8u : 0u);
+            __builtin_amdgcn_raw_buffer_store_b8((unsigned char)bits, s_rsrc, (int)(tv ? e_sg : SW_OOB), (int)(vrow * 4u), 0);
+            float s_ = (v0 + v1) + (v2 + v3);
+            s_ += __shfl_xor(s_, 16, 64);
+            s_ += __shfl_xor(s_, 32, 64);
+            __builtin_amdgcn_raw_buffer_store_b32(__builtin_bit_cast(int, s_), u_rsrc, (int)(tv ? e_sum : SW_OOB), (int)(vrow * 4u), 0);
+        }
+        float x = v0, y = v1, z = v2, w = v3;
+        const unsigned h0 = t3_split2(x, y), h1 = t3_split2(z, w);
+        const unsigned m0 = t3_split2(x, y), m1 = t3_split2(z, w);
+        unsigned eo = e_out;
+        asm volatile("" : "+v"(eo));
+        char *d = dtlds + DT_RING + 32 + (4 * wave + ry) * DT_UROW + (zo & 1) * DT_UPLANE + (eo >> 1);
+        *reinterpret_cast<i32x2 *>(d) = i32x2{(int)h0, (int)h1};
+        *reinterpret_cast<i32x2 *>(d + DT_UPIECE) = i32x2{(int)m0, (int)m1};
+        *reinterpret_cast<i32x2 *>(d + 2 * DT_UPIECE) = i32x2{(int)t3_pack2(x, y), (int)t3_pack2(z, w)};
+    };
+
+    auto up2_plane = [&](int p, int iz) __attribute__((always_inline)) {
+        const int keepz = iz == 0 ? 0 : -1;
+        int ln = lane;
+        asm volatile("" : "+v"(ln));
+        const int un = ln & 15, ukg = ln >> 4;
+        const char *const uf_base = dtlds + DT_RING + 4 * wave * DT_UROW + (un + 1 - (ukg >> 1)) * 32 + (ukg & 1) * 16;
+        const char *const uw2 = dtlds + DT_W2 + ln * 16;
+        const unsigned st_off = (unsigned)(2 * un + (ukg >> 1)) * 32u + (unsigned)(ukg & 1) * 16u;
+        const unsigned sm_off = (ukg & 1) ? SW_OOB : (unsigned)(2 * un + (ukg >> 1)) * 4u;
+        const f32x4 bias2 = *reinterpret_cast<const f32x4 *>(dtlds + DT_B2 + (ukg & 1) * 16);
+        float amx = 0.f;
+        bf16x8 W[2][3], F0[3][3], F1[3][3];
+        auto wload = [&](int g, bf16x8 *w) __attribute__((always_inline)) {
+            const int cz = g < 3 ? 2 : (g < 6 ? 0 : 1), cy = g % 3;
+#pragma unroll
+            for (int pc = 0; pc < 3; ++pc) w[pc] = *reinterpret_cast<const bf16x8 *>(uw2 + ((cz * 3 + cy) * 3 + pc) * 1024);
+        };
+        auto fload = [&](int d, int h, bf16x8 (*F)[3]) __attribute__((always_inline)) {
+            const char *rb = uf_base + ((iz & 1) ^ d) * DT_UPLANE + (2 * h - 1) * DT_UROW;
+#pragma unroll
+            for (int rr = 0; rr < 3; ++rr)
+#pragma unroll
+                for (int pc = 0; pc < 3; ++pc) F[rr][pc] = *reinterpret_cast<const bf16x8 *>(rb + rr * DT_UROW + pc * DT_UPIECE);
+        };
+        auto fmask = [&](bf16x8 *f, int keep) __attribute__((always_inline)) {
+#pragma unroll
+            for (int pc = 0; pc < 3; ++pc) {
+                i32x4 t = __builtin_bit_cast(i32x4, f[pc]);
+                t.x &= keep; t.y &= keep; t.z &= keep; t.w &= keep;
+                f[pc] = __builtin_bit_cast(bf16x8, t);
+            }
+        };
+        auto finish = [&](f32x4 v, int h, int t, int pz, int py) __attribute__((always_inline)) {
+            v.x += bias2.x; v.y += bias2.y; v.z += bias2.z; v.w += bias2.w;
+            amx = fmaxf(fmaxf(amx, fmaxf(__builtin_fabsf(v.x), __builtin_fabsf(v.y))), fmaxf(__builtin_fabsf(v.z), __builtin_fabsf(v.w)));
+            const unsigned orow = (unsigned)sw_s(((unsigned)p * 32u + (unsigned)(2 * iz + pz)) * 32u + (unsigned)(2 * (4 * wave + 2 * h + t) + py));
+            __builtin_amdgcn_raw_buffer_store_b128(__builtin_bit_cast(i32x4, v), o2_rsrc, (int)st_off, (int)(orow * 1024u), 0);
+            ALQ_STORE_HOLD("v"(v));
+            if constexpr (SUMS) {
+                const float s = (v.x + v.y) + (v.z + v.w);
+                const float ts = s + __shfl_xor(s, 16, 64);
+                __builtin_amdgcn_raw_buffer_store_b32(__builtin_bit_cast(int, ts), u2_rsrc, (int)sm_off, (int)(orow * 128u), 0);
+            }
+        };
+        wload(0, W[0]);
+        fload(0, 0, F0);
+        fmask(F0[0], wave == 0 ? 0 : -1);
+        f32x4 last[2];
+#pragma unroll
+        for (int h = 0; h < 2; ++h) {
+            f32x4 uc[2][2][2];
+#pragma unroll
+            for (int t = 0; t < 2; ++t)
+#pragma unroll
+                for (int i = 0; i < 4; ++i) uc[t][i >> 1][i & 1] = f32x4{0.f, 0.f, 0.f, 0.f};
+#pragma unroll
+            for (int g = 0; g < 9; ++g) {
+                const int gg = 9 * h + g;
+                const int cz = g < 3 ? 2 : (g < 6 ? 0 : 1), cy = g % 3;
+                const int pz = cz == 2, py = cy == 2, dy = cy == 1;
+                __builtin_amdgcn_sched_barrier(0);
+                if (g < 8) wload(g + 1, W[(gg + 1) & 1]);
+                else if (h == 0) wload(0, W[(gg + 1) & 1]);
+                if (g == 5) fload(1, h, F1);
+                if (g == 6) {
+                    fmask(F1[0], keepz & ((h == 0 && wave == 0) ? 0 : -1));
+                    fmask(F1[1], keepz);
+                    fmask(F1[2], keepz);
+                }
+                if (g == 8 && h == 0) fload(0, 1, F0);
+                if (g == 0 && h == 1) { finish(last[0], 0, 0, 0, 1); finish(last[1], 0, 1, 0, 1); }
+                if (g == 2) { finish(uc[0][1][0], h, 0, 1, 0); finish(uc[1][1][0], h, 1, 1, 0); }
+                if (g == 3) { finish(uc[0][1][1], h, 0, 1, 1); finish(uc[1][1][1], h, 1, 1, 1); }
+                if (g == 8) { finish(uc[0][0][0], h, 0, 0, 0); finish(uc[1][0][0], h, 1, 0, 0); }
+                const bf16x8 *w = W[gg & 1];
+                bf16x8 (*F)[3] = g < 6 ? F0 : F1;
+                const bf16x8 *f0 = F[1 - dy], *f1 = F[2 - dy];
+                f32x4 c0 = uc[0][pz][py], c1 = uc[1][pz][py];
+                c0 = __builtin_amdgcn_mfma_f32_16x16x32_bf16(w[2], f0[0], c0, 0, 0, 0);
+                c1 = __builtin_amdgcn_mfma_f32_16x16x32_bf16(w[2], f1[0], c1, 0, 0, 0);
+                c0 = __builtin_amdgcn_mfma_f32_16x16x32_bf16(w[0], f0[2], c0, 0, 0, 0);
+                c1 = __builtin_amdgcn_mfma_f32_16x16x32_bf16(w[0], f1[2], c1, 0, 0, 0);
+                c0 = __builtin_amdgcn_mfma_f32_16x16x32_bf16(w[1], f0[1], c0, 0, 0, 0);
+                c1 = __builtin_amdgcn_mfma_f32_16x16x32_bf16(w[1], f1[1], c1, 0, 0, 0);
+                c0 = __builtin_amdgcn_mfma_f32_16x16x32_bf16(w[1], f0[0], c0, 0, 0, 0);
+                c1 = __builtin_amdgcn_mfma_f32_16x16x32_bf16(w[1], f1[0], c1, 0, 0, 0);
+                c0 = __builtin_amdgcn_mfma_f32_16x16x32_bf16(w[0], f0[1], c0, 0, 0, 0);
+                c1 = __builtin_amdgcn_mfma_f32_16x16x32_bf16(w[0], f1[1], c1, 0, 0, 0);
+                c0 = __builtin_amdgcn_mfma_f32_16x16x32_bf16(w[0], f0[0], c0, 0, 0, 0);
+                c1 = __builtin_amdgcn_mfma_f32_16x16x32_bf16(w[0], f1[0], c1, 0, 0, 0);
+                uc[0][pz][py] = c0; uc[1][pz][py] = c1;
+            }
+            last[0] = uc[0][0][1]; last[1] = uc[1][0][1];
+        }
+        __builtin_amdgcn_sched_barrier(0);
+        finish(last[0], 1, 0, 0, 1); finish(last[1], 1, 1, 0, 1);
+        __builtin_amdgcn_sched_barrier(0);
+#pragma unroll
+        for (int off = 32; off >= 1; off >>= 1) amx = fmaxf(amx, __shfl_xor(amx, off, 64));
+        amx_lds[(iz & 1) * 4 + wave] = amx;
+    };
+    auto amax_flush = [&](int p, int iz, bool ok) __attribute__((always_inline)) {
+        int ln = lane;
+        asm volatile("" : "+v"(ln));
+        const unsigned amx_off = (wave == 0 && ln == 0) ? 0u : SW_OOB;
+        float v = amx_lds[(iz & 1) * 4 + (ln & 3)];
+        v = fmaxf(v, __shfl_xor(v, 1, 64));
+        v = fmaxf(v, __shfl_xor(v, 2, 64));
+        __builtin_amdgcn_raw_buffer_store_b32(__builtin_bit_cast(int, v), amx_rsrc, (int)(ok ? amx_off : SW_OOB), sw_s((unsigned)(p * 16 + (ok ? iz : 0)) * 4u), 0);
+    };
+
+    auto step = [&](auto JJ, auto PH, int i, int s) __attribute__((always_inline)) {
+        constexpr int J = decltype(JJ)::value;
+        constexpr bool phase = decltype(PH)::value != 0;
+        constexpr int S0 = (J + 1) % 3, S1 = J, S2 = (J + 2) % 3;
+        __builtin_amdgcn_sched_barrier(0);
+        const int q = 16 * i + s;
+        const int p = patch_of(i);
+        const float inv = __builtin_ldexpf(1.f, -(patch_exp(p) + a.e_w));
+        const int pn = patch_of((q + 1) >> 4);
+        const int cen = patch_exp(pn);
+        const bool nv = ((q + 1) >> 4) < npw;
+        const float sc = nv ? __builtin_ldexpf(1.f, cen) : 0.f, sc11 = nv ? __builtin_ldexpf(1.f, cen + 11) : 0.f;
+        const int img = q & 1;
+        asm volatile("s_waitcnt lgkmcnt(0)\n\ts_barrier" ::: "memory");
+        if constexpr (phase) amax_flush(p, s - 2, s >= 2);
+        __builtin_amdgcn_sched_barrier(0);
+        const char *fb = f_base + img * DT_PLANE;
+        f16x8 Fh[2][3], Fl[2][3];
+        auto frag = [&](auto R, f16x8 *fh, f16x8 *fl) __attribute__((always_inline)) {
+            constexpr int r = decltype(R)::value;
+#pragma unroll
+            for (int dx = 0; dx < 3; ++dx) {
+                fh[dx] = *reinterpret_cast<const f16x8 *>(fb + r * DT_SLOT + dx * 16);
+                fl[dx] = *reinterpret_cast<const f16x8 *>(fb + r * DT_SLOT + dx * 16 + DT_ROWB);
+            }
+        };
+        frag(IC<0>{}, Fh[0], Fl[0]);
+        auto block = [&](auto R) __attribute__((always_inline)) {
+            constexpr int r = decltype(R)::value;
+            __builtin_amdgcn_sched_barrier(0);
+            if constexpr (r + 1 < 6) frag(IC<r + 1>{}, Fh[(r + 1) % 2], Fl[(r + 1) % 2]);
+            if constexpr (r == 1) { stage_unit(IC<0>{}, img ^ 1, sc, sc11); stage_unit(IC<1>{}, img ^ 1, sc, sc11); stage_unit(IC<2>{}, img ^ 1, sc, sc11); stage_unit(IC<3>{}, img ^ 1, sc, sc11); }
+            if constexpr (r == 2) { stage_unit(IC<4>{}, img ^ 1, sc, sc11); stage_unit(IC<5>{}, img ^ 1, sc, sc11); stage_unit(IC<6>{}, img ^ 1, sc, sc11); stage_unit(IC<7>{}, img ^ 1, sc, sc11); }
+            if constexpr (r == 3) {
+                fetch(q + 2);
+                epi_row(IC<S2>{}, IC<0>{}, p, s - 1, s >= 1, inv);
+            }
+            if constexpr (r == 4) epi_row(IC<S2>{}, IC<1>{}, p, s - 1, s >= 1, inv);
+            if constexpr (r == 5) epi_row(IC<S2>{}, IC<2>{}, p, s - 1, s >= 1, inv);
+#pragma unroll
+            for (int dx = 0; dx < 3; ++dx) {
+                const f16x8 xh = Fh[r % 2][dx], xl = Fl[r % 2][dx];
+#pragma unroll
+                for (int dy = 0; dy < 3; ++dy) {
+                    const int ry = r - dy;
+                    if (ry < 0 || ry > 3) continue;
+#pragma unroll
+                    for (int dz = 0; dz < 3; ++dz) {
+                        const int st = dz == 0 ? S0 : (dz == 1 ? S1 : S2);
+                        const int tap = (dz * 3 + dy) * 3 + dx;
+                        const bool first = dz == 0 && dy == 0 && dx == 0;
+                        const f32x4 zero = f32x4{0.f, 0.f, 0.f, 0.f};
+                        acx[st][ry] = __builtin_amdgcn_mfma_f32_16x16x32_f16(wl[tap], xh, first ? zero : acx[st][ry], 0, 0, 0);
+                        acc[st][ry] = __builtin_amdgcn_mfma_f32_16x16x32_f16(wh[tap], xh, first ? zero : acc[st][ry], 0, 0, 0);
+                        acx[st][ry] = __builtin_amdgcn_mfma_f32_16x16x32_f16(wh[tap], xl, acx[st][ry], 0, 0, 0);
+                    }
+                }
+            }
+#pragma unroll
+            for (int m = 0; m < 27 * ((r == 0 || r == 5) ? 1 : ((r == 1 || r == 4) ? 2 : 3)); ++m) {
+                __builtin_amdgcn_sched_group_barrier(0x008, 1, 0);
+                __builtin_amdgcn_sched_group_barrier(SW_FILL_MASK, DT_PIPE, 0);
+            }
+        };
+        block(IC<0>{}); block(IC<1>{}); block(IC<2>{}); block(IC<3>{}); block(IC<4>{}); block(IC<5>{});
+        __builtin_amdgcn_sched_barrier(0);
+        epi_row(IC<S2>{}, IC<3>{}, p, s - 1, s >= 1, inv);
+        if constexpr (STORE_MID) {
+            const f32x4 k0 = okeep[0], k1 = okeep[1];
+            asm volatile("" :: "v"(k0), "v"(k1));
+        }
+        if constexpr (phase) {
+            asm volatile("s_waitcnt lgkmcnt(0)\n\ts_barrier" ::: "memory");
+            up2_plane(p, s - 1);
+        }
+        __builtin_amdgcn_sched_barrier(0);
+    };
+
+    if (npw > 0) {
+        {
+            fetch(0);
+            const int ce = patch_exp(patch_of(0));
+            const float sc = __builtin_ldexpf(1.f, ce), sc11 = __builtin_ldexpf(1.f, ce + 11);
+            stage_unit(IC<0>{}, 0, sc, sc11); stage_unit(IC<1>{}, 0, sc, sc11); stage_unit(IC<2>{}, 0, sc, sc11); stage_unit(IC<3>{}, 0, sc, sc11);
+            stage_unit(IC<4>{}, 0, sc, sc11); stage_unit(IC<5>{}, 0, sc, sc11); stage_unit(IC<6>{}, 0, sc, sc11); stage_unit(IC<7>{}, 0, sc, sc11);
+            __builtin_amdgcn_sched_barrier(0);
+            fetch(1);
+        }
+        for (int i = 0; i < npw; ++i) {
+            step(IC<0>{}, IC<0>{}, i, 0);
+            for (int k = 0; k < 5; ++k) {
+                step(IC<1>{}, IC<1>{}, i, 3 * k + 1);
+                step(IC<2>{}, IC<1>{}, i, 3 * k + 2);
+                step(IC<0>{}, IC<1>{}, i, 3 * k + 3);
+            }
+            __builtin_amdgcn_sched_barrier(0);
+            const int p = patch_of(i);
+            const float inv = __builtin_ldexpf(1.f, -(patch_exp(p) + a.e_w));
+            asm volatile("s_waitcnt lgkmcnt(0)\n\ts_barrier" ::: "memory");
+            amax_flush(p, 14, true);
+            epi_row(IC<0>{}, IC<0>{}, p, 15, true, inv);
+            epi_row(IC<0>{}, IC<1>{}, p, 15, true, inv);
+            epi_row(IC<0>{}, IC<2>{}, p, 15, true, inv);
+            epi_row(IC<0>{}, IC<3>{}, p, 15, true, inv);
+#pragma unroll
+            for (int ry = 0; ry < 4; ++ry) { acc[0][ry] = f32x4{0.f, 0.f, 0.f, 0.f}; acx[0][ry] = f32x4{0.f, 0.f, 0.f, 0.f}; }
+            __builtin_amdgcn_sched_barrier(0);
+            if constexpr (STORE_MID) asm volatile("s_nop 7" :: "v"(okeep[0]), "v"(okeep[1]) : "memory");
+            asm volatile("s_waitcnt lgkmcnt(0)\n\ts_barrier" ::: "memory");
+            up2_plane(p, 15);
+            asm volatile("s_waitcnt lgkmcnt(0)\n\ts_barrier" ::: "memory");
+            amax_flush(p, 15, true);
+            __builtin_amdgcn_sched_barrier(0);
+        }
+    }
+}
+
+int d3t_fwd_launch(alq_ctx *ctx, const D3dPlan &plan, const T3dPlan &up, int N, const float *inA, const float *inB, const unsigned *amaxA, const unsigned *amaxB,
+                   const float *bias, int relu, float *mid, unsigned char *sg, float *osum, const float *bias2, float *out, float *osum2, unsigned *out_amax) {
+    ALQ_REQUIRE(plan.ok && plan.d_Whi && plan.d_Wlo, ALQ_EINVAL, "d3t: dec1 weights not set");
+    ALQ_REQUIRE(up.ok && up.kind == 0 && up.d_W, ALQ_EINVAL, "d3t: up2 weights not set");
+    ALQ_REQUIRE(inA && inB && amaxA && amaxB && bias && bias2 && out, ALQ_EINVAL, "d3t: missing argument");
+    ALQ_REQUIRE((osum != nullptr) == (osum2 != nullptr), ALQ_EINVAL, "d3t: channel sums of both layers or of none");
+    SWEEP_REQUIRE_PATCHES(N, "d3t");
+    if (N <= 0) return ALQ_OK;
+    D3TArgs a;
+    a.inA = inA; a.inB = inB; a.amaxA = amaxA; a.amaxB = amaxB;
+    a.Whi = reinterpret_cast<const unsigned short *>(plan.d_Whi); a.Wlo = reinterpret_cast<const unsigned short *>(plan.d_Wlo);
+    a.bias = bias; a.mid = mid; a.sg = sg; a.osum = osum;
+    a.W2 = reinterpret_cast<const unsigned short *>(up.d_W); a.bias2 = bias2; a.out = out; a.osum2 = osum2; a.out_amax = out_amax;
+    a.e_w = plan.w_exp; a.relu = relu; a.N = N;
+    unsigned grid = sweep_grid(ctx, N, 1);
+    if (g_dbg_knobs[KNOB_D3T_GRID_CAP] > 0) grid = std::min<unsigned>(grid, (unsigned)g_dbg_knobs[KNOB_D3T_GRID_CAP]);
+    ProfScope ps(ctx, PROF_IGEMM_F16, plan.flops_per_patch * N);
+    if (ps.active) {
+        ctx->prof[PROF_IGEMM3_FWD].launches += 1;
+        ctx->prof[PROF_IGEMM3_FWD].flops += up.flops_per_patch * N;
+    }
+    const bool sums = osum != nullptr;
+    if (sums && mid) return sweep_launch(ctx, d3t_fwd_kernel<true, true>, grid, 256, DT_LDS, a);
+    if (sums) return sweep_launch(ctx, d3t_fwd_kernel<true, false>, grid, 256, DT_LDS, a);
+    if (mid) return sweep_launch(ctx, d3t_fwd_kernel<false, true>, grid, 256, DT_LDS, a);
+    return sweep_launch(ctx, d3t_fwd_kernel<false, false>, grid, 256, DT_LDS, a);
+}
+
+}
diff --git a/nn-active-learning_amd/csrc/engine_switches.h b/nn-active-learning_amd/csrc/engine_switches.h
--- a/nn-active-learning_amd/csrc/engine_switches.h
+++ b/nn-active-learning_amd/csrc/engine_switches.h
@@ -16,11 +16,12 @@
     KNOB_NO_CONV_POOL = 7,
     KNOB_DCP_NARROW = 8,
     KNOB_E3D_GRID_CAP = 9,
-    ALQ_NKNOBS = 10
+    KNOB_D3T_GRID_CAP = 10,
+    ALQ_NKNOBS = 11
 };
 
 struct EngineSwitches {
-    int knobs[ALQ_NKNOBS] = {0, 0, 0, 0, 0, 0, 0, 0, 0, 0};
+    int knobs[ALQ_NKNOBS] = {0, 0, 0, 0, 0, 0, 0, 0, 0, 0, 0};
     int disable_v2 = 0;
     int disable_v3 = 0;
     int disable_v4 = 0;
@@ -57,6 +58,7 @@
     int no_d3b = 0;
     int no_f3d = 0;
     int no_t3d = 0;
+    int no_d3t = 0;
 };
 
 enum SwitchRule {
diff --git a/nn-active-learning_amd/csrc/igemm2.hip b/nn-active-learning_amd/csrc/igemm2.hip
--- a/nn-active-learning_amd/csrc/igemm2.hip
+++ b/nn-active-learning_amd/csrc/igemm2.hip
@@ -507,7 +507,7 @@
 int g_no_f16x2 = 0;
 int g_no_xcd_order = 0;
 int g_no_fixed = 0;
-int g_dbg_knobs[ALQ_NKNOBS] = {0, 0, 0, 0, 0, 0, 0, 0, 0, 0};
+int g_dbg_knobs[ALQ_NKNOBS] = {0, 0, 0, 0, 0, 0, 0, 0, 0, 0, 0};
 
 template <int NTW, bool WRES, int GEO, bool SUMS>
 static int launch2_s(alq_ctx *ctx, const Igemm2Plan &plan, const Igemm2Args &a, unsigned grid) {
diff --git a/nn-active-learning_amd/csrc/model.hip b/nn-active-learning_amd/csrc/model.hip
--- a/nn-active-learning_amd/csrc/model.hip
+++ b/nn-active-learning_amd/csrc/model.hip
@@ -18,7 +18,7 @@
 
 using namespace alq;
 
-static int g_knob_override[ALQ_NKNOBS] = {-1, -1, -1, -1, -1, -1, -1, -1, -1, -1};
+static int g_knob_override[ALQ_NKNOBS] = {-1, -1, -1, -1, -1, -1, -1, -1, -1, -1, -1};
 
 static void apply_knobs(const alq_model *m) {
     for (int k = 0; k < ALQ_NKNOBS; ++k) g_dbg_knobs[k] = g_knob_override[k] >= 0 ? g_knob_override[k] : m->sw.knobs[k];
@@ -595,6 +595,26 @@
            !(drop && drop->on(i)) && (!with_sums || ly.osum) && !(ly.t3f.kind == 8 && prod[i]);
 }
 
+static int materialise_dec1(alq_model *m) {
+    if (m->last.fwd.d3t != 1) return ALQ_OK;
+    const Layer &ly = m->layers[m->last.fwd.d3t_layer];
+    const View &in = ly.in;
+    ALQ_TRY(d3d_fwd_launch(m->ctx, ly.d3f, m->last.fwd.d3t_N, in.p, in.p + in.delta, m->last.fwd.d3t_amaxA, m->last.fwd.d3t_amaxB, ly.d_bias, ly.spec.relu ? 1 : 0,
+                           ly.out.p, nullptr, nullptr));
+    m->last.fwd.d3t = 2;
+    return ALQ_OK;
+}
+
+static bool d3t_fwd_applies(const alq_model *m, int i, const std::vector<char> &prod, const std::vector<char> &cons, bool with_sums, const DropSpec *drop) {
+    if (m->sw.no_d3t || i + 1 >= (int)m->layers.size()) return false;
+    const Layer &ly = m->layers[i], &nx = m->layers[i + 1];
+    if (nx.spec.type != ALQ_CONVT || nx.spec.skip_src >= 0 || !t3d_fwd_applies(m, i + 1, prod, cons, with_sums, drop) || nx.t3f.kind != 0) return false;
+    for (const Layer &l : m->layers)
+        if (l.spec.skip_src == i) return false;
+    return nx.in.p == ly.out.p && nx.in.cs == 16 && nx.in.c0 == 0 && nx.in.split == 0 && nx.in.D == 16 && nx.out.cs == 8 && nx.out.c0 == 0 && nx.out.split == 0 &&
+           nx.out.D == 32 && nx.d_bias && ly.spec.relu && !(drop && drop->on(i + 1));
+}
+
 int run_forward(alq_model *m, const float *d_x, int N, bool with_sums, bool keep_all, const DropSpec *drop) {
     alq_ctx *ctx = m->ctx;
     const int nl = (int)m->layers.size();
@@ -739,6 +759,26 @@
                 if (fuse) take_amax(fz, i);
                 if (d3d_fwd_applies(m, i, in, fuse, prod, with_sums, light, drop)) {
                     const bool sgd = with_sums && !m->sw.no_signs && ly.spec.relu && ly.out.sg;
+                    if (d3t_fwd_applies(m, i, prod, cons, with_sums, drop)) {
+                        const bool store_mid = with_sums && !(sgd && !g_dbg_knobs[KNOB_NO_BWD_FUSE] && !m->sw.no_bound16 && nx->t3b.ok && nx->t3b.d_W);
+                        const bool want_amax = prod[i + 1] != 0;
+                        ALQ_TRY(d3t_fwd_launch(ctx, ly.d3f, nx->t3f, N, in.p, in.p + in.delta, fz.in_amax, fz.in_amax2, ly.d_bias, 1, store_mid ? ly.out.p : nullptr,
+                                               sgd ? ly.out.sg : nullptr, fz.osumA, nx->d_bias, nx->out.p, with_sums ? nx->osum : nullptr,
+                                               want_amax ? m->amax_tiles : nullptr));
+                        if (want_amax) ALQ_TRY(k_rowmax_u32(ctx, m->amax_tiles, 16, N, nx->amax_fwd));
+                        ly.signs_ready = sgd;
+                        nx->signs_ready = false;
+                        fused = true;
+                        skip_next = true;
+                        m->last.fwd.d3f = 1;
+                        m->last.fwd.t3f += 1;
+                        m->last.fwd.d3t = store_mid ? 2 : 1;
+                        m->last.fwd.d3t_layer = i;
+                        m->last.fwd.d3t_N = N;
+                        m->last.fwd.d3t_amaxA = fz.in_amax;
+                        m->last.fwd.d3t_amaxB = fz.in_amax2;
+                        break;
+                    }
                     ALQ_TRY(d3d_fwd_launch(ctx, ly.d3f, N, in.p, in.p + in.delta, fz.in_amax, fz.in_amax2, ly.d_bias, ly.spec.relu ? 1 : 0, ly.out.p,
                                            sgd ? ly.out.sg : nullptr, fz.osumA));
                     ly.signs_ready = sgd;
@@ -999,6 +1039,7 @@
         }
         const bool isfc = ly.spec.type == ALQ_FC;
         if (!ly.delta_ready) {
+            if (i == m->last.fwd.d3t_layer) ALQ_TRY(materialise_dec1(m));
             View dv = isfc ? flat_view(ly.dout) : ly.dout;
             View av = isfc ? flat_view(ly.out) : ly.out;
             ALQ_TRY(k_mask_chansum(ctx, dv, ly.spec.relu ? &av : nullptr, ly.dsum, N));
@@ -1118,6 +1159,8 @@
                 }
                 const unsigned *mine = ly.dout_amax;
                 ly.dout_amax = nullptr;
+                if (i - 1 == m->last.fwd.d3t_layer && !(t3d_bwd_applies(m, ly, fuse, acc, hand, prev_param) && (!fz.mask || fz.mask_bits)))
+                    ALQ_TRY(materialise_dec1(m));
                 if (t3d_bwd_applies(m, ly, fuse, acc, hand, prev_param)) {
                     ALQ_TRY(t3d_bwd_launch(ctx, ly.t3b, ly.dout, ly.din, N, fz.in_bound, fz.mask ? fz.mask_bits : nullptr, fz.osumA));
                     fused = true;
@@ -1206,6 +1249,7 @@
     m->ctx = ctx;
     m->max_batch = max_batch;
     m->sw = read_engine_switches();
+    m->sw.no_d3t = getenv("ALQ_NO_D3T") != nullptr;
     for (int i = 0; i < 4; ++i) m->in_dims[i] = in_dims[i];
     m->epp = (int64_t)in_dims[0] * in_dims[1] * in_dims[2] * in_dims[3];
     const int rc = build_model(m, layers, n_layers);
@@ -1400,6 +1444,10 @@
                                  : (m->last.call_fisher && head.fc_maskbits != nullptr && two_slot_allowed()))),
                     ALQ_EUNSUPPORTED, "layer %d: this tensor is not materialised in a Fisher pass (fc head fused into the layer: "
                     "create the model under ALQ_NO_FC_BITS=1 to keep it)", layer_idx);
+        if (what == 0 && m->last.fwd.d3t == 1 && layer_idx == m->last.fwd.d3t_layer) {
+            ALQ_REQUIRE(N <= m->last.fwd.d3t_N, ALQ_EUNSUPPORTED, "layer %d: not materialised for %d patches", layer_idx, N);
+            ALQ_TRY(materialise_dec1(m));
+        }
         const View &v = what == 0 ? ly.out : ly.dout;
         if (elems_out) *elems_out = (int64_t)N * v.elems();
         return debug_view_copy(m->ctx, v, N, d_out);
@@ -1445,6 +1493,7 @@
         case ALQ_INFO_LSUM: return m->last.lsum;
         case ALQ_INFO_DCP_FORM: return m->last.fwd.dcp;
         case ALQ_INFO_E3D_BWD_FORM: return m->last.bwd.e3b_form;
+        case ALQ_INFO_D3T_FWD: return m->last.fwd.d3t;
         default: break;
     }
     set_error("alq_model_engine_info: bad argument");
diff --git a/nn-active-learning_amd/csrc/model_types.h b/nn-active-learning_amd/csrc/model_types.h
--- a/nn-active-learning_amd/csrc/model_types.h
+++ b/nn-active-learning_amd/csrc/model_types.h
@@ -78,6 +78,9 @@
         bool c3 = false;
         int t3f = 0;
         int d3f = 0;
+        int d3t = 0;
+        int d3t_layer = -1, d3t_N = 0;
+        const unsigned *d3t_amaxA = nullptr, *d3t_amaxB = nullptr;
         int f3f = 0;
         int dcp = 0;
         bool f16_derived = false;
diff --git a/nn-active-learning_amd/csrc/sweep_common.h b/nn-active-learning_amd/csrc/sweep_common.h
--- a/nn-active-learning_amd/csrc/sweep_common.h
+++ b/nn-active-learning_amd/csrc/sweep_common.h
@@ -32,6 +32,17 @@
     return fm ? (ce < 96 ? ce : 96) : 0;
 }
 
+__device__ inline unsigned t3_split2(float &a, float &b) {
+    const bf16x2 h = __builtin_convertvector(f32x2{a, b}, bf16x2);
+    const unsigned hb = __builtin_bit_cast(unsigned, h);
+    a -= __builtin_bit_cast(float, hb << 16);
+    b -= __builtin_bit_cast(float, hb & 0xffff0000u);
+    return hb;
+}
+__device__ inline unsigned t3_pack2(float a, float b) {
+    return __builtin_amdgcn_perm(__builtin_bit_cast(unsigned, b), __builtin_bit_cast(unsigned, a), 0x07060302u);
+}
+
 #define SW_XCD_DEAL(N)                                                                                         \
     const int G8 = (int)gridDim.x >> 3, xcd = (int)blockIdx.x & 7, jb = (int)blockIdx.x >> 3;                  \
     const int npx = (N) > xcd ? ((N) - xcd + 7) >> 3 : 0
diff --git a/nn-active-learning_amd/csrc/t3d.hip b/nn-active-learning_amd/csrc/t3d.hip
--- a/nn-active-learning_amd/csrc/t3d.hip
+++ b/nn-active-learning_amd/csrc/t3d.hip
@@ -35,16 +35,6 @@
 constexpr int T3F_ROWB = 17 * 32, T3F_WAVE = 2 * 3 * T3F_ROWB;
 constexpr int T3B_ROWB = 34 * 16, T3B_WAVE = 6 * 2 * T3B_ROWB;
 
-__device__ inline unsigned t3_split2(float &a, float &b) {
-    const bf16x2 h = __builtin_convertvector(f32x2{a, b}, bf16x2);
-    const unsigned hb = __builtin_bit_cast(unsigned, h);
-    a -= __builtin_bit_cast(float, hb << 16);
-    b -= __builtin_bit_cast(float, hb & 0xffff0000u);
-    return hb;
-}
-__device__ inline unsigned t3_pack2(float a, float b) {
-    return __builtin_amdgcn_perm(__builtin_bit_cast(unsigned, b), __builtin_bit_cast(unsigned, a), 0x07060302u);
-}
 
 struct T3Cur { int p, iz, s; bool ok; };
 __device__ inline T3Cur t3_tile(int T, int total, int wave) {
```

Result: no change. 286,300 (median of 6 runs) (+0.9%).
